# lebrice/blurred-GAN

Hardware: AMD Instinct MI355X
Metric: images/sec (G+D+GP step) (higher is better)
Workload: dtype f32; 1 GPU; celeba64 64x64x3 batch 256/GPU, blur sigma 5.0 (31 taps), D-step+GP+G-step+Adam; global_batch=256, parallelism=dp1

## Files before the change

### blurred-gan_amd/_lib.py

```python
from __future__ import annotations

import ctypes as C
import os

HERE = os.path.dirname(os.path.abspath(__file__))
LIB_PATH = os.environ.get("BGAN_HIP_LIB") or os.path.join(HERE, "libbgan_hip.so")


class BgError(RuntimeError):
    pass


class Epilogue(C.Structure):
    _fields_ = [("mode", C.c_int), ("bias", C.c_void_p), ("ref", C.c_void_p), ("keep", C.c_void_p),
                ("alpha", C.c_float), ("scale", C.c_float), ("splitk_ws", C.c_void_p), ("splitk_ws_bytes", C.c_size_t),
                ("keep_elems", C.c_size_t), ("stats", C.c_void_p), ("stats_capacity", C.c_size_t), ("stats_rows", C.POINTER(C.c_int))]


ABI_VERSION = 5
EPI_NONE, EPI_BIAS_LRELU, EPI_MUL_GRAD, EPI_TANH, EPI_AFFINE_LRELU = 0, 1, 2, 3, 4

_p, _i, _f, _z, _u64 = C.c_void_p, C.c_int, C.c_float, C.c_size_t, C.c_uint64

SIGNATURES = {
    "bg_version": (_i, []),
    "bg_last_error": (C.c_char_p, []),
    "bg_status_string": (C.c_char_p, [_i]),
    "bg_prof_enable": (_i, [_i]),
    "bg_prof_reset": (_i, []),
    "bg_prof_count": (_i, []),
    "bg_prof_get": (_i, [_i, C.c_char_p, _i, C.POINTER(_f), C.POINTER(C.c_double), C.POINTER(C.c_double)]),
    "bg_prof_get_exec": (_i, [_i, C.POINTER(C.c_double)]),
    "bg_prof_get_useful": (_i, [_i, C.POINTER(C.c_double)]),
    "bg_conv2d_useful_flops": (C.c_double, [_i] * 7),
    "bg_range_enable": (_i, [_i]),
    "bg_range_push": (_i, [C.c_char_p]),
    "bg_range_pop": (_i, []),
    "bg_blur_policy": (_i, [_f, _i, _i, C.POINTER(_f), C.POINTER(_f), C.POINTER(_i)]),
    "bg_gauss_kernel_1d": (_i, [_f, _f, C.POINTER(_f), _i, C.POINTER(_i)]),
    "bg_blur_workspace_bytes": (_z, [_i, _i, _i, _i, _i]),
    "bg_blur_nhwc_f32": (_i, [_p, _p, _i, _i, _i, _i, _p, _i, _p, _p]),
    "bg_blur3_lerp_supported": (_i, [_i, _i, _i, _i, _i]),
    "bg_blur3_lerp_nhwc_f32": (_i, [_p, _p, _p, _p, _i, _i, _i, _i, _p, _i, _p]),
    "bg_conv2d_splitk_workspace_bytes": (_z, [_i, _i, _i, _i, _i, _i, _i, _i]),
    "bg_conv2d_fwd": (_i, [_p, _p, _p, _i, _i, _i, _i, _i, _i, _i, C.POINTER(Epilogue), _p]),
    "bg_conv2d_bwd_data": (_i, [_p, _p, _p, _i, _i, _i, _i, _i, _i, _i, C.POINTER(Epilogue), _p]),
    "bg_conv2d_fwd_math": (_i, [_p, _p, _p, _i, _i, _i, _i, _i, _i, _i, C.POINTER(Epilogue), _p, _i]),
    "bg_conv2d_bwd_data_math": (_i, [_p, _p, _p, _i, _i, _i, _i, _i, _i, _i, C.POINTER(Epilogue), _p, _i]),
    "bg_conv2d_math_taken": (_i, [_i] * 9),
    "bg_conv2d_bwd_filter_workspace_bytes": (_z, [_i, _i, _i, _i, _i, _i, _i]),
    "bg_conv2d_bwd_filter": (_i, [_p, _p, _p, _i, _i, _i, _i, _i, _i, _i, _f, _f, _p, _z, _p]),
    "bg_transpose_last2": (_i, [_p, _p, _i, _i, _i, _p]),
    "bg_transpose_last2_batched": (_i, [_p, _p, _p, _i, _i, _p]),
    "bg_gemm_f32": (_i, [_p, _p, _p, _i, _i, _i, _i, _i, _p, _f, _f, _p]),
    "bg_colsum_workspace_bytes": (_z, [_i, _i]),
    "bg_colsum_f32": (_i, [_p, _p, _i, _i, _i, _f, _f, _p, _z, _p]),
    "bg_bn_workspace_bytes": (_z, [_i, _i]),
    "bg_bn_train_fwd": (_i, [_p, _p, _i, _i, _p, _p, _p, _p, _p, _p, _f, _f, _i, _f, _p, _z, _p]),
    "bg_bn_train_fwd_partials": (_i, [_p, _i, _p, _p, _i, _i, _p, _p, _p, _p, _p, _p, _f, _f, _i, _f, _p]),
    "bg_bn_sums_from_partials": (_i, [_p, _i, _i, _p, _p]),
    "bg_bn_infer_fwd": (_i, [_p, _p, _i, _i, _p, _p, _p, _p, _f, _f, _p]),
    "bg_bn_train_bwd": (_i, [_p, _p, _p, _p, _i, _i, _p, _p, _p, _p, _p, _p, _f, _p, _z, _p]),
    "bg_bn_fold_f32": (_i, [_p, _p, _p, _p, _f, _i, _p, _p, _p]),
    "bg_bn_fold_many_f32": (_i, [_i, _p, _p, _p, _p, _p, _p, _p, _p, _p]),
    "bg_bn_stats_f32": (_i, [_p, _i, _i, _p, _p, _z, _p]),
    "bg_bn_finalize_f32": (_i, [_p, _i, _i, _p, _p, _p, _p, _f, _f, _i, _p]),
    "bg_bn_apply_f32": (_i, [_p, _p, _i, _i, _p, _p, _p, _p, _f, _p]),
    "bg_bn_finalize_apply_f32": (_i, [_p, _i, _p, _p, _i, _i, _p, _p, _p, _p, _p, _p, _f, _f, _i, _f, _p]),
    "bg_bn_bwd_stats_f32": (_i, [_p, _p, _p, _i, _i, _p, _p, _p, _p, _f, _p, _p, _z, _p]),
    "bg_bn_bwd_apply_f32": (_i, [_p, _p, _p, _p, _i, _i, _i, _p, _p, _p, _p, _p, _f, _p]),
    "bg_bn_param_grads_f32": (_i, [_p, _i, _f, _p, _p, _p]),
    "bg_ln_route": (_i, [_i, C.POINTER(_i), C.POINTER(_i), C.POINTER(_i), C.POINTER(_i)]),
    "bg_ln_workspace_bytes": (_z, [_i, _i]),
    "bg_ln_fwd_f32": (_i, [_p, _p, _i, _i, _p, _p, _f, _f, _p, _f, _z, _p, _p, _p]),
    "bg_ln_bwd_f32": (_i, [_p, _p, _p, _i, _i, _p, _p, _p, _p, _f, _p, _f, _z, _p, _p, _i, _i, _p, _p, _i, _f, _f, _p, _z, _p]),
    "bg_ln_tangent_f32": (_i, [_p, _p, _p, _i, _i, _p, _p, _p, _p, _f, _p]),
    "bg_ln_gp_source_f32": (_i, [_p, _p, _p, _p, _i, _i, _p, _p, _p, _p, _f, _f, _p, _z, _p]),
    "bg_pixelnorm_route": (_i, [_i, C.POINTER(_i)]),
    "bg_pixelnorm_fwd_f32": (_i, [_p, _p, _p, _i, _i, _f, _f, _p]),
    "bg_pixelnorm_bwd_f32": (_i, [_p, _p, _p, _p, _i, _i, _f, _p]),
    "bg_diffaug_route": (_i, [_i, _i, _i, C.POINTER(_i), C.POINTER(_i)]),
    "bg_diffaug_plan": (_i, [_i, _i, _i, _i, _i] + [C.POINTER(_i)] * 5),
    "bg_diffaug_decode": (_i, [C.POINTER(_f), _i, _i, _i, _f, _f, C.POINTER(_f), C.POINTER(_i)]),
    "bg_diffaug_f32": (_i, [_p, _p, _p, _i, _i, _i, _i, _i, _f, _f, _i, _p]),
    "bg_diffaug_adjoint_f32": (_i, [_p, _p, _p, _i, _i, _i, _i, _i, _f, _f, _p]),
    "bg_mbstd_plan": (_i, [_i, _i, _i, _i, _i, _i, C.POINTER(_i)]),
    "bg_mbstd_workspace_bytes": (_z, [_i, _i, _i, _i]),
    "bg_mbstd_fwd_f32": (_i, [_p, _p, _p, _p, _p, _i, _i, _i, _i, _f, _p, _z, _p]),
    "bg_mbstd_bwd_f32": (_i, [_p, _p, _p, _p, _p, _p, _i, _i, _i, _i, _p]),
    "bg_mbstd_gp_f32": (_i, [_p, _p, _p, _p, _p, _p, _p, _p, _i, _i, _i, _i, _f, _p, _z, _p]),
    "bg_spectral_route":(_i, [_i, _i, _i] + [C.POINTER(_i)] * 8),
    "bg_spectral_workspace_bytes": (_z, [_p, _i]),
    "bg_spectral_power_f32": (_i, [_p, _p, _p, _p, _i, _i, _p, _z, _p]),
    "bg_spectral_scale_f32": (_i, [_p, _p, _p, _p, _p, _i, _p]),
    "bg_spectral_grad_f32": (_i, [_p, _p, _p, _p, _p, _i, _p, _z, _p]),
    "bg_eqlr_plan": (_i, [_i, _i, _i] + [C.POINTER(_i)] * 4),
    "bg_eqlr_check_table": (_i, [_p, _i, _z, _z]),
    "bg_eqlr_scale_f32": (_i, [_p, _z, _p, _z, _p, _p, _i, _p]),
    "bg_eqlr_grad_f32": (_i, [_p, _z, _p, _p, _i, _p]),
    "bg_lerp_f32":(_i, [_p, _p, _p, _p, _i, _i, _p]),
    "bg_row_norm_f32": (_i, [_p, _p, _i, _i, _p]),
    "bg_gp_seed_f32": (_i, [_p, _p, _f, _p, _i, _i, _p]),
    "bg_gp_seed_guarded_f32": (_i, [_p, _p, _f, _p, _i, _i, _p]),
    "bg_mul_grad_f32": (_i, [_p, _p, _p, _f, _f, _p, _z, _p]),
    "bg_tanh_bwd_f32": (_i, [_p, _p, _p, _z, _p]),
    "bg_outer_f32": (_i, [_p, _p, _p, _i, _i, _p]),
    "bg_fill_f32": (_i, [_p, _f, _z, _p]),
    "bg_scale_f32": (_i, [_p, _f, _z, _p]),
    "bg_copy_f32": (_i, [_p, _p, _z, _p]),
    "bg_upsample2x_nhwc_f32": (_i, [_p, _p, _i, _i, _i, _i, _f, _p, _p, _f, _f, _p]),
    "bg_pool2x_sum_nhwc_f32": (_i, [_p, _p, _i, _i, _i, _i, _f, _p]),
    "bg_wgangp_d_loss": (_i, [_p, _p, _p, _i, _f, _f, _f, _f, _p, _p, _p, _p]),
# ... 79 lines not shown
```

### blurred-gan_amd/csrc/conv_rows.hip

```cpp
#include "conv_common.h"
#include <algorithm>
#include <cstdlib>
#include <cstring>
#include <type_traits>

namespace {

typedef float floatx4 __attribute__((ext_vector_type(4)));

struct RowParams {
  const float* A;
  const float* Wt;
  float* C;
  int B, Hi, Wi, Ck, Ho, Wo, N;
  int pt, pl, flip;
  int R, strips;
  int wpr, ipw;
  int epi_mode;
  const float* bias;
  const float* ref;
  const unsigned char* keep;
  size_t keep_elems;
  float alpha, scale;
};

__device__ inline int floordiv(int a, int b) { return a >= 0 ? a / b : -((-a + b - 1) / b); }

__device__ inline float tanh_branchless(float x) {
  float ax = fabsf(x);
  ax = ax > 15.f ? 15.f : ax;
  const float e = __builtin_amdgcn_exp2f(ax * 2.885390081777927f);
  const float big = 1.f - 2.f * __builtin_amdgcn_rcpf(e + 1.f);
  const float x2 = ax * ax;
  const float small = ax * fmaf(x2, fmaf(x2, fmaf(x2, -17.f / 315.f, 2.f / 15.f), -1.f / 3.f), 1.f);
  return copysignf(ax < 0.1f ? small : big, x);
}

template <int KS, int K, int S, int PIXW, int EP>
__global__ __launch_bounds__(PIXW * 4) void conv_rows_scatter_kernel(const RowParams p) {
  constexpr int NTH = PIXW * 4;
  constexpr unsigned kOob = 0x80000000u;
  extern __shared__ __attribute__((aligned(16))) float row_lds[];
  constexpr int AS = 4 * KS + 4;
  float* abuf = row_lds;
  constexpr int PS = PIXW * 17 + 1;
  float* pbuf = row_lds + 2 * PIXW * AS;
  const int tid = threadIdx.x, lane = tid & 63, wave = tid >> 6;
  const int li = lane & 15, kq = lane >> 4;
  const int t = wave % p.wpr, img = wave / p.wpr;
  const int strip = blockIdx.x % p.strips, bgrp = blockIdx.x / p.strips;
  const int Ck = 4 * KS, N = p.N;
  const int y0 = strip * p.R, y1 = min(y0 + p.R, p.Ho);
  const int iy_lo = -floordiv(-(y0 + p.pt - (K - 1)), S);
  const int iy_hi = floordiv(y1 - 1 + p.pt, S);
  const int nrows = iy_hi - iy_lo + 1;
  const int nimg = min(p.ipw, p.B - bgrp * p.ipw);
  const size_t img0 = (size_t)bgrp * p.ipw;
  const __amdgpu_buffer_rsrc_t rsA = __builtin_amdgcn_make_buffer_rsrc(const_cast<float*>(p.A + img0 * p.Hi * p.Wi * Ck), 0,
                                                                        nimg * p.Hi * p.Wi * Ck * 4, 0x00020000);
  const __amdgpu_buffer_rsrc_t rsC = __builtin_amdgcn_make_buffer_rsrc(p.C + img0 * p.Ho * p.Wo * N, 0, nimg * p.Ho * p.Wo * N * 4, 0x00020000);

  float bw[K][KS];
  {
    const int lc = min(li, K * N - 1);
    const int kw = lc / N, n = lc - kw * N;
#pragma unroll
    for (int kh = 0; kh < K; ++kh) {
      const int tap = p.flip ? (K - 1 - kh) * K + (K - 1 - kw) : kh * K + kw;
#pragma unroll
      for (int ks = 0; ks < KS; ++ks) {
        const float w = p.Wt[((size_t)tap * N + n) * Ck + 4 * ks + kq];
        bw[kh][ks] = li < K * N ? w : 0.f;
      }
    }
  }
  floatx4 acc[K];
#pragma unroll
  for (int i = 0; i < K; ++i) acc[i] = floatx4{0.f, 0.f, 0.f, 0.f};

  constexpr int QPR = KS;
  constexpr int NQ = PIXW * QPR / NTH;
  static_assert(NQ >= 1, "Ck >= 16");
  unsigned g_off[NQ], l_off[NQ];
#pragma unroll
  for (int q = 0; q < NQ; ++q) {
    const int f = tid + q * NTH, pix = f / QPR, c4 = f - pix * QPR;
    const int im = pix / p.Wi, ix = pix - im * p.Wi;
    g_off[q] = im < nimg ? (unsigned)(((im * p.Hi * p.Wi + ix) * Ck + c4 * 4) * 4) : kOob;
    l_off[q] = (unsigned)(pix * AS + c4 * 4);
  }
  const int rowB = p.Wi * Ck * 4;
  auto gload = [&](int r, float4 (&g)[NQ]) {
    const int iy = iy_lo + r;
    const bool row_ok = r < nrows && (unsigned)iy < (unsigned)p.Hi;
    const unsigned add = row_ok ? (unsigned)(iy * rowB) : 0u, force = row_ok ? 0u : kOob;
#pragma unroll
    for (int q = 0; q < NQ; ++q)
      g[q] = __builtin_bit_cast(float4, __builtin_amdgcn_raw_buffer_load_b128(rsA, (g_off[q] + add) | force, 0, 0));
  };
  auto lstore = [&](int buf, const float4 (&g)[NQ]) {
#pragma unroll
    for (int q = 0; q < NQ; ++q) *reinterpret_cast<float4*>(abuf + (size_t)buf * PIXW * AS + l_off[q]) = g[q];
  };
  const float* afrag = abuf + ((size_t)img * p.Wi + 16 * t + li) * AS + kq;
  constexpr int NE = (S * (16 / K) + 3) / 4;
  constexpr int NTERM = (K + S - 1) / S;
  int e_src[NE][NTERM];
  unsigned e_dst[NE];
  float e_bias[NE], e_mul[NE];
  int e_n[NE];
  if (tid < 2 * S) pbuf[(size_t)tid * PS + PIXW * 17] = 0.f;
  {
    const int per_img = p.Wo * N;
#pragma unroll
    for (int q = 0; q < NE; ++q) {
      const int e = tid + q * NTH;
      const int im = e / per_img, rem = e - im * per_img;
      const int x = rem / N, n = rem - x * N;
      const bool ok = e < p.ipw * per_img && im < nimg;
      e_dst[q] = ok ? (unsigned)(((im * p.Ho * p.Wo + x) * N + n) * 4) : kOob;
      e_n[q] = n;
      e_bias[q] = ok && p.bias ? p.bias[n] : 0.f;
      e_mul[q] = ok && p.epi_mode == BG_EPI_AFFINE_LRELU ? p.ref[n] : 0.f;
#pragma unroll
      for (int i = 0; i < NTERM; ++i) {
        const int kw = (x + p.pl) % S + i * S;
        const int num = x + p.pl - kw, ix = num / S;
        e_src[q][i] = (ok && kw < K && num >= 0 && ix < p.Wi) ? (im * p.Wi + ix) * 17 + kw * N + n : PIXW * 17;
      }
    }
  }
  const size_t out0 = img0 * p.Ho * p.Wo * N;
  auto pwrite = [&](const floatx4& pacc, int slot) {
    float* pb = pbuf + (size_t)slot * PS;
#pragma unroll
    for (int rr = 0; rr < 4; ++rr) pb[((size_t)img * p.Wi + 16 * t + 4 * kq + rr) * 17 + li] = pacc[rr];
  };
  auto pstore = [&](int slot, int y, bool live) {
    const float* pb = pbuf + (size_t)slot * PS;
    float v[NE];
#pragma unroll
    for (int q = 0; q < NE; ++q) {
      v[q] = pb[e_src[q][0]];
#pragma unroll
      for (int i = 1; i < NTERM; ++i) v[q] += pb[e_src[q][i]];
    }
    const unsigned add = live ? (unsigned)(y * p.Wo * N * 4) : 0u, force = live ? 0u : kOob;
#pragma unroll
    for (int q = 0; q < NE; ++q) {
      const unsigned off = (e_dst[q] + add) | force;
      float o;
      if (EP == 0) {
        o = v[q] + e_bias[q];
      } else if (EP == 1) {
        o = tanh_branchless(v[q] + e_bias[q]);
      } else {
        const bool mine = (off & kOob) == 0;
        o = mine ? bg::apply_epilogue_pre(p, v[q], out0 + (off >> 2), e_bias[q], e_mul[q]) : 0.f;
      }
      __builtin_amdgcn_raw_buffer_store_b32(__builtin_bit_cast(unsigned, o), rsC, off, 0, 0);
    }
  };

  float4 g0[NQ], g1[NQ], g2[NQ], g3[NQ];
  gload(0, g0);
  gload(1, g1);
  gload(2, g2);
  gload(3, g3);
  lstore(0, g0);
  gload(4, g0);
#pragma unroll
  for (int i = 0; i < 4 * NE * S; ++i) __builtin_amdgcn_raw_buffer_store_b32(0u, rsC, kOob + 4u * i, 0, 0);
  int y_prev = 0;
  bool have_prev = false;
  auto flush_prev = [&](int prev_par) {
#pragma unroll
    for (int kh = 0; kh < S; ++kh) {
      const int y = y_prev + kh;
      pstore(prev_par * S + kh, y, have_prev & (y >= y0) & (y < y1));
    }
  };
  auto trip = [&](int r, auto parity, float4 (&g)[NQ]) {
    constexpr int cur = decltype(parity)::value;
    __syncthreads();
    float a[KS];
#pragma unroll
    for (int ks = 0; ks < KS; ++ks) a[ks] = afrag[(size_t)cur * PIXW * AS + 4 * ks];
#pragma unroll
    for (int ks = 0; ks < KS; ++ks)
#pragma unroll
      for (int kh = 0; kh < K; ++kh) acc[kh] = __builtin_amdgcn_mfma_f32_16x16x4f32(a[ks], bw[kh][ks], acc[kh], 0, 0, 0);
    flush_prev(cur ^ 1);
    lstore(cur ^ 1, g);
    gload(r + 5, g);
#pragma unroll
    for (int kh = 0; kh < S; ++kh) pwrite(acc[kh], cur * S + kh);
    y_prev = (iy_lo + r) * S - p.pt;
    have_prev = true;
#pragma unroll
    for (int i = 0; i < K; ++i) acc[i] = i + S < K ? acc[i + S] : floatx4{0.f, 0.f, 0.f, 0.f};
  };
  int r = 0;
  for (; r + 4 <= nrows; r += 4) {
    trip(r, std::integral_constant<int, 0>{}, g1);
    trip(r + 1, std::integral_constant<int, 1>{}, g2);
    trip(r + 2, std::integral_constant<int, 0>{}, g3);
    trip(r + 3, std::integral_constant<int, 1>{}, g0);
  }
  int last_par = 1;
  if (r < nrows) {
    trip(r, std::integral_constant<int, 0>{}, g1);
    last_par = 0;
    if (r + 1 < nrows) {
      trip(r + 1, std::integral_constant<int, 1>{}, g2);
      last_par = 1;
      if (r + 2 < nrows) {
        trip(r + 2, std::integral_constant<int, 0>{}, g3);
        last_par = 0;
      }
    }
  }
  __syncthreads();
  if (last_par == 0) flush_prev(0); else flush_prev(1);
}

template <int K, int S>
int launch_rows(const RowParams& p, dim3 grid, size_t lds, hipStream_t s) {
  const bool wide = p.Wi == 128;
  const int ep = p.epi_mode == BG_EPI_NONE ? 0 : p.epi_mode == BG_EPI_TANH ? 1 : 2;
#define BG_RS2(KSv, EPv) do { if (wide) bg::launch((conv_rows_scatter_kernel<KSv, K, S, 128, EPv>), grid, dim3(512), lds, s, p); \
                              else bg::launch((conv_rows_scatter_kernel<KSv, K, S, 64, EPv>), grid, dim3(256), lds, s, p); } while (0)
#define BG_RS(KSv) do { if (ep == 0) BG_RS2(KSv, 0); else if (ep == 1) BG_RS2(KSv, 1); else BG_RS2(KSv, 2); } while (0)
  switch (p.Ck) {
    case 16: BG_RS(4); return 1;
    case 32: BG_RS(8); return 1;
    case 64: BG_RS(16); return 1;
    default: return 0;
  }
#undef BG_RS
#undef BG_RS2
}

constexpr int kRgHalo = 16;

struct RowGParams {
  const float* A;
  const float* Wt;
  float* C;
  int B, Hi, Wi, Ct, Ho, Wo, N;
  int s, pt, pl, flip;
  int R, strips;
  int epi_mode;
  const float* bias;
  const float* ref;
  const unsigned char* keep;
  size_t keep_elems;
  float alpha, scale;
};

template <int TG, int NT, int K, bool MASK>
__global__ __launch_bounds__(256) void conv_rows_gather_kernel(const RowGParams p) {
  extern __shared__ __attribute__((aligned(16))) float xl[];
  const int tid = threadIdx.x, lane = tid & 63, wave = tid >> 6;
  const int li = lane & 15, kq = lane >> 4;
  const int Ct = p.Ct, N = 16 * NT, st = p.s;
  const int RS = p.Wi * Ct + 2 * kRgHalo;
  const int strip = blockIdx.x % p.strips, b = blockIdx.x / p.strips;
  const int oy0 = strip * p.R, rows = min(p.R, p.Ho - oy0);
  const int nrows_in = (rows - 1) * st + K;

  float bw[K][4][NT];
#pragma unroll
  for (int ks = 0; ks < 4; ++ks) {
    const int i = 4 * ks + kq, kw = i / Ct, ci = i - kw * Ct;
#pragma unroll
    for (int kh = 0; kh < K; ++kh) {
      const int tap = p.flip ? (K - 1 - kh) * K + (K - 1 - kw) : kh * K + kw;
#pragma unroll
      for (int nt = 0; nt < NT; ++nt) bw[kh][ks][nt] = i < K * Ct ? p.Wt[((size_t)tap * N + nt * 16 + li) * Ct + ci] : 0.f;
    }
  }
  const int RL = p.Wi * Ct;
// ... 89 lines not shown
#undef BG_RG
  return 1;
}

}

namespace bg {

int try_conv_rows_gather(int bwd_data, const float* a, const float* w, float* c, int B, int H, int W, int Cin, int Cout, int k, int s,
                         const bg_epilogue* epi, void* stream, int* taken) {
  *taken = 0;
  static const int off = getenv("BG_NO_ROWS") ? 1 : 0;
  if (off || (k != 5 && k != 3)) return BG_OK;
  RowGParams p;
  memset(&p, 0, sizeof p);
  int Ho, Wo, pt, pl;
  same_pads(H, k, s, &Ho, &pt);
  same_pads(W, k, s, &Wo, &pl);
  if (bwd_data) {
    if (s != 1 || Cout * k > 16 || (Cin != 16 && Cin != 32 && Cin != 64)) return BG_OK;
    p.Hi = H; p.Wi = W; p.Ct = Cout; p.Ho = H; p.Wo = W; p.N = Cin; p.s = 1; p.pt = k - 1 - pt; p.pl = k - 1 - pl; p.flip = 1;
  } else {
    if (Cin * k > 16 || (Cout != 16 && Cout != 32 && Cout != 64)) return BG_OK;
    p.Hi = H; p.Wi = W; p.Ct = Cin; p.Ho = Ho; p.Wo = Wo; p.N = Cout; p.s = s; p.pt = pt; p.pl = pl; p.flip = 0;
  }
  if (p.Wo % 16 != 0) return BG_OK;
  if ((size_t)B * p.Ho * p.Wo * p.N >= (1ull << 31)) return BG_OK;
  const int tiles = p.Wo / 16;
  const int tg = tiles % 4 == 0 ? 4 : (tiles % 2 == 0 ? 2 : 1);
  p.A = a; p.Wt = w; p.C = c; p.B = B;
  static const int rows_r = getenv("BG_ROWSG_R") ? atoi(getenv("BG_ROWSG_R")) : 0;
  p.R = std::min(rows_r ? rows_r : (s == 2 ? 8 : 16), p.Ho);
  p.strips = (int)cdiv(p.Ho, p.R);
  const size_t lds = ((size_t)((p.R - 1) * p.s + k) * (p.Wi * p.Ct + 2 * kRgHalo)) * sizeof(float);
  if (lds > 64 * 1024) return BG_OK;
  p.epi_mode = BG_EPI_NONE; p.alpha = 0.3f; p.scale = 1.f;
  if (epi) {
    BG_REQUIRE(epi->mode >= BG_EPI_NONE && epi->mode <= BG_EPI_AFFINE_LRELU, BG_ERR_UNSUPPORTED, "conv rows: epilogue mode %d", epi->mode);
    BG_REQUIRE(epi->mode != BG_EPI_MUL_GRAD || epi->ref, BG_ERR_NULL, "conv rows: BG_EPI_MUL_GRAD needs ref");
    BG_REQUIRE(epi->mode != BG_EPI_AFFINE_LRELU || (epi->ref && epi->bias), BG_ERR_NULL, "conv rows: BG_EPI_AFFINE_LRELU needs ref and bias");
    p.epi_mode = epi->mode; p.bias = epi->bias; p.ref = epi->ref; p.keep = epi->keep; p.keep_elems = epi->keep_elems; p.alpha = epi->alpha; p.scale = epi->scale;
  }
  const dim3 grid((unsigned)(B * p.strips));
  const double flops = 2.0 * B * (double)Ho * Wo * Cin * Cout * k * k;
  Launch L(stream, bwd_data ? "conv_rows_thin_k_dgrad" : "conv_rows_thin_k_fwd", flops, 0);
  if (k == 5) launch_rows_gather<5>(p, tg, grid, lds, L.s);
  else launch_rows_gather<3>(p, tg, grid, lds, L.s);
  *taken = 1;
  return L.done("conv_rows_gather_kernel");
}



int try_conv_rows(int bwd_data, const float* a, const float* w, float* c, int B, int H, int W, int Cin, int Cout, int k, int s,
                  const bg_epilogue* epi, void* stream, int* taken) {
  *taken = 0;
  static const int off = getenv("BG_NO_ROWS") ? 1 : 0;
  if (off || (k != 5 && k != 3)) return BG_OK;
  RowParams p;
  memset(&p, 0, sizeof p);
  int Ho, Wo, pt, pl;
  same_pads(H, k, s, &Ho, &pt);
  same_pads(W, k, s, &Wo, &pl);
  if (bwd_data) {
    if (Cin * k > 16 || (Cout != 16 && Cout != 32 && Cout != 64)) return BG_OK;
    p.Hi = Ho; p.Wi = Wo; p.Ck = Cout; p.Ho = H; p.Wo = W; p.N = Cin; p.pt = pt; p.pl = pl; p.flip = 0;
  } else {
    if (s != 1 || Cout * k > 16 || (Cin != 16 && Cin != 32 && Cin != 64)) return BG_OK;
    p.Hi = H; p.Wi = W; p.Ck = Cin; p.Ho = H; p.Wo = W; p.N = Cout; p.pt = k - 1 - pt; p.pl = k - 1 - pl; p.flip = 1;
  }
  if (p.Wi != 16 && p.Wi != 32 && p.Wi != 64 && p.Wi != 128) return BG_OK;
  if ((size_t)B * p.Hi * p.Wi * p.Ck >= (1ull << 31) || (size_t)B * p.Ho * p.Wo * p.N >= (1ull << 31)) return BG_OK;
  p.A = a; p.Wt = w; p.C = c; p.B = B;
  static const int rows_r = getenv("BG_ROWS_R") ? atoi(getenv("BG_ROWS_R")) : 0;
  p.R = std::min(rows_r ? rows_r : (s == 1 ? 32 : 16), p.Ho);
  p.strips = (int)cdiv(p.Ho, p.R);
  p.wpr = p.Wi / 16;
  p.ipw = p.Wi == 128 ? 1 : 4 / p.wpr;
  const int pixw = p.Wi == 128 ? 128 : 64;
  if ((long)p.ipw * p.Wo * p.N > (long)((s * (16 / k) + 3) / 4) * pixw * 4) return BG_OK;
  if ((size_t)p.ipw * p.Hi * p.Wi * p.Ck >= (1ull << 29) || (size_t)p.ipw * p.Ho * p.Wo * p.N >= (1ull << 29)) return BG_OK;
  p.epi_mode = BG_EPI_NONE; p.alpha = 0.3f; p.scale = 1.f;
  if (epi) {
    BG_REQUIRE(epi->mode >= BG_EPI_NONE && epi->mode <= BG_EPI_AFFINE_LRELU, BG_ERR_UNSUPPORTED, "conv rows: epilogue mode %d", epi->mode);
    BG_REQUIRE(epi->mode != BG_EPI_MUL_GRAD || epi->ref, BG_ERR_NULL, "conv rows: BG_EPI_MUL_GRAD needs ref");
    BG_REQUIRE(epi->mode != BG_EPI_AFFINE_LRELU || (epi->ref && epi->bias), BG_ERR_NULL, "conv rows: BG_EPI_AFFINE_LRELU needs ref and bias");
    p.epi_mode = epi->mode; p.bias = epi->bias; p.ref = epi->ref; p.keep = epi->keep; p.keep_elems = epi->keep_elems; p.alpha = epi->alpha; p.scale = epi->scale;
  }
  const dim3 grid((unsigned)(cdiv(B, p.ipw) * p.strips));
  const size_t lds = ((size_t)2 * pixw * (p.Ck + 4) + (size_t)2 * s * (pixw * 17 + 1)) * sizeof(float);
  const double flops = 2.0 * B * (double)H * W * Cin * Cout * k * k / (s * s);
  Launch L(stream, bwd_data ? "conv_rows_dgrad" : "conv_rows_fwd", flops, 0);
  int ok;
  if (k == 5) ok = s == 2 ? launch_rows<5, 2>(p, grid, lds, L.s) : launch_rows<5, 1>(p, grid, lds, L.s);
  else ok = s == 2 ? launch_rows<3, 2>(p, grid, lds, L.s) : launch_rows<3, 1>(p, grid, lds, L.s);
  (void)ok;
  *taken = 1;
  return L.done("conv_rows_scatter_kernel");
}

}
```

### blurred-gan_amd/csrc/conv_wgrad.hip

```cpp
#include "conv_common.h"
#include <algorithm>
#include <cmath>
#include <cstdlib>
#include <mutex>
#include <type_traits>
#include <utility>

namespace {

typedef float floatx16 __attribute__((ext_vector_type(16)));

struct WgradParams {
  const float* X;
  const float* DY;
  float* out;
  int B, H, W, Ci, Ho, Wo, Co;
  int k, s, pt, pl;
  int M;
  int chunk;
  int ksplit;
  int tiles_m, tiles_n, xcd_swizzle;
  float beta, scale;
  unsigned x_bytes, dy_bytes;
  unsigned mul_hw, sh_hw, mul_w, sh_w;
  int lg_w, lg_h, lg_b, pow2;
  int order_n;
  unsigned char tap_order[32];
};

__device__ inline int fastdiv(int m, unsigned mul, unsigned sh) { return (int)(((unsigned long long)(unsigned)m * mul) >> sh); }

template <int BM, int BN, int BKP, int WAVES_M, int WAVES_N, int WAVES_K, int P2>
__global__ __launch_bounds__(256) void conv_wgrad_v3_kernel(const WgradParams p) {
  static_assert(WAVES_M * WAVES_N * WAVES_K == 4, "4 waves");
  constexpr int WTM = BM / WAVES_M, WTN = BN / WAVES_N;
  constexpr int MI = WTM / 32, NI = WTN / 32;
  static_assert(MI >= 1 && NI >= 1 && WTM % 32 == 0 && WTN % 32 == 0, "wave tile");
  constexpr int TPR_A = BM / 4, RPP_A = 256 / TPR_A, AP = BKP / RPP_A;
  constexpr int TPR_B = BN / 4, RPP_B = 256 / TPR_B, BP = BKP / RPP_B;
  static_assert(AP >= 1 && BP >= 1 && BKP % RPP_A == 0 && BKP % RPP_B == 0, "loader passes must tile the chunk exactly");
  constexpr int STAGE = BKP * (BM + BN);
  constexpr int RED = (WAVES_K > 1) ? (WAVES_K - 1) * WAVES_M * WAVES_N * MI * NI * 1024 : 0;
  constexpr int SMEM = (2 * STAGE > RED) ? 2 * STAGE : RED;
  constexpr unsigned kOob = 0x80000000u;
  __shared__ __attribute__((aligned(16))) float smem[SMEM];

  const int tid = threadIdx.x, lane = tid & 63, wave = tid >> 6;
  const int wk = wave % WAVES_K, wmn = wave / WAVES_K;
  const int wm = wmn / WAVES_N, wn = wmn % WAVES_N;
  const int ntile = p.tiles_m * p.tiles_n, ntap = p.k * p.k;
  int tile, tap, zsplit;
  if (P2 == 2 && p.order_n > 0) {
    const int w = blockIdx.x, r = w >> 8;
    const int u = ((r & 1) && ((r + 1) << 8) <= (int)gridDim.x) ? (r << 8) + ((31 - ((w & 255) >> 3)) << 3) + (w & 7) : w;
    tile = u % ntile;
    const int rest = u / ntile;
    zsplit = rest % p.ksplit;
    tap = p.tap_order[rest / p.ksplit];
  } else {
    const int L = p.xcd_swizzle ? bg::xcd_remap(blockIdx.x, gridDim.x) : (int)blockIdx.x;
    tile = L % ntile; tap = (L / ntile) % ntap; zsplit = L / (ntile * ntap);
  }
  const int tile_m = tile / p.tiles_n, tile_n = tile % p.tiles_n;
  const int ci0 = tile_m * BM, co0 = tile_n * BN;
  const int kh = tap / p.k, kw = tap % p.k;
  const int m_begin = zsplit * p.chunk;
  const int m_end = min(p.M, m_begin + p.chunk);
  const int nsteps = (m_end - m_begin + BKP - 1) / BKP;

  const __amdgpu_buffer_rsrc_t rsX = __builtin_amdgcn_make_buffer_rsrc(const_cast<float*>(p.X), 0, (int)p.x_bytes, 0x00020000);
  const __amdgpu_buffer_rsrc_t rsY = __builtin_amdgcn_make_buffer_rsrc(const_cast<float*>(p.DY), 0, (int)p.dy_bytes, 0x00020000);
  const int arow = tid / TPR_A, aq = tid % TPR_A;
  const int brow = tid / TPR_B, bq = tid % TPR_B;
  const int HoWo = p.Ho * p.Wo;
  const bool a_col_ok = ci0 + aq * 4 < p.Ci, b_col_ok = co0 + bq * 4 < p.Co;
  const int a_coloff = (ci0 + aq * 4) * 4, b_coloff = (co0 + bq * 4) * 4;
  const int dyk = kh - p.pt, dxk = kw - p.pl;
  float4 regA[AP], regB[BP];

  const int WoS = p.Wo * p.s, HoS = p.Ho * p.s;
// ... 632 lines not shown
          const int ci = ci0 + row, co = co0 + col;
          ok = ci < p.Ci && co < p.Co;
          idx = ((size_t)tap * p.Ci + ci) * p.Co + co;
        } else if (MODE == 1) {
          const int co = co0 + col;
          ok = row < kk * p.Ci && co < p.Co;
          idx = (size_t)row * p.Co + co;
        } else {
          const int ci = ci0 + row;
          const int t = col / p.Co, co = col - t * p.Co;
          ok = ci < p.Ci && col < kk * p.Co;
          idx = ((size_t)t * p.Ci + ci) * p.Co + co;
        }
        if (ok) {
          float* q = out + idx;
          const float v = acc[i][j][r];
          if (direct) *q = (p.beta != 0.f ? p.beta * *q : 0.f) + p.scale * v;
          else *q = v;
        }
      }
    }
}

__global__ __launch_bounds__(256) void wgrad_direct_kernel(const WgradParams p) {
  const int nout = p.k * p.k * p.Ci * p.Co;
  const int e = blockIdx.x * 256 + threadIdx.x;
  if (e >= nout) return;
  const int co = e % p.Co;
  const int ci = (e / p.Co) % p.Ci;
  const int tap = e / (p.Co * p.Ci);
  const int kh = tap / p.k, kw = tap % p.k;
  const int m_begin = blockIdx.y * p.chunk, m_end = min(p.M, m_begin + p.chunk);
  const int HoWo = p.Ho * p.Wo;
  int b = m_begin / HoWo;
  int rem = m_begin - b * HoWo;
  int oh = rem / p.Wo, ow = rem - oh * p.Wo;
  float acc = 0.f;
  for (int m = m_begin; m < m_end; ++m) {
    const int iy = oh * p.s + kh - p.pt, ix = ow * p.s + kw - p.pl;
    if ((unsigned)iy < (unsigned)p.H && (unsigned)ix < (unsigned)p.W)
      acc = fmaf(p.X[((size_t)(b * p.H + iy) * p.W + ix) * p.Ci + ci], p.DY[(size_t)m * p.Co + co], acc);
    if (++ow == p.Wo) {
      ow = 0;
      if (++oh == p.Ho) { oh = 0; ++b; }
    }
  }
  float* q = p.out + (size_t)blockIdx.y * nout + e;
  if (p.ksplit == 1) *q = (p.beta != 0.f ? p.beta * *q : 0.f) + p.scale * acc;
  else *q = acc;
}

typedef float floatx4 __attribute__((ext_vector_type(4)));
constexpr int kTcRows = 16, kTcHalo = 8;

template <int MT, int K>
__global__ __launch_bounds__(256) void conv_wgrad_thin_co_kernel(const WgradParams p, int nblocks, int blocks_per_img) {
  extern __shared__ __attribute__((aligned(16))) float tc_lds[];
  const int W = p.W, H = p.H, Ci = 16 * MT, Co = p.Co;
  const int RS = W * Co + 2 * kTcHalo;
  const int nrows = kTcRows + K - 1;
  const int tid = threadIdx.x, lane = tid & 63, wave = tid >> 6;
  const int li = lane & 15, kq = lane >> 4;
  floatx4 acc[K][MT];
#pragma unroll
  for (int kh = 0; kh < K; ++kh)
#pragma unroll
    for (int mt = 0; mt < MT; ++mt) acc[kh][mt] = floatx4{0.f, 0.f, 0.f, 0.f};
  const int ncol = K * Co;
  const int kw_n = li / Co, co_n = li - kw_n * Co;
  const int b_base = li < ncol ? kTcHalo + (kq + p.pl - kw_n) * Co + co_n : 0;
  const int b_step = li < ncol ? 4 * Co : 0;
  const int ksteps = W / 4;

  for (int blk = blockIdx.x; blk < nblocks; blk += gridDim.x) {
    const int b = blk / blocks_per_img, y0 = (blk - b * blocks_per_img) * kTcRows;
    __syncthreads();
    if (((W * Co) & 3) == 0) {
      const int q4 = RS / 4;
      bg::stage_rows_f4<4>(tc_lds, nrows, q4, RS, tid, [&](int r, int c4) -> const float* {
        const int oy = y0 - (K - 1 - p.pt) + r, e = c4 * 4 - kTcHalo;
        return ((unsigned)oy < (unsigned)p.Ho && (unsigned)e < (unsigned)(W * Co)) ? p.DY + ((size_t)b * p.Ho + oy) * W * Co + e : nullptr;
      });
    } else {
      for (int idx = tid; idx < nrows * RS; idx += 256) {
        const int r = idx / RS, c = idx - r * RS;
        const int oy = y0 - (K - 1 - p.pt) + r, e = c - kTcHalo;
        float v = 0.f;
        if ((unsigned)oy < (unsigned)p.Ho && (unsigned)e < (unsigned)(W * Co)) v = p.DY[((size_t)b * p.Ho + oy) * W * Co + e];
        tc_lds[idx] = v;
      }
    }
    __syncthreads();
    const int groups = (ksteps + 7) / 8;
    const int myrows = min(kTcRows, H - y0);
    const int nitems = ((myrows - wave + 3) / 4) * groups;
    const float* xblk = p.X + ((size_t)b * H + y0) * W * Ci + kq * Ci + li;
    auto xload = [&](int it, float (&a)[8][MT]) {
      const int j = it / groups, g = it - j * groups;
      const float* xrow = xblk + (size_t)(wave + 4 * j) * W * Ci + (size_t)g * 32 * Ci;
#pragma unroll
      for (int q = 0; q < 8; ++q)
#pragma unroll
        for (int mt = 0; mt < MT; ++mt) a[q][mt] = (it < nitems && g * 8 + q < ksteps) ? xrow[(size_t)q * 4 * Ci + mt * 16] : 0.f;
    };
    auto compute = [&](int it, const float (&a)[8][MT]) {
      const int j = it / groups, g = it - j * groups;
      const int r = wave + 4 * j;
#pragma unroll
      for (int kh = 0; kh < K; ++kh) {
        const float* brow = tc_lds + (r + (K - 1) - kh) * RS + b_base + g * 8 * b_step;
#pragma unroll
        for (int q = 0; q < 8; ++q) {
          const float bv = brow[q * b_step];
#pragma unroll
          for (int mt = 0; mt < MT; ++mt) acc[kh][mt] = __builtin_amdgcn_mfma_f32_16x16x4f32(a[q][mt], bv, acc[kh][mt], 0, 0, 0);
        }
      }
    };
    float a0[8][MT], a1[8][MT];
    xload(0, a0);
    for (int it = 0; it < nitems; it += 2) {
      xload(it + 1, a1);
      compute(it, a0);
      xload(it + 2, a0);
      if (it + 1 < nitems) compute(it + 1, a1);
    }
  }
  __syncthreads();
  float* red = tc_lds;
#pragma unroll
  for (int kh = 0; kh < K; ++kh)
#pragma unroll
    for (int mt = 0; mt < MT; ++mt)
#pragma unroll
      for (int rr = 0; rr < 4; ++rr) red[((wave * K + kh) * MT * 4 + mt * 4 + rr) * 64 + lane] = acc[kh][mt][rr];
  __syncthreads();
  float* out = p.out + (size_t)blockIdx.x * K * K * Ci * Co;
  for (int e = tid; e < K * MT * 4 * 64; e += 256) {
    const int l = e & 63, slot = e >> 6;
    const int rr = slot & 3, mt = (slot >> 2) % MT, kh = slot / (4 * MT);
    const int n = l & 15;
    if (n >= ncol) continue;
    const float v = (red[(0 * K * MT * 4 + slot) * 64 + l] + red[(1 * K * MT * 4 + slot) * 64 + l]) +
                    (red[(2 * K * MT * 4 + slot) * 64 + l] + red[(3 * K * MT * 4 + slot) * 64 + l]);
    const int kw = n / Co, co = n - kw * Co, ci = mt * 16 + 4 * (l >> 4) + rr;
    out[((size_t)(kh * K + kw) * Ci + ci) * Co + co] = v;
  }
}

constexpr int kTiHalo = 16;

template <int NT, int K>
__global__ __launch_bounds__(256) void conv_wgrad_thin_ci_kernel(const WgradParams p, int nblocks, int blocks_per_img, int RB) {
  extern __shared__ __attribute__((aligned(16))) float ti_lds[];
  const int W = p.W, H = p.H, Ci = p.Ci, Co = 16 * NT, Ho = p.Ho, Wo = p.Wo, st = p.s;
  const int RS = W * Ci + 2 * kTiHalo;
  const int nrows = (RB - 1) * st + K;
  const int tid = threadIdx.x, lane = tid & 63, wave = tid >> 6;
  const int li = lane & 15, kq = lane >> 4;
  floatx4 acc[K][NT];
// ... 464 lines not shown
    }
    if (z < ksplit) {
      const float4 v0 = *reinterpret_cast<const float4*>(slabs + (size_t)z * n + e);
      s0.x += v0.x; s0.y += v0.y; s0.z += v0.z; s0.w += v0.w;
    }
  }
  red[zg][c] = make_float4(s0.x + s1.x, s0.y + s1.y, s0.z + s1.z, s0.w + s1.w);
  __syncthreads();
  for (int h = 32; h > 0; h >>= 1) {
    if (zg < h) {
      const float4 a = red[zg][c], b = red[zg + h][c];
      red[zg][c] = make_float4(a.x + b.x, a.y + b.y, a.z + b.z, a.w + b.w);
    }
    __syncthreads();
  }
  if (zg != 0 || e >= n) return;
  const float4 a = red[0][c];
  float4 o = make_float4(scale * a.x, scale * a.y, scale * a.z, scale * a.w);
  if (beta != 0.f) {
    const float4 q = *reinterpret_cast<const float4*>(dw + e);
    o.x += beta * q.x; o.y += beta * q.y; o.z += beta * q.z; o.w += beta * q.w;
  }
  *reinterpret_cast<float4*>(dw + e) = o;
}

__global__ __launch_bounds__(256) void wgrad_reduce_scalar_kernel(const float* __restrict__ slabs, float* __restrict__ dw, int n,
                                                                  int ksplit, float beta, float scale) {
  const int e = blockIdx.x * 256 + threadIdx.x;
  if (e >= n) return;
  float s = 0.f;
  for (int z = 0; z < ksplit; ++z) s += slabs[(size_t)z * n + e];
  dw[e] = (beta != 0.f ? beta * dw[e] : 0.f) + scale * s;
}

struct WgradPlan {
  int mode;
  int ksplit, chunk, tiles_m, tiles_n, bkp, taps_in_grid;
  int always_slab;
};

inline bool strip_ok(int H, int W, int Ci, int Co, int k, int s) {
  if (k != 5 || s != 2 || (H & 1) || (W & 1) || Ci % 32 || Co % 64) return false;
  const int Wo = W / 2, Ho = H / 2;
  if (Wo != 8 && Wo != 16 && Wo != 32) return false;
  return Ho % (64 / Wo) == 0;
}

constexpr size_t kRowLdsMax = 64 * 1024;
inline int thin_ci_rows(int s) { return s == 2 ? 8 : 16; }
inline size_t thin_ci_lds(int W, int Ci, int Co, int k, int s) {
  return std::max((size_t)((thin_ci_rows(s) - 1) * s + k) * ((size_t)W * Ci + 2 * kTiHalo), (size_t)k * (Co / 16) * 4 * 64) * sizeof(float);
}
inline size_t thin_co_lds(int W, int Ci, int Co, int k) {
  return std::max((size_t)(kTcRows + k - 1) * ((size_t)W * Co + 2 * kTcHalo), (size_t)4 * k * (Ci / 16) * 4 * 64) * sizeof(float);
}

WgradPlan plan_wgrad(int B, int H, int W, int Ci, int Co, int k, int s) {
  WgradPlan pl{};
  int Ho, Wo, pt, pp;
  bg::same_pads(H, k, s, &Ho, &pt);
  bg::same_pads(W, k, s, &Wo, &pp);
  const long M = (long)B * Ho * Wo;
  const bool mfma = (Ci % 4 == 0) && (Co % 4 == 0) && Ci >= 16 && Co >= 16;
  const int kk = k * k;
  const bool thin_ci = Ci <= 4 && Co % 4 == 0 && Co >= 16 && kk * Ci <= 128;
  const bool thin_co = Co <= 4 && Ci % 4 == 0 && Ci >= 16 && s == 1 && kk * Co <= 128;
  int bm = 0, bn = 0;
  if (!mfma && !thin_ci && !thin_co) {
    pl.mode = 0;
    const long nblk = bg::cdiv((size_t)k * k * Ci * Co, 256);
    long want = std::max(1L, 2048 / nblk);
    long chunk = std::max(256L, (M + want - 1) / want);
    pl.chunk = (int)chunk;
    pl.ksplit = (int)((M + chunk - 1) / chunk);
    return pl;
  }
  static const int no_strip = getenv("BG_WGRAD_NO_STRIP") ? 1 : 0;
  if (strip_ok(H, W, Ci, Co, k, s) && !no_strip) {
    pl.mode = 33;
    pl.bkp = 2;
    pl.tiles_m = Ci / 32;
    pl.tiles_n = Co / 64;
    const long nstrips = (long)B * (Ho / (64 / Wo));
    const long ntile = (long)pl.tiles_m * pl.tiles_n;
    long ks = std::max(1L, std::min(nstrips, std::max(1L, 256 / ntile)));
    long spw = (nstrips + ks - 1) / ks;
    ks = (nstrips + spw - 1) / spw;
    pl.ksplit = (int)ks;
    pl.chunk = (int)spw;
    pl.taps_in_grid = 0;
    pl.always_slab = 1;
    return pl;
  }
  static const int no_c16 = getenv("BG_NO_C16") ? 1 : 0;
  if (Ci == 16 && Co == 32 && k == 5 && s == 2 && !(H & 1) && !(W & 1) && (Wo == 32 || Wo == 64) && !(Ho & 1) && !no_c16) {
    pl.mode = 32;
    pl.bkp = 4;
    const long nstrips = (long)B * (Ho / 2);
    pl.ksplit = (int)std::max<long>(2, std::min<long>(nstrips, 256));
    pl.chunk = (int)nstrips;
    pl.tiles_m = pl.tiles_n = 1;
    pl.taps_in_grid = 0;
    return pl;
  }
  static const int no_tc = getenv("BG_WGRAD_NO_TC") ? 1 : 0;
  if (thin_ci && k * Ci <= 16 && (k == 5 || k == 3) && (Co == 16 || Co == 32 || Co == 64) && Wo % 4 == 0 && !no_tc &&
      thin_ci_lds(W, Ci, Co, k, s) <= kRowLdsMax) {
// ... 39 lines not shown
  static const int no_tg = getenv("BG_WGRAD_NO_TG") ? 1 : 0;
  if (k == 5 && Ci <= 64 && !no_tg && M >= 131072) {
    pl.bkp = 32; bm = 32;
    if (Co > 32) { pl.mode = 6; bn = 64; } else { pl.mode = 7; bn = 32; }
    pl.tiles_m = bg::cdiv(Ci, bm);
    pl.tiles_n = bg::cdiv(Co, bn);
    pl.taps_in_grid = 2;
  } else {
  if (Ci > 64 && Co > 64) { pl.mode = 1; bm = 128; bn = 128; pl.bkp = 32; }
  else if (Ci > 32 && Co > 32) { pl.mode = 2; bm = 64; bn = 64; pl.bkp = 32; }
  else if (Ci > 32) { pl.mode = 3; bm = 64; bn = 32; pl.bkp = 64; }
  else if (Co > 32) { pl.mode = 4; bm = 32; bn = 64; pl.bkp = 64; }
  else { pl.mode = 5; bm = 32; bn = 32; pl.bkp = 128; }
  pl.tiles_m = bg::cdiv(Ci, bm);
  pl.tiles_n = bg::cdiv(Co, bn);
  pl.taps_in_grid = 1;
  }
  }
  const long base = (long)pl.tiles_m * pl.tiles_n * (pl.taps_in_grid == 1 ? kk : (pl.taps_in_grid == 2 ? k : 1));
  const long steps = (M + pl.bkp - 1) / pl.bkp;
  long want;
  const bool skipping = Ho * Wo <= 16 && B >= 128 && B % 128 == 0;
  if (pl.taps_in_grid != 1 || skipping) {
    static const int tgt_env = getenv("BG_WGRAD_TARGET") ? atoi(getenv("BG_WGRAD_TARGET")) : 0;
    const int tgt = tgt_env ? tgt_env : (pl.taps_in_grid == 2 && M >= 200000 ? 1536 : 768);
    want = std::max(1L, (tgt + base - 1) / base);
    want = std::min(want, std::max(1L, steps / (skipping ? 8 : 4)));
    if ((size_t)kk * Ci * Co * sizeof(float) > (8u << 20)) want = std::min(want, 2L);
  } else {
    const int bm_eff = pl.taps_in_grid == 2 ? k * bm : bm;
    const int lds = 2 * pl.bkp * (bm_eff + bn) * 4;
    const int per_cu = std::max(1, std::min(160 * 1024 / lds, 5));
    const double slots = 256.0 * per_cu;
    const double t_step = 2.0 * bm_eff * bn * pl.bkp * per_cu / 614e9 * 1e6;
    const double ovh = 5.0 / t_step;
    const double nout_bytes = (double)kk * Ci * Co * 4.0;
    double best = 1e30;
    want = 1;
    for (long ks = 1; ks <= std::min<long>(64, std::max(1L, steps / 4)); ++ks) {
      const double rounds = std::ceil(base * ks / slots);
      const double per_wg = std::ceil((double)steps / ks);
      const double cost = rounds * (per_wg + ovh) * t_step + (ks > 1 ? 5.0 + (ks + 1) * nout_bytes / 3.5e6 + ks * nout_bytes / 5e6 : 0.0);
      if (cost < best * 0.999) { best = cost; want = ks; }
    }
  }
  long chunk = ((M + want - 1) / want + pl.bkp - 1) / pl.bkp * pl.bkp;
  pl.chunk = (int)chunk;
  pl.ksplit = (int)((M + chunk - 1) / chunk);
  return pl;
}

}

extern "C" {

size_t bg_conv2d_bwd_filter_workspace_bytes(int B, int H, int W, int Cin, int Cout, int ksize, int stride) {
  if (B <= 0 || H <= 0 || W <= 0 || Cin <= 0 || Cout <= 0 || ksize <= 0 || stride <= 0) return 0;
  WgradPlan pl = plan_wgrad(B, H, W, Cin, Cout, ksize, stride);
  if (pl.ksplit <= 1 && !pl.always_slab) return 0;
  return (size_t)pl.ksplit * ksize * ksize * Cin * Cout * sizeof(float);
}

int bg_conv2d_bwd_filter(const float* x, const float* dy, float* dw, int B, int H, int W, int Cin, int Cout, int ksize,
                         int stride, float beta, float scale, void* ws_d, size_t ws_bytes, void* stream) {
  BG_REQUIRE(x && dy && dw, BG_ERR_NULL, "bg_conv2d_bwd_filter: null pointer");
  BG_REQUIRE(B > 0 && H > 0 && W > 0 && Cin > 0 && Cout > 0, BG_ERR_BAD_SHAPE, "bg_conv2d_bwd_filter: B=%d H=%d W=%d Cin=%d Cout=%d", B, H, W, Cin, Cout);
  BG_REQUIRE(ksize >= 1 && (ksize & 1) && ksize * ksize <= bg::kMaxTaps, BG_ERR_UNSUPPORTED, "bg_conv2d_bwd_filter: kernel size %d", ksize);
  BG_REQUIRE(stride == 1 || stride == 2, BG_ERR_UNSUPPORTED, "bg_conv2d_bwd_filter: stride %d", stride);
  BG_REQUIRE(bg::aligned16(x) && bg::aligned16(dy) && bg::aligned16(dw), BG_ERR_BAD_ALIGNMENT, "bg_conv2d_bwd_filter: pointers must be 16-byte aligned");
  bg::UsefulScope useful(bg::conv_useful_flops(B, H, W, Cin, Cout, ksize, stride));
  WgradPlan pl = plan_wgrad(B, H, W, Cin, Cout, ksize, stride);
  const size_t nout = (size_t)ksize * ksize * Cin * Cout;
  const bool slabs = pl.ksplit > 1 || pl.always_slab;
  const size_t need = slabs ? (size_t)pl.ksplit * nout * sizeof(float) : 0;
  BG_REQUIRE(need == 0 || (ws_d && ws_bytes >= need), BG_ERR_WORKSPACE, "bg_conv2d_bwd_filter: workspace %zu bytes < %zu needed", ws_bytes, need);
  WgradParams p;
  memset(&p, 0, sizeof p);
  p.X = x; p.DY = dy;
  p.B = B; p.H = H; p.W = W; p.Ci = Cin; p.Co = Cout; p.k = ksize; p.s = stride;
  bg::same_pads(H, ksize, stride, &p.Ho, &p.pt);
  bg::same_pads(W, ksize, stride, &p.Wo, &p.pl);
  p.M = B * p.Ho * p.Wo;
  BG_REQUIRE((size_t)B * H * W * (size_t)Cin < (1ull << 29) && (size_t)p.M * (size_t)Cout < (1ull << 29), BG_ERR_UNSUPPORTED,
             "bg_conv2d_bwd_filter: tensor exceeds 2 GiB");
  {
    auto magic = [](unsigned d, unsigned* mul, unsigned* sh) {
      unsigned sft = 0;
      while ((1ull << sft) < d) ++sft;
      *mul = (unsigned)((1ull << (31 + sft)) / d + 1);
      *sh = 31 + sft;
    };
    magic((unsigned)(p.Ho * p.Wo), &p.mul_hw, &p.sh_hw);
    magic((unsigned)p.Wo, &p.mul_w, &p.sh_w);
    auto lg2 = [](int v) { int l = 0; while ((1 << l) < v) ++l; return l; };
    p.lg_w = lg2(p.Wo); p.lg_h = lg2(p.Ho);
    p.pow2 = ((1 << p.lg_w) == p.Wo && (1 << p.lg_h) == p.Ho) ? 1 : 0;
    p.lg_b = lg2(B);
    static const int no_pm = getenv("BG_NO_POS_MAJOR") ? 1 : 0;
    if (p.pow2 && !no_pm && B % 128 == 0 && B >= 128 && p.Ho * p.Wo <= 16) p.pow2 = 2;
    p.x_bytes = (unsigned)((size_t)B * H * W * Cin * sizeof(float));
    p.dy_bytes = (unsigned)((size_t)p.M * Cout * sizeof(float));
  }
  p.chunk = pl.chunk; p.ksplit = pl.ksplit; p.tiles_n = pl.tiles_n; p.tiles_m = pl.tiles_m;
  {
    static const int swz = getenv("BG_WGRAD_SWZ") ? atoi(getenv("BG_WGRAD_SWZ")) : 0;
    static const int swz_tg = getenv("BG_WGRAD_SWZ_TG") ? atoi(getenv("BG_WGRAD_SWZ_TG")) : 1;
    p.xcd_swizzle = (pl.mode == 6 || pl.mode == 7) ? swz_tg : swz;
  }
  p.beta = beta; p.scale = scale;
  p.order_n = 0;
  {
    static const int no_sort = getenv("BG_NO_TILE_SORT") ? 1 : 0;
    if (p.pow2 == 2 && pl.taps_in_grid == 1 && pl.mode >= 1 && pl.mode <= 5 && !no_sort && ksize * ksize <= 32) {
      int live[32], idx[32];
      for (int t = 0; t < ksize * ksize; ++t) {
        const int dyk = t / ksize - p.pt, dxk = t % ksize - p.pl;
        auto floordiv = [](int a, int b) { return a >= 0 ? a / b : -((-a + b - 1) / b); };
        const int oh_lo = std::max(0, (-dyk + stride - 1) / stride), oh_hi = std::min(p.Ho - 1, floordiv(H - 1 - dyk, stride));
        const int ow_lo = std::max(0, (-dxk + stride - 1) / stride), ow_hi = std::min(p.Wo - 1, floordiv(W - 1 - dxk, stride));
        live[t] = std::max(0, oh_hi - oh_lo + 1) * std::max(0, ow_hi - ow_lo + 1);
        idx[t] = t;
      }
      std::stable_sort(idx, idx + ksize * ksize, [&](int a, int b) { return live[a] > live[b]; });
      for (int t = 0; t < ksize * ksize; ++t) p.tap_order[t] = (unsigned char)idx[t];
      p.order_n = ksize * ksize;
    }
  }
  p.out = slabs ? static_cast<float*>(ws_d) : dw;
  const double flops = 2.0 * p.M * (double)nout;
  const double abytes = 4.0 * ((double)B * H * W * Cin + (double)p.M * Cout + (double)nout * (beta != 0.f ? 2 : 1));
  int rc;
  if (pl.mode == 0) {
    bg::Launch L(stream, "conv_wgrad_direct", flops, abytes);
    bg::launch(wgrad_direct_kernel, dim3(bg::cdiv(nout, 256), pl.ksplit), dim3(256), 0, L.s, p);
    rc = L.done("wgrad_direct_kernel");
  } else if (pl.mode == 33) {
    bg::Launch L(stream, "conv_wgrad_mfma", flops, abytes);
    const int lgwo = p.Wo == 32 ? 5 : (p.Wo == 16 ? 4 : 3);
    const int spi = p.Ho / (64 / p.Wo), nstrips = B * spi, ntile = pl.tiles_m * pl.tiles_n;
    BG_LDS_ATTR_ONCE_V(conv_wgrad_strip_kernel<5>, StripGeom<5>::lds_bytes);
    BG_LDS_ATTR_ONCE_V(conv_wgrad_strip_kernel<4>, StripGeom<4>::lds_bytes);
    BG_LDS_ATTR_ONCE_V(conv_wgrad_strip_kernel<3>, StripGeom<3>::lds_bytes);
    const dim3 grid((unsigned)(ntile * pl.ksplit));
    if (lgwo == 5) bg::launch((conv_wgrad_strip_kernel<5>), grid, dim3(256), StripGeom<5>::lds_bytes, L.s, p, nstrips, spi, pl.chunk, ntile);
    else if (lgwo == 4) bg::launch((conv_wgrad_strip_kernel<4>), grid, dim3(256), StripGeom<4>::lds_bytes, L.s, p, nstrips, spi, pl.chunk, ntile);
    else bg::launch((conv_wgrad_strip_kernel<3>), grid, dim3(256), StripGeom<3>::lds_bytes, L.s, p, nstrips, spi, pl.chunk, ntile);
    rc = L.done("conv_wgrad_strip_kernel");
  } else if (pl.mode == 32) {
    bg::Launch L(stream, "conv_wgrad_c16", flops, abytes);
    const int spi = p.Ho / 2, nstrips = B * spi;
    const size_t lds = std::max((size_t)2 * kC16Rows * 2 * (p.Wo + 2) * 16, (size_t)25 * 2 * 4 * 64) * sizeof(float);
    BG_LDS_ATTR_ONCE_V(conv_wgrad_c16_kernel<64>, 150 * 1024);
    BG_LDS_ATTR_ONCE_V(conv_wgrad_c16_kernel<32>, 150 * 1024);
    if (p.Wo == 64) bg::launch((conv_wgrad_c16_kernel<64>), dim3(pl.ksplit), dim3(256), lds, L.s, p, nstrips, spi);
    else bg::launch((conv_wgrad_c16_kernel<32>), dim3(pl.ksplit), dim3(256), lds, L.s, p, nstrips, spi);
    rc = L.done("conv_wgrad_c16_kernel");
  } else if (pl.mode == 31) {
    bg::Launch L(stream, "conv_wgrad_mfma_thin_ci", flops, abytes);
    const int rb = thin_ci_rows(stride);
    const int bpi = (int)bg::cdiv(p.Ho, rb), nblocks = B * bpi;
    const int nt = Cout / 16;
    const size_t lds = thin_ci_lds(W, Cin, Cout, ksize, stride);
    BG_REQUIRE(lds <= kRowLdsMax, BG_ERR_UNSUPPORTED, "bg_conv2d_bwd_filter: thin-Ci row kernel needs %zu bytes of LDS", lds);
#define BG_TI(NTv, Kv) bg::launch((conv_wgrad_thin_ci_kernel<NTv, Kv>), dim3(pl.ksplit), dim3(256), lds, L.s, p, nblocks, bpi, rb)
    if (ksize == 5) { if (nt == 1) BG_TI(1, 5); else if (nt == 2) BG_TI(2, 5); else BG_TI(4, 5); }
    else { if (nt == 1) BG_TI(1, 3); else if (nt == 2) BG_TI(2, 3); else BG_TI(4, 3); }
#undef BG_TI
    rc = L.done("conv_wgrad_thin_ci_kernel");
  } else if (pl.mode == 30) {
    bg::Launch L(stream, "conv_wgrad_mfma_thin_co", flops, abytes);
    const int bpi = (int)bg::cdiv(H, kTcRows), nblocks = B * bpi;
    const int mt = Cin / 16;
    const size_t lds = thin_co_lds(W, Cin, Cout, ksize);
    BG_REQUIRE(lds <= kRowLdsMax, BG_ERR_UNSUPPORTED, "bg_conv2d_bwd_filter: thin-Co row kernel needs %zu bytes of LDS", lds);
    if (ksize == 5 && mt == 2) bg::launch((conv_wgrad_thin_co_kernel<2, 5>), dim3(pl.ksplit), dim3(256), lds, L.s, p, nblocks, bpi);
    else if (ksize == 5) bg::launch((conv_wgrad_thin_co_kernel<1, 5>), dim3(pl.ksplit), dim3(256), lds, L.s, p, nblocks, bpi);
    else if (mt == 2) bg::launch((conv_wgrad_thin_co_kernel<2, 3>), dim3(pl.ksplit), dim3(256), lds, L.s, p, nblocks, bpi);
    else bg::launch((conv_wgrad_thin_co_kernel<1, 3>), dim3(pl.ksplit), dim3(256), lds, L.s, p, nblocks, bpi);
    rc = L.done("conv_wgrad_thin_co_kernel");
  } else {
    dim3 grid(pl.tiles_m * pl.tiles_n, pl.taps_in_grid == 1 ? ksize * ksize : (pl.taps_in_grid == 2 ? ksize : 1), pl.ksplit);
    bg::Launch L(stream, pl.mode >= 20 ? "conv_wgrad_mfma_thin_co" : (pl.mode >= 10 ? "conv_wgrad_mfma_thin_ci" : "conv_wgrad_mfma"), flops, abytes);
    const dim3 grid1((unsigned)(grid.x * grid.y * grid.z));
    switch (pl.mode) {
#define BG_V3(BMv, BNv, BKv, WMv, WNv, WKv)                                                                               \
  do {                                                                                                                   \
    if (p.pow2 == 2) bg::launch((conv_wgrad_v3_kernel<BMv, BNv, BKv, WMv, WNv, WKv, 2>), grid1, dim3(256), 0, L.s, p);     \
    else if (p.pow2 == 1) bg::launch((conv_wgrad_v3_kernel<BMv, BNv, BKv, WMv, WNv, WKv, 1>), grid1, dim3(256), 0, L.s, p); \
    else bg::launch((conv_wgrad_v3_kernel<BMv, BNv, BKv, WMv, WNv, WKv, 0>), grid1, dim3(256), 0, L.s, p);        \
  } while (0)
      case 1: BG_V3(128, 128, 32, 2, 2, 1); break;
      case 2: BG_V3(64, 64, 32, 2, 2, 1); break;
      case 3: BG_V3(64, 32, 64, 2, 1, 2); break;
      case 4: BG_V3(32, 64, 64, 1, 2, 2); break;
      case 5: BG_V3(32, 32, 128, 1, 1, 4); break;
#undef BG_V3
      case 6: bg::launch((conv_wgrad_tg_kernel<5, 64, 2, 2>), grid1, dim3(256), 0, L.s, p); break;
      case 7: bg::launch((conv_wgrad_tg_kernel<5, 32, 1, 4>), grid1, dim3(256), 0, L.s, p); break;
      case 10: bg::launch((conv_wgrad_kernel<32, 64, 64, 1, 2, 2, 1>), grid, dim3(256), 0, L.s, p); break;
      case 11: bg::launch((conv_wgrad_kernel<96, 32, 64, 1, 1, 4, 1>), grid, dim3(256), 0, L.s, p); break;
      case 12: bg::launch((conv_wgrad_kernel<128, 32, 64, 1, 1, 4, 1>), grid, dim3(256), 0, L.s, p); break;
      case 20: bg::launch((conv_wgrad_kernel<64, 32, 64, 2, 1, 2, 2>), grid, dim3(256), 0, L.s, p); break;
      case 21: bg::launch((conv_wgrad_kernel<32, 96, 64, 1, 1, 4, 2>), grid, dim3(256), 0, L.s, p); break;
      default: bg::launch((conv_wgrad_kernel<32, 128, 64, 1, 1, 4, 2>), grid, dim3(256), 0, L.s, p); break;
    }
    rc = L.done("conv_wgrad_kernel");
  }
  if (rc) return rc;
  if (slabs) {
    bg::Launch L(stream, "conv_wgrad_reduce", 0, (double)(pl.ksplit + 1) * nout * 4);
    if (nout % 4 == 0 && bg::aligned16(ws_d) && pl.ksplit >= 64 && nout <= 65536)
      bg::launch(wgrad_reduce_tall_kernel, dim3(bg::cdiv(nout / 4, 16)), dim3(1024), 0, L.s, static_cast<const float*>(ws_d), dw,
                         (int)nout, pl.ksplit, beta, scale);
    else if (nout % 4 == 0 && bg::aligned16(ws_d))
      bg::launch(wgrad_reduce_kernel, dim3(bg::cdiv(nout / 4, 64)), dim3(256), 0, L.s, static_cast<const float*>(ws_d), dw,
                         (int)nout, pl.ksplit, beta, scale);
    else
      bg::launch(wgrad_reduce_scalar_kernel, dim3(bg::cdiv(nout, 256)), dim3(256), 0, L.s, static_cast<const float*>(ws_d), dw,
                         (int)nout, pl.ksplit, beta, scale);
    rc = L.done("wgrad_reduce_kernel");
  }
  return rc;
}

}
```

### blurred-gan_amd/csrc/misc.hip

```cpp
#include "common.h"
#include "reduce.h"
#include <algorithm>
#include <cmath>

namespace {

__device__ inline bool bg_aligned16(const void* p) { return (reinterpret_cast<uintptr_t>(p) & 15u) == 0; }

constexpr int kT = 256;

inline unsigned grid_for(size_t n, int per_thread = 1) { return bg::grid_cap(n, kT, per_thread); }

__global__ __launch_bounds__(kT) void gemm_naive_kernel(const float* __restrict__ A, const float* __restrict__ Bm,
                                                        float* __restrict__ C, int M, int N, int K, int transA, int transB,
                                                        const float* __restrict__ bias, float beta, float scale) {
  const size_t total = (size_t)M * N;
  for (size_t e = (size_t)blockIdx.x * kT + threadIdx.x; e < total; e += (size_t)gridDim.x * kT) {
    const int m = (int)(e / N), n = (int)(e - (size_t)m * N);
    float acc = 0.f;
    for (int k = 0; k < K; ++k) {
      const float a = transA ? A[(size_t)k * M + m] : A[(size_t)m * K + k];
      const float b = transB ? Bm[(size_t)n * K + k] : Bm[(size_t)k * N + n];
      acc = fmaf(a, b, acc);
    }
    float v = scale * acc;
    if (bias) v += bias[n];
    if (beta != 0.f) v += beta * C[e];
    C[e] = v;
  }
}

typedef float gemm_floatx16 __attribute__((ext_vector_type(16)));
__global__ __launch_bounds__(kT) void gemm_tiled_kernel(const float* __restrict__ A, const float* __restrict__ Bm,
                                                        float* __restrict__ C, int M, int N, int K, int transA, int transB,
                                                        const float* __restrict__ bias, float beta, float scale) {
  constexpr int KT = 32, NL = 64 * KT / kT;
  __shared__ float As[KT][64 + 4], Bs[KT][64 + 4];
  const int lane = threadIdx.x & 63, wave = threadIdx.x >> 6;
  const int li = lane & 31, kk = lane >> 5, wm = wave >> 1, wn = wave & 1;
  const int m0 = blockIdx.y * 64, n0 = blockIdx.x * 64;
  gemm_floatx16 acc;
#pragma unroll
  for (int q = 0; q < 16; ++q) acc[q] = 0.f;
  float ra[NL], rb[NL];
  auto gload = [&](int k0) {
#pragma unroll
    for (int i = 0; i < NL; ++i) {
      const int e = threadIdx.x + i * kT;
      int ka, mm;
      if (transA) { ka = e >> 6; mm = e & 63; } else { mm = e / KT; ka = e - mm * KT; }
      const int m = m0 + mm, k = k0 + ka;
      ra[i] = (m < M && k < K) ? (transA ? A[(size_t)k * M + m] : A[(size_t)m * K + k]) : 0.f;
// ... 193 lines not shown
    return o;
  }, [&](const Ops& o, int c4, float4* a) {
    const float4 d = o.d, xx = o.xx;
    const float4 mu = *reinterpret_cast<const float4*>(mean + c4), iv = *reinterpret_cast<const float4*>(inv + c4);
    float4 yy = o.yy;
    if (!y) {
      const float4 g = make_float4(gamma[c4], gamma[c4 + 1], gamma[c4 + 2], gamma[c4 + 3]);
      const float4 bt = make_float4(beta[c4], beta[c4 + 1], beta[c4 + 2], beta[c4 + 3]);
      yy.x = bn_pre_act(xx.x, g.x, mu.x, iv.x, bt.x); yy.y = bn_pre_act(xx.y, g.y, mu.y, iv.y, bt.y);
      yy.z = bn_pre_act(xx.z, g.z, mu.z, iv.z, bt.z); yy.w = bn_pre_act(xx.w, g.w, mu.w, iv.w, bt.w);
    }
    const float dz0 = d.x * (yy.x > 0.f ? 1.f : alpha), dz1 = d.y * (yy.y > 0.f ? 1.f : alpha);
    const float dz2 = d.z * (yy.z > 0.f ? 1.f : alpha), dz3 = d.w * (yy.w > 0.f ? 1.f : alpha);
    a[0].x += dz0; a[0].y += dz1; a[0].z += dz2; a[0].w += dz3;
    a[1].x = fmaf(dz0, (xx.x - mu.x) * iv.x, a[1].x); a[1].y = fmaf(dz1, (xx.y - mu.y) * iv.y, a[1].y);
    a[1].z = fmaf(dz2, (xx.z - mu.z) * iv.z, a[1].z); a[1].w = fmaf(dz3, (xx.w - mu.w) * iv.w, a[1].w);
  }, M, C, partial);
}

__device__ inline float wave_sum_partials(const float* __restrict__ partial, int nblk, int NQ, int q, int C, int c) {
  float s = bg::lane_sum_partials(partial, nblk, NQ, q, C, c);
  for (int off = 32; off > 0; off >>= 1) s += __shfl_down(s, off, 64);
  return __shfl(s, 0, 64);
}

__global__ __launch_bounds__(kT) void colsum_partial_kernel(const float* __restrict__ x, int M, int N, int square, float* partial) {
  col_reduce<1>([&](int m, int n, float* a) {
    const float v = x[(size_t)m * N + n];
    a[0] += square ? v * v : v;
  }, M, N, partial);
}

__global__ __launch_bounds__(kT) void colsum_final_kernel(const float* __restrict__ partial, int nblk, int N, float* out, float beta,
                                                          float scale) {
  const int n = blockIdx.x * (kT / 64) + (threadIdx.x >> 6);
  if (n >= N) return;
  const float s = wave_sum_partials(partial, nblk, 1, 0, N, n);
  if ((threadIdx.x & 63) == 0) out[n] = (beta != 0.f ? beta * out[n] : 0.f) + scale * s;
}

int col_blocks(int M) { return std::max(1, std::min(kColBlocks, M / 16)); }
int red_blocks(int M, int C) { return flat_ok(M, C) ? flat_blocks(M, C) : col_blocks(M); }

__global__ __launch_bounds__(kT) void bn_stats_partial_kernel(const float* __restrict__ x, int M, int C, float* partial) {
  col_reduce<2>([&](int m, int n, float* a) {
    const float v = x[(size_t)m * C + n];
    a[0] += v;
    a[1] = fmaf(v, v, a[1]);
  }, M, C, partial);
}

__global__ __launch_bounds__(kT) void bn_stats_final_kernel(const float* __restrict__ partial, int nblk, int M, int C, float* save_mean,
                                                            float* save_inv, float* moving_mean, float* moving_var, float eps,
                                                            float momentum, int unbiased) {
  const int c = blockIdx.x * (kT / 64) + (threadIdx.x >> 6);
  if (c >= C) return;
  const float s = wave_sum_partials(partial, nblk, 2, 0, C, c), s2 = wave_sum_partials(partial, nblk, 2, 1, C, c);
  if ((threadIdx.x & 63) != 0) return;
  const float mean = s / (float)M;
  const float var = fmaxf(s2 / (float)M - mean * mean, 0.f);
  save_mean[c] = mean;
  save_inv[c] = 1.0f / sqrtf(var + eps);
  if (moving_mean) {
    const float vu = unbiased ? var * ((float)M / (float)max(M - 1, 1)) : var;
    moving_mean[c] = moving_mean[c] * momentum + mean * (1.f - momentum);
    moving_var[c] = moving_var[c] * momentum + vu * (1.f - momentum);
  }
}

__global__ __launch_bounds__(kT) void bn_fold_kernel(const float* __restrict__ gamma, const float* __restrict__ beta,
                                                     const float* __restrict__ mm, const float* __restrict__ mv, float eps, int C,
                                                     float* scale, float* shift) {
  const int c = blockIdx.x * kT + threadIdx.x;
  if (c >= C) return;
  const float s = gamma[c] * (1.0f / sqrtf(mv[c] + eps));
  scale[c] = s;
  shift[c] = beta[c] - mm[c] * s;
}

constexpr int kFoldMax = 8;
struct FoldMany {
  const float* gamma[kFoldMax]; const float* beta[kFoldMax]; const float* mm[kFoldMax]; const float* mv[kFoldMax];
  float* scale[kFoldMax]; float* shift[kFoldMax];
  float eps[kFoldMax]; int C[kFoldMax];
};
__global__ __launch_bounds__(kT) void bn_fold_many_kernel(const FoldMany f) {
  const int l = blockIdx.y, c = blockIdx.x * kT + threadIdx.x;
  if (c >= f.C[l]) return;
  const float s = f.gamma[l][c] * (1.0f / sqrtf(f.mv[l][c] + f.eps[l]));
  f.scale[l][c] = s;
  f.shift[l][c] = f.beta[l][c] - f.mm[l][c] * s;
}

__global__ __launch_bounds__(kT) void partials_to_sums_kernel(const float* __restrict__ partial, int nblk, int C, float* sums) {
  const int c = blockIdx.x * (kT / 64) + (threadIdx.x >> 6);
  if (c >= C) return;
  const float s0 = wave_sum_partials(partial, nblk, 2, 0, C, c), s1 = wave_sum_partials(partial, nblk, 2, 1, C, c);
  if ((threadIdx.x & 63) == 0) {
    sums[c] = s0;
    sums[C + c] = s1;
  }
}

__global__ __launch_bounds__(kT) void bn_finalize_sums_kernel(const float* __restrict__ sums, int M, int C, float* save_mean,
                                                              float* save_inv, float* moving_mean, float* moving_var, float eps,
                                                              float momentum, int unbiased) {
  const int c = blockIdx.x * kT + threadIdx.x;
  if (c >= C) return;
  const float mean = sums[c] / (float)M;
  const float var = fmaxf(sums[C + c] / (float)M - mean * mean, 0.f);
  save_mean[c] = mean;
  save_inv[c] = 1.0f / sqrtf(var + eps);
  if (moving_mean) {
    const float vu = unbiased ? var * ((float)M / (float)max(M - 1, 1)) : var;
    moving_mean[c] = moving_mean[c] * momentum + mean * (1.f - momentum);
    moving_var[c] = moving_var[c] * momentum + vu * (1.f - momentum);
  }
}

__device__ inline float4 load4_param(const float* __restrict__ p, int c, bool al16) {
  if (al16) return *reinterpret_cast<const float4*>(p + c);
  return make_float4(p[c], p[c + 1], p[c + 2], p[c + 3]);
}
__device__ inline bool ptr_al16(const void* p) { return (reinterpret_cast<uintptr_t>(p) & 15) == 0; }

__global__ __launch_bounds__(kT) void bn_finalize_apply_kernel(const float* __restrict__ sums, int M, const float* __restrict__ x,
                                                               float* __restrict__ y, size_t total, int C, const float* __restrict__ gamma,
                                                               const float* __restrict__ beta, float* save_mean, float* save_inv,
                                                               float* moving_mean, float* moving_var, float eps, float momentum,
                                                               int unbiased, float alpha) {
  for (size_t e = (size_t)blockIdx.x * kT + threadIdx.x; e < total; e += (size_t)gridDim.x * kT) {
    const int c = (int)(e % C);
    const float mean = sums[c] / (float)M;
    const float var = fmaxf(sums[C + c] / (float)M - mean * mean, 0.f);
    const float inv = 1.0f / sqrtf(var + eps);
    if (e < (size_t)C) {
      save_mean[c] = mean;
      save_inv[c] = inv;
      if (moving_mean) {
        const float vu = unbiased ? var * ((float)M / (float)max(M - 1, 1)) : var;
        moving_mean[c] = moving_mean[c] * momentum + mean * (1.f - momentum);
        moving_var[c] = moving_var[c] * momentum + vu * (1.f - momentum);
      }
    }
    const float v = gamma[c] * ((x[e] - mean) * inv) + beta[c];
    y[e] = v > 0.f ? v : alpha * v;
  }
}

__global__ __launch_bounds__(kT) void bn_apply_kernel(const float* __restrict__ x, float* __restrict__ y, size_t total, int C,
                                                      const float* __restrict__ gamma, const float* __restrict__ beta,
                                                      const float* __restrict__ mean, const float* __restrict__ inv_or_var,
                                                      int is_var, float eps, float alpha) {
  if ((C & 3) == 0 && ptr_al16(x) && ptr_al16(y) && total <= 0xffffffffull) {
    const bool pa = ptr_al16(gamma) && ptr_al16(beta) && ptr_al16(mean) && ptr_al16(inv_or_var);
    const unsigned total4 = (unsigned)(total >> 2);
    const unsigned stride = gridDim.x * kT;
    auto one = [&](const float4& xv, const float4& g, const float4& bt, const float4& m, const float4& iv) {
      float4 v;
      v.x = g.x * ((xv.x - m.x) * iv.x) + bt.x; v.y = g.y * ((xv.y - m.y) * iv.y) + bt.y;
      v.z = g.z * ((xv.z - m.z) * iv.z) + bt.z; v.w = g.w * ((xv.w - m.w) * iv.w) + bt.w;
      v.x = v.x > 0.f ? v.x : alpha * v.x; v.y = v.y > 0.f ? v.y : alpha * v.y;
      v.z = v.z > 0.f ? v.z : alpha * v.z; v.w = v.w > 0.f ? v.w : alpha * v.w;
      return v;
    };
    auto params = [&](int c, float4& g, float4& bt, float4& m, float4& iv) {
      g = load4_param(gamma, c, pa); bt = load4_param(beta, c, pa); m = load4_param(mean, c, pa);
      iv = load4_param(inv_or_var, c, pa);
      if (is_var) { iv.x = 1.0f / sqrtf(iv.x + eps); iv.y = 1.0f / sqrtf(iv.y + eps); iv.z = 1.0f / sqrtf(iv.z + eps); iv.w = 1.0f / sqrtf(iv.w + eps); }
    };
    unsigned q = blockIdx.x * kT + threadIdx.x;
    if ((stride * 4u) % (unsigned)C == 0u) {
      float4 g, bt, m, iv;
      params((int)((q * 4u) % (unsigned)C), g, bt, m, iv);
      for (; q + stride < total4; q += 2 * stride) {
        const float4 x0 = *reinterpret_cast<const float4*>(x + q * 4u), x1 = *reinterpret_cast<const float4*>(x + (q + stride) * 4u);
        *reinterpret_cast<float4*>(y + q * 4u) = one(x0, g, bt, m, iv);
        *reinterpret_cast<float4*>(y + (q + stride) * 4u) = one(x1, g, bt, m, iv);
      }
      if (q < total4) *reinterpret_cast<float4*>(y + q * 4u) = one(*reinterpret_cast<const float4*>(x + q * 4u), g, bt, m, iv);
      return;
    }
    for (; q < total4; q += stride) {
      const unsigned e = q * 4u;
      float4 g, bt, m, iv;
      params((int)(e % (unsigned)C), g, bt, m, iv);
      *reinterpret_cast<float4*>(y + e) = one(*reinterpret_cast<const float4*>(x + e), g, bt, m, iv);
    }
    return;
  }
  for (size_t e = (size_t)blockIdx.x * kT + threadIdx.x; e < total; e += (size_t)gridDim.x * kT) {
    const int c = (int)(e % C);
    const float inv = is_var ? 1.0f / sqrtf(inv_or_var[c] + eps) : inv_or_var[c];
    float v = gamma[c] * ((x[e] - mean[c]) * inv) + beta[c];
    y[e] = v > 0.f ? v : alpha * v;
  }
}

__global__ __launch_bounds__(kT) void bn_bwd_partial_kernel(const float* __restrict__ dy, const float* __restrict__ y,
                                                            const float* __restrict__ x, int M, int C, const float* __restrict__ gamma,
                                                            const float* __restrict__ beta,
                                                            const float* __restrict__ mean, const float* __restrict__ inv, float alpha,
                                                            float* partial) {
  col_reduce<2>([&](int m, int n, float* a) {
    const size_t e = (size_t)m * C + n;
    const float yv = y ? y[e] : bn_pre_act(x[e], gamma[n], mean[n], inv[n], beta[n]);
    const float dz = dy[e] * (yv > 0.f ? 1.f : alpha);
    a[0] += dz;
    a[1] = fmaf(dz, (x[e] - mean[n]) * inv[n], a[1]);
  }, M, C, partial);
}

__global__ __launch_bounds__(kT) void bn_bwd_final_kernel(const float* __restrict__ partial, int nblk, int C, float* dgamma, float* dbeta) {
  const int c = blockIdx.x * (kT / 64) + (threadIdx.x >> 6);
  if (c >= C) return;
  const float s = wave_sum_partials(partial, nblk, 2, 0, C, c), s2 = wave_sum_partials(partial, nblk, 2, 1, C, c);
  if ((threadIdx.x & 63) != 0) return;
  dbeta[c] = s;
  dgamma[c] = s2;
}

__global__ __launch_bounds__(kT) void bn_bwd_apply_kernel(const float* __restrict__ dy, const float* __restrict__ y,
                                                          const float* __restrict__ x, float* __restrict__ dx, size_t total, int M , int C,
                                                          const float* __restrict__ gamma, const float* __restrict__ beta,
                                                          const float* __restrict__ mean,
                                                          const float* __restrict__ inv, const float* __restrict__ dgamma,
                                                          const float* __restrict__ dbeta, float alpha) {
  const float invM = 1.0f / (float)M;
  if ((C & 3) == 0 && ptr_al16(dy) && ptr_al16(y) && ptr_al16(x) && ptr_al16(dx) && total <= 0xffffffffull) {
    const bool pa = ptr_al16(gamma) && ptr_al16(mean) && ptr_al16(inv) && ptr_al16(dgamma) && ptr_al16(dbeta) && ptr_al16(beta);
    const unsigned total4 = (unsigned)(total >> 2);
    const float fM = (float)M;
    const unsigned stride = gridDim.x * kT;
    struct P { float4 g, m, iv, dg, db, bt; };
    auto params = [&](int c) {
      P p;
      p.g = load4_param(gamma, c, pa); p.m = load4_param(mean, c, pa); p.iv = load4_param(inv, c, pa);
      p.dg = load4_param(dgamma, c, pa); p.db = load4_param(dbeta, c, pa);
      p.bt = y ? make_float4(0.f, 0.f, 0.f, 0.f) : load4_param(beta, c, pa);
      return p;
    };
    auto one = [&](const float4& dyv, const float4& xv, float4 yv, const P& p) {
      if (!y) {
        yv.x = bn_pre_act(xv.x, p.g.x, p.m.x, p.iv.x, p.bt.x); yv.y = bn_pre_act(xv.y, p.g.y, p.m.y, p.iv.y, p.bt.y);
        yv.z = bn_pre_act(xv.z, p.g.z, p.m.z, p.iv.z, p.bt.z); yv.w = bn_pre_act(xv.w, p.g.w, p.m.w, p.iv.w, p.bt.w);
      }
      float4 o;
#define BG_BN_BWD1(k)                                                   \
// ... 386 lines not shown
extern "C" {

int bg_gemm_f32(const float* A, const float* Bm, float* C, int M, int N, int K, int transA, int transB, const float* bias,
                float beta, float scale, void* stream) {
  BG_REQUIRE(A && Bm && C, BG_ERR_NULL, "bg_gemm_f32: null pointer");
  BG_REQUIRE(M > 0 && N > 0 && K > 0, BG_ERR_BAD_SHAPE, "bg_gemm_f32: M=%d N=%d K=%d", M, N, K);
  const double flops = 2.0 * M * (double)N * K;
  if (N == 1 && !transA && K >= 64) {
    bg::Launch L(stream, "dense_rowdot", flops, 4.0 * M * K);
    bg::launch(rowdot_kernel, dim3(M), dim3(kT), 0, L.s, A, Bm, C, M, K, bias, beta, scale);
    return L.done("rowdot_kernel");
  }
  if (N == 1 && transA && K >= 64) {
    bg::Launch L(stream, "dense_gemv_t", flops, 4.0 * M * K);
    bg::launch(gemv_t_kernel, dim3(bg::cdiv(M, 64)), dim3(1024), 0, L.s, A, Bm, C, M, K, bias, beta, scale);
    return L.done("gemv_t_kernel");
  }
  if ((size_t)M * N >= 4096 && K >= 8) {
    bg::Launch L(stream, "dense_gemm_tiled", flops, 0);
    bg::launch(gemm_tiled_kernel, dim3(bg::cdiv(N, 64), bg::cdiv(M, 64)), dim3(kT), 0, L.s, A, Bm, C, M, N, K, transA, transB, bias, beta, scale);
    return L.done("gemm_tiled_kernel");
  }
  bg::Launch L(stream, "dense_gemm", flops, 0);
  bg::launch(gemm_naive_kernel, dim3(grid_for((size_t)M * N)), dim3(kT), 0, L.s, A, Bm, C, M, N, K, transA, transB, bias, beta, scale);
  return L.done("gemm_naive_kernel");
}

size_t bg_colsum_workspace_bytes(int M, int N) {
  if (M <= 0 || N <= 0) return 0;
  return (size_t)std::max(col_blocks(M), 512) * 2 * N * sizeof(float);
}

int bg_colsum_f32(const float* x, float* out, int M, int N, int square, float beta, float scale, void* ws_d, size_t ws_bytes,
                  void* stream) {
  BG_REQUIRE(x && out, BG_ERR_NULL, "bg_colsum_f32: null pointer");
  BG_REQUIRE(M > 0 && N > 0, BG_ERR_BAD_SHAPE, "bg_colsum_f32: M=%d N=%d", M, N);
  BG_REQUIRE(ws_d && ws_bytes >= bg_colsum_workspace_bytes(M, N), BG_ERR_WORKSPACE, "bg_colsum_f32: workspace too small");
  const int nblk = red_blocks(M, N);
  float* partial = static_cast<float*>(ws_d);
  {
    bg::Launch L(stream, "colsum_partial", 0, 4.0 * M * N);
    if (flat_ok(M, N) && bg::aligned16(x)) bg::launch(colsum_flat_kernel, dim3(nblk), dim3(kT), 0, L.s, x, M, N, square, partial);
    else bg::launch(colsum_partial_kernel, dim3(nblk, bg::cdiv(N, 64)), dim3(kT), 0, L.s, x, M, N, square, partial);
    int rc = L.done("colsum_partial_kernel");
    if (rc) return rc;
  }
  bg::Launch L(stream, "colsum_final", 0, 0);
  bg::launch(colsum_final_kernel, dim3(bg::cdiv(N, kT / 64)), dim3(kT), 0, L.s, partial, nblk, N, out, beta, scale);
  return L.done("colsum_final_kernel");
}

size_t bg_bn_workspace_bytes(int M, int C) { return bg_colsum_workspace_bytes(M, C); }

int bg_bn_train_fwd(const float* x, float* y, int M, int C, const float* gamma, const float* beta, float* moving_mean,
                    float* moving_var, float* save_mean, float* save_inv, float eps, float momentum, int unbiased,
                    float lrelu_alpha, void* ws_d, size_t ws_bytes, void* stream) {
  BG_REQUIRE(x && y && gamma && beta && save_mean && save_inv, BG_ERR_NULL, "bg_bn_train_fwd: null pointer");
  BG_REQUIRE((moving_mean == nullptr) == (moving_var == nullptr), BG_ERR_NULL, "bg_bn_train_fwd: moving_mean/var must both be given or both NULL");
  BG_REQUIRE(M > 0 && C > 0, BG_ERR_BAD_SHAPE, "bg_bn_train_fwd: M=%d C=%d", M, C);
  BG_REQUIRE(ws_d && ws_bytes >= bg_bn_workspace_bytes(M, C), BG_ERR_WORKSPACE, "bg_bn_train_fwd: workspace too small");
  const int nblk = red_blocks(M, C);
  float* partial = static_cast<float*>(ws_d);
  const size_t total = (size_t)M * C;
  {
    bg::Launch L(stream, "bn_stats_partial", 0, 4.0 * total);
    if (flat_ok(M, C) && bg::aligned16(x)) bg::launch(bn_stats_flat_kernel, dim3(nblk), dim3(kT), 0, L.s, x, M, C, partial);
    else bg::launch(bn_stats_partial_kernel, dim3(nblk, bg::cdiv(C, 64)), dim3(kT), 0, L.s, x, M, C, partial);
    int rc = L.done("bn_stats_partial_kernel");
    if (rc) return rc;
  }
  {
    bg::Launch L(stream, "bn_stats_final", 0, 0);
    bg::launch(bn_stats_final_kernel, dim3(bg::cdiv(C, kT / 64)), dim3(kT), 0, L.s, partial, nblk, M, C, save_mean, save_inv,
                       moving_mean, moving_var, eps, momentum, unbiased);
    int rc = L.done("bn_stats_final_kernel");
    if (rc) return rc;
  }
  bg::Launch L(stream, "bn_apply_lrelu", 0, 8.0 * total);
  bg::launch(bn_apply_kernel, dim3(grid_for(total)), dim3(kT), 0, L.s, x, y, total, C, gamma, beta, save_mean, save_inv, 0, eps,
                     lrelu_alpha);
  return L.done("bn_apply_kernel");
}

int bg_bn_train_fwd_partials(const float* partial_d, int nrows, const float* x, float* y, int M, int C, const float* gamma,
                             const float* beta, float* moving_mean, float* moving_var, float* save_mean, float* save_inv, float eps,
                             float momentum, int unbiased, float lrelu_alpha, void* stream) {
  BG_REQUIRE(partial_d && x && y && gamma && beta && save_mean && save_inv, BG_ERR_NULL, "bg_bn_train_fwd_partials: null pointer");
  BG_REQUIRE((moving_mean == nullptr) == (moving_var == nullptr), BG_ERR_NULL, "bg_bn_train_fwd_partials: moving_mean/var must both be given or both NULL");
  BG_REQUIRE(M > 0 && C > 0 && nrows > 0, BG_ERR_BAD_SHAPE, "bg_bn_train_fwd_partials: M=%d C=%d nrows=%d", M, C, nrows);
  const size_t total = (size_t)M * C;
  {
    bg::Launch L(stream, "bn_stats_final", 0, 0);
    bg::launch(bn_stats_final_kernel, dim3(bg::cdiv(C, kT / 64)), dim3(kT), 0, L.s, partial_d, nrows, M, C, save_mean, save_inv,
                       moving_mean, moving_var, eps, momentum, unbiased);
    int rc = L.done("bn_stats_final_kernel");
    if (rc) return rc;
  }
  bg::Launch L(stream, "bn_apply_lrelu", 0, 8.0 * total);
  bg::launch(bn_apply_kernel, dim3(grid_for(total)), dim3(kT), 0, L.s, x, y, total, C, gamma, beta, save_mean, save_inv, 0, eps,
                     lrelu_alpha);
  return L.done("bn_apply_kernel");
}

int bg_bn_sums_from_partials(const float* partial_d, int nrows, int C, float* sums_d, void* stream) {
  BG_REQUIRE(partial_d && sums_d, BG_ERR_NULL, "bg_bn_sums_from_partials: null pointer");
  BG_REQUIRE(C > 0 && nrows > 0, BG_ERR_BAD_SHAPE, "bg_bn_sums_from_partials: C=%d nrows=%d", C, nrows);
  bg::Launch L(stream, "bn_stats_final", 0, 0);
  bg::launch(partials_to_sums_kernel, dim3(bg::cdiv(C, kT / 64)), dim3(kT), 0, L.s, partial_d, nrows, C, sums_d);
  return L.done("partials_to_sums_kernel");
}

int bg_bn_infer_fwd(const float* x, float* y, int M, int C, const float* gamma, const float* beta, const float* moving_mean,
                    const float* moving_var, float eps, float lrelu_alpha, void* stream) {
  BG_REQUIRE(x && y && gamma && beta && moving_mean && moving_var, BG_ERR_NULL, "bg_bn_infer_fwd: null pointer");
  BG_REQUIRE(M > 0 && C > 0, BG_ERR_BAD_SHAPE, "bg_bn_infer_fwd: M=%d C=%d", M, C);
  const size_t total = (size_t)M * C;
  bg::Launch L(stream, "bn_apply_lrelu", 0, 8.0 * total);
  bg::launch(bn_apply_kernel, dim3(grid_for(total)), dim3(kT), 0, L.s, x, y, total, C, gamma, beta, moving_mean, moving_var, 1,
                     eps, lrelu_alpha);
  return L.done("bn_apply_kernel");
}

int bg_bn_train_bwd(const float* dy, const float* y, const float* x, float* dx, int M, int C, const float* gamma, const float* beta,
                    const float* save_mean, const float* save_inv, float* dgamma, float* dbeta, float lrelu_alpha, void* ws_d,
                    size_t ws_bytes, void* stream) {
  BG_REQUIRE(dy && (y || beta) && x && dx && gamma && save_mean && save_inv && dgamma && dbeta, BG_ERR_NULL, "bg_bn_train_bwd: null pointer");
  BG_REQUIRE(y || lrelu_alpha >= 0.f, BG_ERR_UNSUPPORTED, "bg_bn_train_bwd: the sign of y follows from x only for lrelu_alpha >= 0");
  BG_REQUIRE(M > 0 && C > 0, BG_ERR_BAD_SHAPE, "bg_bn_train_bwd: M=%d C=%d", M, C);
  BG_REQUIRE(ws_d && ws_bytes >= bg_bn_workspace_bytes(M, C), BG_ERR_WORKSPACE, "bg_bn_train_bwd: workspace too small");
  const int nblk = red_blocks(M, C);
  float* partial = static_cast<float*>(ws_d);
  const size_t total = (size_t)M * C;
  {
    bg::Launch L(stream, "bn_bwd_partial", 0, (y ? 12.0 : 8.0) * total);
    if (flat_ok(M, C) && bg::aligned16(dy) && bg::aligned16(y) && bg::aligned16(x) && bg::aligned16(save_mean) && bg::aligned16(save_inv))
      bg::launch(bn_bwd_flat_kernel, dim3(nblk), dim3(kT), 0, L.s, dy, y, x, M, C, gamma, beta, save_mean, save_inv, lrelu_alpha, partial);
    else
      bg::launch(bn_bwd_partial_kernel, dim3(nblk, bg::cdiv(C, 64)), dim3(kT), 0, L.s, dy, y, x, M, C, gamma, beta, save_mean, save_inv,
                         lrelu_alpha, partial);
    int rc = L.done("bn_bwd_partial_kernel");
    if (rc) return rc;
  }
  {
    bg::Launch L(stream, "bn_bwd_final", 0, 0);
    bg::launch(bn_bwd_final_kernel, dim3(bg::cdiv(C, kT / 64)), dim3(kT), 0, L.s, partial, nblk, C, dgamma, dbeta);
    int rc = L.done("bn_bwd_final_kernel");
    if (rc) return rc;
// ... 318 lines not shown
```

### blurred-gan_amd/engine.py

```python
from __future__ import annotations

import functools
import os
from typing import List, Optional

import numpy as np
import torch

from . import dist, ops
from ._lib import EPI_NONE, EPI_BIAS_LRELU, EPI_MUL_GRAD, EPI_TANH, EPI_AFFINE_LRELU
from .layers import EqualizedLearningRate, SpectralNormalization


RESAMPLE = ("upsample", "avgpool")
PARAMETER_FREE = RESAMPLE + ("mbstd",)
SOURCE_KINDS = ("ln", "mbstd")


class Stage:
    def __init__(self, lin, in_shape):
        self.lin = lin
        self.kind = lin.kind
        self.in_shape = tuple(in_shape)
        self.out_shape = tuple(lin.out_shape(in_shape))
        self.bn = None
        self.ln = None
        self.pn = None
        self.pn_channels = None
        self.act = getattr(lin, "activation", None)
        self.alpha = 1.0
        self.drop = None
        self.mask_index = None
        self.folds_inference_bn = False
        self.geom = None
        if self.kind == "conv":
            self.geom = (*self.in_shape, lin.filters, lin.k, lin.stride)
        elif self.kind == "convT":
            self.geom = (*self.out_shape[:2], lin.filters, self.in_shape[2], lin.k, lin.stride)

    @property
    def fusable_grad(self):
        return self.bn is None and self.ln is None and self.pn is None and self.act == "lrelu"

    @property
    def drop_scale(self):
        return 1.0 / (1.0 - self.drop) if self.drop else 1.0

    def bn_args(self):
        v = self.bn.vars
        return dict(gamma=v["gamma"], beta=v["beta"], moving_mean=v["moving_mean"], moving_var=v["moving_variance"], eps=self.bn.epsilon)

    @property
    def ln_pixels(self):
        return int(np.prod(self.out_shape[:-1]))

    @property
    def pn_rows(self):
        return int(np.prod(self.out_shape)) // self.pn_channels


class _StageBuffers:
    def buf(self, lst, i):
        if lst[i] is None:
            lst[i] = torch.empty((self.B,) + self._net.stages[i].out_shape, dtype=torch.float32, device=self._device)
        return lst[i]

    def mbstd_source(self, i):
        st = self._net.stages[i]
        if self.s[i] is None:
            self.s[i] = torch.empty((self.B,) + st.in_shape, dtype=torch.float32, device=self._device)
        return self.s[i], self.mbstd_stats(i)[4]


class Context(_StageBuffers):

    def __init__(self, net, B, device, drop_rows=None):
        self.B = B
        self.drop_rows = B if drop_rows is None else int(drop_rows)
        f = lambda *s: torch.empty(*s, dtype=torch.float32, device=device)
        self.a0 = f(B, *net.in_shape)
        self.din = None
        self.a, self.z, self.keep, self.mean, self.inv, self.dz, self.v = [], [], [], [], [], [], []
        n = len(net.stages)
        self.u, self.u_rows, self.zdot, self.s, self.gin = [None] * n, None, [None] * n, [None] * n, [None] * n
        self.xin: List[Optional[torch.Tensor]] = [None] * len(net.stages)
        for st in net.stages:
            self.a.append(f(B, *st.out_shape))
            self.dz.append(None)
            self.v.append(None)
            self.z.append(f(B, *st.out_shape) if st.bn is not None or st.ln is not None or st.pn is not None else None)
            c = B * st.ln_pixels if st.ln is not None else B * st.pn_rows if st.pn is not None else st.out_shape[-1]
            self.mean.append(f(c) if st.bn is not None or st.ln is not None else None)
            self.inv.append(f(c) if st.bn is not None or st.ln is not None or st.pn is not None else None)
            self.keep.append(None)
        DR = self.drop_rows
        sizes = [int(np.prod((DR,) + st.out_shape)) if st.drop else 0 for st in net.stages]
        offs, total = [], 0
        for n in sizes:
            offs.append(total)
            total += -(-n // 16) * 16
        self.keep_flat = torch.empty(max(total, 16), dtype=torch.uint8, device=device)
        self.keep_total = total
        for i, (st, n) in enumerate(zip(net.stages, sizes)):
            if n:
                self.keep[i] = self.keep_flat[offs[i]:offs[i] + n].view((DR,) + st.out_shape)
        rates = {float(st.drop) for st in net.stages if st.drop}
        self.keep_rate = rates.pop() if len(rates) == 1 else None
        self._net, self._device = net, device
        net.check_rows(B)
        self._extra = {}
        self._bn_grad_scratch = {}
        self.dropout_active = False
        self.aug = None

    def keep_elems(self, i):
        return 0 if self.drop_rows >= self.B else self.drop_rows * int(np.prod(self._net.stages[i].out_shape))

    def dropout(self, i):
        st = self._net.stages[i]
        if not (st.drop and self.dropout_active):
            return None, 1.0, 0
        return self.keep[i], st.drop_scale, self.keep_elems(i)

    def masked_then_tail(self, i, launch):
        keep, scale, _ = self.dropout(i)
        if keep is not None and self.drop_rows < self.B:
            launch(slice(0, self.drop_rows), keep, scale)
            launch(slice(self.drop_rows, None), None, 1.0)
        else:
            launch(slice(None), keep, scale)

    def rows(self, lo, hi):
        return _RowView(self, lo, hi)

    def bn_partials(self, i, rows, C):
        key = ("bn_partials", i)
        n = rows * 2 * C
        if key not in self._extra or self._extra[key].numel() < n:
            self._extra[key] = torch.empty(n, dtype=torch.float32, device=self._device)
        return self._extra[key]

    def bn_sums(self, i, C):
        key = ("bn_sums", i)
        if key not in self._extra:
            self._extra[key] = torch.empty(2 * C, dtype=torch.float32, device=self._device)
        return self._extra[key]

    def bn_grad_scratch(self, i, C):
        if i not in self._bn_grad_scratch:
            self._bn_grad_scratch[i] = tuple(torch.empty(C, dtype=torch.float32, device=self._device) for _ in range(2))
        return self._bn_grad_scratch[i]

    def mbstd_stats(self, i):
        key = ("mbstd", i)
        if key not in self._extra:
            st = self._net.stages[i]
            n, E = self.B // st.lin.group_size, int(np.prod(st.in_shape))
            f = lambda *s: torch.empty(*s, dtype=torch.float32, device=self._device)
            self._extra[key] = (f(n, E), f(n, E), f(n), f(n), f(n))
        return self._extra[key]

    def keep_u(self, i, rows):
        n = rows[1] - rows[0]
        if self.u[i] is None or self.u[i].size(0) != n:
            self.u[i] = torch.empty((n,) + self._net.stages[i].out_shape, dtype=torch.float32, device=self._device)
        self.u_rows = tuple(rows)
        return self.u[i]

    def aug_input(self):
        if "aug_input" not in self._extra:
            self._extra["aug_input"] = torch.empty_like(self.a0)
        return self._extra["aug_input"]

    def blur_grad(self):
        if "blur_grad" not in self._extra:
            self._extra["blur_grad"] = torch.empty_like(self.a0)
        return self._extra["blur_grad"]

    def input_grad(self):
        if self.din is None:
            self.din = torch.empty((self.B,) + self._net.in_shape, dtype=torch.float32, device=self._device)
        return self.din


class _RowView(_StageBuffers):

    def __init__(self, ctx, lo, hi):
        self._ctx, self.lo, self.hi, self.B = ctx, lo, hi, hi - lo
        self.a = [t[lo:hi] for t in ctx.a]
        self.dz = [None if t is None else t[lo:hi] for t in ctx.dz]
        key = ("rowview_v", lo, hi)
        self.v = ctx._extra.setdefault(key, [None] * len(ctx.a))
        self._net, self._device = ctx._net, ctx._device
        px = [st.ln_pixels for st in ctx._net.stages]
        self.z = [None if t is None else t[lo:hi] for t in ctx.z]
        self.mean = [t[lo * n:hi * n] if st.ln is not None else None for t, n, st in zip(ctx.mean, px, ctx._net.stages)]
        self.inv = [t[lo * n:hi * n] if st.ln is not None else None for t, n, st in zip(ctx.inv, px, ctx._net.stages)]
        self.xin = [None if t is None else t[lo:hi] for t in ctx.xin]
        self.u, self.u_rows = ctx.u, (None if ctx.u_rows is None else (ctx.u_rows[0] - lo, ctx.u_rows[1] - lo))
        self.zdot = ctx._extra.setdefault(("rowview_zdot", lo, hi), [None] * len(ctx.a))
        self.s = ctx._extra.setdefault(("rowview_s", lo, hi), [None] * len(ctx.a))

    def mbstd_stats(self, i):
        G = self._net.stages[i].lin.group_size
        assert self.lo % G == 0 and self.hi % G == 0, (self.lo, self.hi, G)
        return tuple(t[self.lo // G:self.hi // G] for t in self._ctx.mbstd_stats(i))


class _BackwardPass:

    def __init__(self, ctx, need_dw, beta, scale, reducer, dw_rows, defer_conv_dw, sync_bn, keep_u_rows=None):
        self.ctx, self.need_dw, self.beta, self.scale, self.reducer = ctx, need_dw, beta, scale, reducer
        self.keep_u_rows = keep_u_rows
        self.dw_rows = ctx.B if dw_rows is None else int(dw_rows)
        self.defer_conv_dw, self.sync_bn = defer_conv_dw, sync_bn
        self.pending_stats = None
        self.deferred_ready = []

    def release_deferred(self):
        if self.reducer is not None:
            for rng in self.deferred_ready:
                self.reducer.ready(*rng)
        self.deferred_ready.clear()


_GP_SHAPE_MESSAGE = ("gradient penalty second order supports the reference critic shape only: "
                     "[Conv2D+LeakyReLU(+Dropout) | UpSampling2D | AveragePooling2D]* -> Flatten -> Dense(1) (demo_celeba.py:96-124)")


class Net:
    def __init__(self, flat_layers, store):
        self.store = store
        self.device = store.device
        self.blur = None
        self.capture_branches = None
        self.stages: List[Stage] = []
        self.latent_pn = None
        self.in_shape = tuple(flat_layers[0][1])
        cur = None
        n_masks = 0
        for idx, (l, s) in enumerate(flat_layers):
            k = l.kind
# ... 21 lines not shown
            elif k == "layernorm":
                if cur is not None and cur.bn is not None:
                    raise NotImplementedError("LayerNormalization together with BatchNormalization in one stage is not supported")
                if cur is not None and cur.act == "tanh":
                    raise NotImplementedError("LayerNormalization and tanh in one stage are not supported")
                if cur is None or cur.kind != "conv" or cur.ln is not None or cur.act is not None or cur.drop:
                    raise NotImplementedError("LayerNormalization must directly follow a Conv2D (not a Dense, a Conv2DTranspose or a "
                                              "resampling layer)")
                cur.ln = l
            elif k == "lrelu":
                if cur is None or cur.kind in PARAMETER_FREE or cur.act is not None or cur.drop:
                    raise NotImplementedError("LeakyReLU must follow a linear layer or its BatchNormalization")
                cur.act, cur.alpha = "lrelu", l.alpha
            elif k == "dropout":
                if cur is None or cur.kind in PARAMETER_FREE or cur.drop or cur.bn is not None or cur.act != "lrelu":
                    raise NotImplementedError("Dropout is supported after conv + LeakyReLU (demo_celeba.py:99-121)")
                cur.drop = l.rate
                if cur.drop:
                    cur.mask_index, n_masks = n_masks, n_masks + 1
            elif k in ("reshape", "flatten"):
                pass
            else:
                raise NotImplementedError(f"layer kind {k!r}")
        for st in self.stages:
            st.folds_inference_bn = st.bn is not None and st.kind != "dense" and st.lin.vars.get("bias") is None
            if st.kind == "dense" and st.bn is None and st.pn is None and st.act is not None:
                raise NotImplementedError("Dense + activation without BatchNormalization is not on the reference path")
            if st.act == "tanh" and st.bn is not None:
                raise NotImplementedError("tanh after BatchNormalization is not on the reference path")
            if st.ln is not None and st.act != "lrelu":
                raise NotImplementedError("LayerNormalization must be followed by a LeakyReLU")
        if self.stages and (self.stages[0].kind in RESAMPLE or self.stages[-1].kind in RESAMPLE):
            raise NotImplementedError("UpSampling2D / AveragePooling2D must stand between two linear layers, not first or last in a network")
        self.out_shape = self.stages[-1].out_shape
        self.conv_layers = [st.lin for st in self.stages if st.kind in ("conv", "convT")]
        self.spectral_layers = [st.lin for st in self.stages if isinstance(st.lin, SpectralNormalization)]
        self.eqlr_layers = [st.lin for st in self.stages if isinstance(st.lin, EqualizedLearningRate)]
        if self.spectral_layers and self.eqlr_layers:
            raise NotImplementedError("SpectralNormalization and EqualizedLearningRate layers in one model are not supported: both lay "
                                      "out the store's effective-weight buffer")
        self.plain_conv_layers = [l for l in self.conv_layers if not isinstance(l, (SpectralNormalization, EqualizedLearningRate))]
        rounds = {l.power_iterations for l in self.spectral_layers}
        if len(rounds) > 1:
            raise NotImplementedError(f"SpectralNormalization layers of one model must share power_iterations, got {sorted(rounds)}")
        self.spectral_rounds = rounds.pop() if rounds else 0
        self.has_ln = any(st.ln is not None for st in self.stages)
        self.mbstd_layers = [st.lin for st in self.stages if st.kind == "mbstd"]
        self.has_source = self.has_ln or bool(self.mbstd_layers)
        self.has_pn = self.latent_pn is not None or any(st.pn is not None for st in self.stages)
        self._ctx = {}
        self._rows_checked = set()
        self._ws = None
        self._taps_cache = {}
        self._taps_ring = {"i": 0, "bufs": [], "evs": []}
        self._splitk_bytes = {}
        self.rng_offset = 0
        self.conv_math = "fp32"
        self.sync_bn = True
        self.fuse_bn_stats = False

    def context(self, B, tag="default", drop_rows=None) -> Context:
        key = (B, tag, drop_rows)
        if key not in self._ctx:
            self._ctx[key] = Context(self, B, self.device, drop_rows=drop_rows)
        return self._ctx[key]

    def workspace(self, nbytes):
        n = max(int(nbytes), 1024)
        if self._ws is None or self._ws.numel() * 4 < n:
            self._ws = torch.empty((n + 3) // 4 + 1024, dtype=torch.float32, device=self.device)
        return self._ws

    def _epi(self, bwd_data, B, H, W, Cin, Cout, k, stride, mode, **kw):
        key = (bool(bwd_data), B, H, W, Cin, Cout, k, stride)
        nb = self._splitk_bytes.get(key)
        if nb is None:
            nb = self._splitk_bytes[key] = ops.conv2d_splitk_workspace_bytes(bwd_data, B, H, W, Cin, Cout, k, stride)
        return ops.epilogue(mode, ws=self.workspace(nb) if nb else None, **kw)

    def _conv(self, st, x, y, transpose, mode, **kw):
        bwd_data = (st.kind == "convT") != transpose
        lin = st.lin
        epi = self._epi(bwd_data, x.size(0), *st.geom, mode, **kw)
        if bwd_data:
            ops.conv2d_bwd_data(x, self.store.kernel(lin), y, lin.k, lin.stride, epi, math=self.conv_math)
        else:
            ops.conv2d_fwd(x, self.store.kernel(lin, transposed=True), y, lin.k, lin.stride, epi, math=self.conv_math)
        return epi

    def _filter_grad(self, st, a, dz, beta, scale):
        x, dy = (a, dz) if st.kind == "conv" else (dz, a)
        dW = self.store.grad_of(st.lin, "kernel")
        nb = ops.conv2d_bwd_filter_workspace_bytes(x.size(0), *st.geom)
        ops.conv2d_bwd_filter(x, dy, dW, st.lin.k, st.lin.stride, beta, scale, self.workspace(nb) if nb else None)

    def prepare_weights(self):
        self.spectral_update(iterate=False)
        self.eqlr_update()
        self.store.refresh_transposed(self.plain_conv_layers)

    def spectral_update(self, iterate=True):
        if not self.spectral_layers or not (iterate or self.store.sn_dirty):
            return
        table = self.store.spectral_table(self.spectral_layers)
        for _ in range(self.spectral_rounds if iterate else 1):
            ops.spectral.power(self.store.theta, self.store.state, table, sigma_only=not iterate)
        ops.spectral.scale(self.store.theta, self.store.state, self.store.eff, table)
        self.store.sn_dirty = False

    def spectral_project_gradients(self):
        if self.spectral_layers:
            ops.spectral.grad(self.store.grad, self.store.eff, self.store.state, self.store.spectral_table(self.spectral_layers))

    def eqlr_update(self):
        if self.eqlr_layers:
            table = self.store.eqlr_table(self.eqlr_layers)
            ops.eqlr.scale(self.store.theta, self.store.eff, table)

    def eqlr_scale_gradients(self):
        if self.eqlr_layers:
            ops.eqlr.grad(self.store.grad, self.store.eqlr_table(self.eqlr_layers))

    def blur_taps(self, H, W):
        std = float(self.blur.std)
        ent = self._taps_cache.get((H, W))
        if ent is None:
            ent = self._taps_cache[(H, W)] = {"std": None, "nt": 0, "dev": torch.zeros(1024, dtype=torch.float32, device=self.device)}
        if ent["std"] != std:
            ks, se, nt = ops.blur_policy(std, H, W)
            taps = ops.gauss_kernel_1d(se, ks)
            assert len(taps) == nt
            if nt > 1024:
                raise NotImplementedError(f"blur with {nt} taps (> 1024)")
            ring = self._taps_ring
            if not ring["bufs"]:
                for _ in range(8):
                    ring["bufs"].append(torch.empty(1024, dtype=torch.float32, pin_memory=self.device.type == "cuda"))
                    ring["evs"].append(None)
            i = ring["i"] = (ring["i"] + 1) % len(ring["bufs"])
            if ring["evs"][i] is not None:
                ring["evs"][i].synchronize()
            host = ring["bufs"][i][:nt]
            host.copy_(torch.tensor(taps, dtype=torch.float32))
            ent["dev"][:nt].copy_(host, non_blocking=True)
            if self.device.type == "cuda":
                ev = torch.cuda.Event()
                ev.record()
                ring["evs"][i] = ev
            ent["std"], ent["nt"] = std, nt
        return ent["dev"], ent["nt"]

    def blur_n_taps(self, H=None, W=None):
        if self.blur is None:
            return 0
        H = self.in_shape[0] if H is None else H
        W = self.in_shape[1] if W is None else W
        return self.blur_taps(H, W)[1]

    def apply_blur(self, x, y):
        B, H, W, C = x.shape
        taps, nt = self.blur_taps(H, W)
        nb = ops.blur_workspace_bytes(B, H, W, C, nt)
        tmp = self.workspace(nb) if nb else None
        with ops.trace_range("blur"):
            return ops.blur_nhwc(x, y, taps, nt, tmp)

    def forward(self, ctx: Context, inputs, training=False, masks=None, seed=0, lerp_alpha=None, lerp_out=None, augment=None):
        if self.store.tr_dirty:
            self.prepare_weights()
        x = self._assemble_input(ctx, inputs, lerp_alpha, lerp_out)
        ctx.aug = augment
        if augment is not None: x = self.aug_forward(ctx, x)
        if self.latent_pn is not None: x = self.pn_latents(ctx, x)
        ctx.dropout_active = bool(training)
        one_draw = bool(training and masks is None and ctx.keep_rate is not None and ctx.keep_total)
        if one_draw:
            ops.keep_mask(ctx.keep_flat[:ctx.keep_total], 1.0 - ctx.keep_rate, seed, counter=(self, "rng_offset"))
        folded = () if training else self._fold_inference_bns(ctx)
        for i, st in enumerate(self.stages):
            xin = ctx.xin[i] = x.view(ctx.B, *st.in_shape)
            x = ctx.a[i]
            if st.kind == "mbstd": self.mbstd_forward(ctx, i, st, xin, x); continue
            if st.kind in RESAMPLE:
                self._resample(st, xin, x)
            else:
                if st.drop and training and masks is not None:
                    ctx.keep[i].copy_(masks[st.mask_index].view(ctx.keep[i].shape))
                elif st.drop and training and not one_draw:
                    ops.keep_mask(ctx.keep[i], 1.0 - st.drop, seed, counter=(self, "rng_offset"))
                self._linear_forward(ctx, i, st, xin, x, training, i in folded)
        return x

    def _assemble_input(self, ctx, inputs, lerp_alpha, lerp_out):
        if not isinstance(inputs, (list, tuple)):
            inputs = [inputs]
        if lerp_alpha is not None:
            f, r = inputs
            n = int(f.shape[0])
            assert 3 * n == ctx.B
            if self.blur is not None:
                H, W, C = self.in_shape
                taps, nt = self.blur_taps(H, W)
                if not os.environ.get("BGAN_NO_FUSED_BLUR3") and ops.blur3_lerp_supported(n, H, W, C, nt):
                    with ops.trace_range("blur"):
                        ops.blur3_lerp(f.view(n, *self.in_shape), r.view(n, *self.in_shape), lerp_alpha, ctx.a0, taps, nt)
                    return ctx.a0
            inputs = [f, r, ops.lerp(r, f, lerp_alpha, lerp_out)]
        assert sum(int(t.shape[0]) for t in inputs) == ctx.B, "batch mismatch"
        if self.blur is None and len(inputs) == 1:
            return inputs[0]
        o = 0
        for t in inputs:
            n = int(t.shape[0])
            if self.blur is not None:
                self.apply_blur(t.view(n, *self.in_shape), ctx.a0[o:o + n])
            else:
                ops.copy_(ctx.a0[o:o + n], t.view(n, *self.in_shape).contiguous())
            o += n
        return ctx.a0

    def _fold_inference_bns(self, ctx):
        fl = [j for j, st in enumerate(self.stages) if st.folds_inference_bn]
        if not 1 < len(fl) <= ops.FOLD_MAX:
            return ()
        ops.bn_fold_many([(*self.stages[j].bn_args().values(), *self._fold_out(ctx, j)) for j in fl])
        return set(fl)

    def _fold_out(self, ctx, i):
        C = self.stages[i].out_shape[-1]
        sc = ctx.bn_sums(i, C)
        return sc[:C], sc[C:]

    def _linear_forward(self, ctx, i, st, xin, out, training, folded):
        if st.ln is not None: return self.ln_forward(ctx, i, st, xin, out)
        if st.pn is not None: return self.pn_forward(ctx, i, st, xin, out)
        bias = st.lin.vars.get("bias")
        tgt = ctx.z[i] if st.bn is not None else out
        stat_rows = 0
        if st.kind == "dense":
            ops.gemm(xin, self.store.kernel(st.lin), tgt, ctx.B, st.out_shape[0], st.in_shape[0], bias=bias)
        elif st.folds_inference_bn and not training:
            scale, shift = self._fold_out(ctx, i)
            if not folded:
                ops.bn_fold(**st.bn_args(), scale_out=scale, shift_out=shift)
            self._conv(st, xin, out, False, EPI_AFFINE_LRELU, bias=shift, ref=scale, alpha=st.alpha)
            return
        elif st.bn is not None:
            stats = None
            if training and bias is None and (self.fuse_bn_stats or (self.sync_bn and dist.collectives_active()
                                                                   and not os.environ.get("BGAN_NO_FUSED_BN_STATS"))):
                stats = ctx.bn_partials(i, int(np.prod((ctx.B,) + st.out_shape[:-1])) // 32 + 64, st.out_shape[-1])
            stat_rows = ops.conv2d_stats_rows(self._conv(st, xin, tgt, False, EPI_NONE, bias=bias, stats=stats))
        elif st.act == "lrelu":
            keep, _, keep_elems = ctx.dropout(i)
            self._conv(st, xin, tgt, False, EPI_BIAS_LRELU, bias=bias, keep=keep, alpha=st.alpha, scale=st.drop_scale, keep_elems=keep_elems)
        else:
            self._conv(st, xin, tgt, False, EPI_TANH if st.act == "tanh" else EPI_NONE, bias=bias)
        if st.bn is not None:
            self._bn_forward(ctx, i, st, tgt, out, training, stat_rows)

    def _bn_forward(self, ctx, i, st, tgt, out, training, stat_rows):
        C = st.out_shape[-1]
        M = tgt.numel() // C
        if not training:
            ops.bn_infer_fwd(tgt, out, M, C, **st.bn_args(), lrelu_alpha=st.alpha)
            return
        train = dict(st.bn_args(), save_mean=ctx.mean[i], save_inv=ctx.inv[i], momentum=st.bn.momentum,
                     unbiased=(len(st.out_shape) == 3), lrelu_alpha=st.alpha)
        if self.sync_bn and dist.collectives_active():
            sums = ctx.bn_sums(i, C)
            if stat_rows:
                ops.bn_sums_from_partials(ctx.bn_partials(i, stat_rows, C), stat_rows, C, sums)
            else:
                ops.bn_stats(tgt, M, C, sums, self.workspace(ops.bn_workspace_bytes(M, C)))
            dist.all_reduce_sum_(sums)
            ops.bn_finalize_apply(sums, M * dist.world_size(), tgt, out, M, C, **train)
        elif stat_rows:
            ops.bn_train_fwd_partials(ctx.bn_partials(i, stat_rows, C), stat_rows, tgt, out, M, C, **train)
        else:
            ops.bn_train_fwd(tgt, out, M, C, ws=self.workspace(ops.bn_workspace_bytes(M, C)), **train)

    def ln_args(self, ctx, i, st):
        C = st.out_shape[-1]
        return dict(R=ctx.B * st.ln_pixels, Cc=C, gamma=st.ln.vars["gamma"], mu=ctx.mean[i], r=ctx.inv[i])

    def ln_forward(self, ctx, i, st, xin, out):
        z = ctx.z[i]
        self._conv(st, xin, z, False, EPI_NONE, bias=st.lin.vars.get("bias"))
        keep, scale, keep_elems = ctx.dropout(i)
        ops.layernorm.fwd(z, out, **self.ln_args(ctx, i, st), beta=st.ln.vars["beta"], eps=st.ln.epsilon, lrelu_alpha=st.alpha, keep=keep,
                          scale=scale, keep_elems=keep_elems)

    @staticmethod
    def _resample(st, x, y):
        if st.kind == "upsample":
            ops.upsample2x(x, y, 1.0)
        else:
            ops.pool2x_sum(x, y, 0.25)

    def predict(self, x, training=False):
        B = x.size(0)
        ctx = self.context(B, "predict")
        x = x.to(self.device, torch.float32).contiguous()
        return self.forward(ctx, x, training=training, seed=np.random.randint(1 << 30)).clone()

    def backward(self, ctx: Context, dout, need_dx=False, need_dw=True, beta=0.0, scale=1.0, reducer=None, dw_rows=None,
                 dx_rows=None, defer_conv_dw=False, keep_u_rows=None):
        if need_dx and self.latent_pn is not None: raise NotImplementedError("the gradient at the input of a network that starts with a PixelNormalization (the latents' normalisation has no backward)")
        if need_dw:
            self.store.ensure_opt_state()
        p = _BackwardPass(ctx, need_dw, beta, scale, reducer, dw_rows, defer_conv_dw, self.sync_bn and dist.collectives_active(),
                          keep_u_rows if self.has_source else None)
        g, g_is_dz = dout, False
        for i in range(len(self.stages) - 1, -1, -1):
            st = self.stages[i]
            prev = self.stages[i - 1] if i > 0 else None
            has_dw = need_dw and st.kind not in PARAMETER_FREE
            dz = ctx.dz[i] = self._grad_through_activation(p, i, st, g.view(ctx.B, *st.out_shape), g_is_dz)
            overlap = has_dw and p.sync_bn and prev is not None and prev.bn is not None
            if has_dw and not overlap:
                self._weight_grads(p, i, st, dz)
            if i == 0 and not need_dx:
                p.release_deferred()
                return None
            g, g_is_dz = self._input_grad(p, i, st, prev, dz, dx_rows)
            if overlap:
                self._bn_bwd_stats(p, i - 1, prev, g)
                p.release_deferred()
                self._weight_grads(p, i, st, dz, defer_ready=True)
        p.release_deferred()
        if ctx.aug is not None: return self.aug_backward(ctx, g, dx_rows)
        if self.blur is not None:
            dst = ctx.a0 if p.keep_u_rows is None else ctx.blur_grad()
# ... 20 lines not shown
        C = st.out_shape[-1]
        M = gv.numel() // C
        dz = ctx.buf(ctx.dz, i)
        dg, db = (self.store.grad_of(st.bn, "gamma"), self.store.grad_of(st.bn, "beta")) if p.need_dw else ctx.bn_grad_scratch(i, C)
        gamma, beta = st.bn.vars["gamma"], st.bn.vars["beta"]
        if not p.sync_bn:
            ops.bn_train_bwd(gv, None, ctx.z[i], dz, M, C, gamma, ctx.mean[i], ctx.inv[i], dg, db,
                             self.workspace(ops.bn_workspace_bytes(M, C)), lrelu_alpha=st.alpha, beta=beta)
            return dz
        world = dist.world_size()
        if p.pending_stats is None:
            self._bn_bwd_stats(p, i, st, gv)
        p.pending_stats.wait()
        p.pending_stats = None
        sums = ctx.bn_sums(i, C)
        ops.bn_bwd_apply(gv, None, ctx.z[i], dz, M, M * world, C, gamma, ctx.mean[i], ctx.inv[i], sums, lrelu_alpha=st.alpha, beta=beta)
        if p.need_dw:
            ops.bn_param_grads(sums, C, 1.0 / world, dg, db)
        return dz

    def ln_backward(self, p, i, st, gv):
        ctx = p.ctx
        dz = ctx.buf(ctx.dz, i)
        keep, scale, keep_elems = ctx.dropout(i)
        args = self.ln_args(ctx, i, st)
        grads = {}
        if p.need_dw:
            grads = dict(dgamma=self.store.grad_of(st.ln, "gamma"), dbeta=self.store.grad_of(st.ln, "beta"), dw_rows=p.dw_rows * st.ln_pixels,
                         acc_beta=p.beta, acc_scale=p.scale, ws=self.workspace(ops.layernorm.workspace_bytes(args["R"], args["Cc"])))
        if p.keep_u_rows is not None:
            lo, hi = p.keep_u_rows
            grads.update(u_out=ctx.keep_u(i, (lo, hi)), u_rows=(lo * st.ln_pixels, hi * st.ln_pixels))
        return ops.layernorm.bwd(gv, ctx.z[i], dz, **args, beta=st.ln.vars["beta"], lrelu_alpha=st.alpha, keep=keep, scale=scale,
                                 keep_elems=keep_elems, **grads)

    def _bn_bwd_stats(self, p, i, st, g):
        ctx = p.ctx
        C = st.out_shape[-1]
        gv = g.view(ctx.B, *st.out_shape)
        M = gv.numel() // C
        sums = ctx.bn_sums(i, C)
        ops.bn_bwd_stats(gv, None, ctx.z[i], M, C, ctx.mean[i], ctx.inv[i], sums, self.workspace(ops.bn_workspace_bytes(M, C)),
                         lrelu_alpha=st.alpha, gamma=st.bn.vars["gamma"], beta=st.bn.vars["beta"])
        p.pending_stats = dist.all_reduce_sum_async(sums)

    def _weight_grads(self, p, i, st, dz, defer_ready=False):
        B, WB, lin = p.ctx.B, p.dw_rows, st.lin
        xin = p.ctx.xin[i]
        xw, dzw = (xin, dz) if WB == B else (xin[:WB], dz.view(B, *st.out_shape)[:WB])
        deferred = p.defer_conv_dw and st.kind == "conv"
        if st.kind == "dense":
            ops.gemm(xw, dzw, self.store.grad_of(lin, "kernel"), st.in_shape[0], st.out_shape[0], WB, transA=True, beta=p.beta, scale=p.scale)
        elif not deferred:
            self._filter_grad(st, xw, dzw, p.beta, p.scale)
        if "bias" in lin.vars:
            N = st.out_shape[-1]
            rows = dzw.numel() // N
            ops.colsum(dzw, self.store.grad_of(lin, "bias"), rows, N, self.workspace(ops.colsum_workspace_bytes(rows, N)), beta=p.beta, scale=p.scale)
        if p.reducer is not None and not deferred:
            if defer_ready:
                p.deferred_ready.append(self._train_range(st))
            else:
                p.reducer.ready(*self._train_range(st))

    def _train_range(self, st):
        return self.store.train_range(st.lin, st.bn if st.ln is None else st.ln)

    def _input_grad(self, p, i, st, prev, dz, dx_rows):
        ctx = p.ctx
        if st.kind == "mbstd": return self.mbstd_backward(p, i, st, prev, dz)
        fuse = prev is not None and prev.fusable_grad and st.kind not in ("dense", "upsample")
        below = ctx.gin if prev is not None and self.rereads_rows(prev) else ctx.dz
        tgt = (ctx.buf(below, i - 1) if i > 0 else ctx.input_grad()).view(ctx.B, *st.in_shape)
        if st.kind == "upsample":
            ops.pool2x_sum(dz.view(ctx.B, *st.out_shape), tgt, 1.0)
        elif st.kind == "avgpool" and not fuse:
            ops.upsample2x(dz.view(ctx.B, *st.out_shape), tgt, 0.25)
        elif st.kind == "avgpool":
            dzp, ref = dz.view(ctx.B, *st.out_shape), ctx.a[i - 1]
            ctx.masked_then_tail(i - 1, lambda rows, keep, scale: ops.upsample2x(dzp[rows], tgt[rows], 0.25, ref=ref[rows], keep=keep,
                                                                                alpha=prev.alpha, grad_scale=scale))
        else:
            if i == 0 and dx_rows is not None:
                lo, hi = dx_rows
                dz, tgt = dz.view(ctx.B, *st.out_shape)[lo:hi], tgt[lo:hi]
            if st.kind == "dense":
                ops.gemm(dz, self.store.kernel(st.lin), tgt, tgt.size(0), st.in_shape[0], st.out_shape[0], transB=True)
            elif fuse:
                keep, scale, keep_elems = ctx.dropout(i - 1)
                self._conv(st, dz, tgt, True, EPI_MUL_GRAD, ref=ctx.a[i - 1], keep=keep, alpha=prev.alpha, scale=scale, keep_elems=keep_elems)
            else:
                self._conv(st, dz, tgt, True, EPI_NONE)
        return tgt, fuse

    @staticmethod
    def rereads_rows(st):
        if st.ln is not None:
            return ops.layernorm.route(st.out_shape[-1])["chunks"] > 1
        return st.pn is not None and ops.pixelnorm.route(st.pn_channels)["chunks"] > 1

    PN_RULE = ("PixelNormalization is supported directly behind the LeakyReLU of a Dense (through its Reshape), Conv2D or Conv2DTranspose "
               "stage without BatchNormalization, LayerNormalization, Dropout or tanh, or as the network's first layer on a [C] vector")

    def pn_place(self, flat_layers, idx, cur):
        l, s = flat_layers[idx]
        if idx == 0:
            if len(s) != 1:
# ... 186 lines not shown
```

### blurred-gan_amd/ops.py

```python
from __future__ import annotations

import ctypes as C

import torch

from . import _lib, program
from ._lib import Epilogue, EPI_NONE, EPI_BIAS_LRELU, EPI_MUL_GRAD, EPI_TANH, EPI_AFFINE_LRELU, check

LRELU_ALPHA = 0.3


_dev_index = None
_raw_stream = getattr(torch._C, "_cuda_getCurrentRawStream", None)
_get_device = getattr(torch._C, "_cuda_getDevice", None)


def _stream():
    if _raw_stream is None or _get_device is None:
        return C.c_void_p(torch.cuda.current_stream().cuda_stream)
    cur = _get_device()
    if _dev_index is not None and cur != _dev_index:
        raise BgDeviceError(f"operands live on cuda:{_dev_index} but the current device is cuda:{cur}")
    return _raw_stream(cur)

# ... 249 lines not shown

def bn_fold_many(layers):
    import ctypes as C
    n = len(layers)
    assert 0 < n <= FOLD_MAX
    P = C.c_void_p * n
    cols = [P(*[_ptr(l[j]) for l in layers]) for j in (0, 1, 2, 3, 5, 6)]
    eps = (C.c_float * n)(*[float(l[4]) for l in layers])
    cs = (C.c_int * n)(*[int(l[0].numel()) for l in layers])
    check(_lib.load().bg_bn_fold_many_f32(n, cols[0], cols[1], cols[2], cols[3], eps, cs, cols[4], cols[5], _stream()),
          "bg_bn_fold_many_f32")


def bn_stats(x, M, Cc, sums, ws):
    check(_lib.load().bg_bn_stats_f32(_ptr(x), M, Cc, _ptr(sums), _ptr(ws), ws.numel() * ws.element_size(), _stream()), "bg_bn_stats_f32")
    return sums


def bn_finalize(sums, M_total, Cc, save_mean, save_inv, moving_mean, moving_var, eps=1e-3, momentum=0.99, unbiased=True):
    check(_lib.load().bg_bn_finalize_f32(_ptr(sums), M_total, Cc, _ptr(save_mean), _ptr(save_inv), _ptr(moving_mean), _ptr(moving_var),
                                         eps, momentum, int(unbiased), _stream()), "bg_bn_finalize_f32")


def bn_apply(x, y, M, Cc, gamma, beta, mean, inv, lrelu_alpha=LRELU_ALPHA):
    check(_lib.load().bg_bn_apply_f32(_ptr(x), _ptr(y), M, Cc, _ptr(gamma), _ptr(beta), _ptr(mean), _ptr(inv), lrelu_alpha, _stream()),
          "bg_bn_apply_f32")
    return y


def bn_finalize_apply(sums, M_total, x, y, M, Cc, gamma, beta, save_mean, save_inv, moving_mean, moving_var, eps=1e-3, momentum=0.99,
                      unbiased=True, lrelu_alpha=LRELU_ALPHA):
    check(_lib.load().bg_bn_finalize_apply_f32(_ptr(sums), M_total, _ptr(x), _ptr(y), M, Cc, _ptr(gamma), _ptr(beta), _ptr(save_mean),
                                               _ptr(save_inv), _ptr(moving_mean), _ptr(moving_var), eps, momentum, int(unbiased), lrelu_alpha,
                                               _stream()), "bg_bn_finalize_apply_f32")
    return y


def bn_bwd_stats(dy, y, x, M, Cc, save_mean, save_inv, sums, ws, lrelu_alpha=LRELU_ALPHA, gamma=None, beta=None):
    check(_lib.load().bg_bn_bwd_stats_f32(_ptr(dy), _ptr(y), _ptr(x), M, Cc, _ptr(gamma), _ptr(beta), _ptr(save_mean), _ptr(save_inv), lrelu_alpha, _ptr(sums),
                                          _ptr(ws), ws.numel() * ws.element_size(), _stream()), "bg_bn_bwd_stats_f32")
    return sums


def bn_bwd_apply(dy, y, x, dx, M, M_total, Cc, gamma, save_mean, save_inv, sums, lrelu_alpha=LRELU_ALPHA, beta=None):
    check(_lib.load().bg_bn_bwd_apply_f32(_ptr(dy), _ptr(y), _ptr(x), _ptr(dx), M, M_total, Cc, _ptr(gamma), _ptr(beta), _ptr(save_mean),
                                          _ptr(save_inv), _ptr(sums), lrelu_alpha, _stream()), "bg_bn_bwd_apply_f32")
    return dx


def bn_param_grads(sums, Cc, scale, dgamma, dbeta):
    check(_lib.load().bg_bn_param_grads_f32(_ptr(sums), Cc, scale, _ptr(dgamma), _ptr(dbeta), _stream()), "bg_bn_param_grads_f32")


class layernorm:

    @staticmethod
    def route(Cc):
        v = [C.c_int() for _ in range(4)]
        check(_lib.load().bg_ln_route(int(Cc), *[C.byref(x) for x in v]), "bg_ln_route")
        vec, lanes, regs, chunks = (x.value for x in v)
        return dict(vec=vec, lanes=lanes, regs=regs, chunks=chunks, rows_per_workgroup=4 * (64 // lanes))

    @staticmethod
    def workspace_bytes(R, Cc):
        return _lib.load().bg_ln_workspace_bytes(R, Cc)

    @staticmethod
    def _ws_bytes(ws):
        return 0 if ws is None else ws.numel() * ws.element_size()

    @staticmethod
    def fwd(z, a, R, Cc, gamma, beta, mu, r, eps=1e-3, lrelu_alpha=LRELU_ALPHA, keep=None, scale=1.0, keep_elems=0):
        _f32(z, a, gamma, beta, mu, r)
        assert z.numel() == R * Cc == a.numel() and gamma.numel() == Cc == beta.numel() and mu.numel() >= R and r.numel() >= R
        assert keep is None or (keep.dtype == torch.uint8 and keep.numel() >= (keep_elems or R * Cc))
        check(_lib.load().bg_ln_fwd_f32(_ptr(z), _ptr(a), R, Cc, _ptr(gamma), _ptr(beta), eps, lrelu_alpha, _ptr(keep), scale, int(keep_elems),
                                        _ptr(mu), _ptr(r), _stream()), "bg_ln_fwd_f32")
        return a

    @staticmethod
    def bwd(g, z, dz, R, Cc, gamma, beta, mu, r, lrelu_alpha=LRELU_ALPHA, keep=None, scale=1.0, keep_elems=0, addend=None, u_out=None,
            u_rows=None, dgamma=None, dbeta=None, dw_rows=0, acc_beta=0.0, acc_scale=1.0, ws=None):
        _f32(g, z, dz, gamma, beta, mu, r, addend, u_out, dgamma, dbeta)
        assert g.numel() == R * Cc == z.numel() == dz.numel() and (addend is None or addend.numel() == R * Cc)
        assert keep is None or (keep.dtype == torch.uint8 and keep.numel() >= (keep_elems or R * Cc))
        lo, hi = (0, R) if u_rows is None else u_rows
        assert u_out is None or u_out.numel() == (hi - lo) * Cc
        assert dgamma is None or (dgamma.numel() == Cc == dbeta.numel())
        check(_lib.load().bg_ln_bwd_f32(_ptr(g), _ptr(z), _ptr(dz), R, Cc, _ptr(gamma), _ptr(beta), _ptr(mu), _ptr(r), lrelu_alpha, _ptr(keep),
                                        scale, int(keep_elems), _ptr(addend), _ptr(u_out), lo, hi - lo, _ptr(dgamma), _ptr(dbeta), int(dw_rows),
                                        acc_beta, acc_scale, _ptr(ws), layernorm._ws_bytes(ws), _stream()), "bg_ln_bwd_f32")
        return dz

    @staticmethod
    def tangent(zdot, z, vout, R, Cc, gamma, beta, mu, r, lrelu_alpha=LRELU_ALPHA):
        _f32(zdot, z, vout, gamma, beta, mu, r)
        assert zdot.numel() == R * Cc == z.numel() == vout.numel()
        check(_lib.load().bg_ln_tangent_f32(_ptr(zdot), _ptr(z), _ptr(vout), R, Cc, _ptr(gamma), _ptr(beta), _ptr(mu), _ptr(r), lrelu_alpha,
                                            _stream()), "bg_ln_tangent_f32")
        return vout

    @staticmethod
    def gp_source(u, zdot, z, s, R, Cc, gamma, mu, r, dgamma, ws, acc_beta=1.0, acc_scale=1.0):
        _f32(u, zdot, z, s, gamma, mu, r, dgamma)
        assert u.numel() == R * Cc == zdot.numel() == z.numel() == s.numel() and dgamma.numel() == Cc
        check(_lib.load().bg_ln_gp_source_f32(_ptr(u), _ptr(zdot), _ptr(z), _ptr(s), R, Cc, _ptr(gamma), _ptr(mu), _ptr(r), _ptr(dgamma),
# ... 545 lines not shown
```

### blurred-gan_amd/wgan.py

```python
from __future__ import annotations

import numbers
import os
from contextlib import contextmanager
from dataclasses import dataclass
from typing import List

import numpy as np
import torch

from . import _lib, diffaugment, dist, ema as ema_mod, objective as objective_mod, ops, optimizers, program
from .gaussian_blur import Variable
from .layers import Sequential, get_seed
from .utils import JsonSerializable, ParseableFromCommandLine

_KEY_ENV = ("BGAN_NO_FUSED_BLUR3", "BGAN_NO_FUSED_BN_STATS", "BG_BLUR_BAND_LD", "BG_BLUR_NO_ROWS", "BG_BLUR_NO_PANEL", "BG_BLUR_PANEL16")


def _env_switches():
    return tuple(os.environ.get(k) for k in _KEY_ENV)


def _plain(v):
    if isinstance(v, (bool, np.bool_)):
        return bool(v)
    if isinstance(v, (numbers.Integral, np.integer)):
        return int(v)
    if isinstance(v, (numbers.Real, np.floating)):
        return float(v)
    return v


@dataclass
class TrainingConfig(JsonSerializable, ParseableFromCommandLine):
    log_dir: str = "results/log"
    checkpoint_dir: str = "results/log/checkpoints"
    save_image_summaries_interval: int = 50


class Mean:

    def __init__(self, name, dtype=None):
        self.name = name
        self.reset_states()

    def reset_states(self):
        self.total, self.count = 0.0, 0

    def __call__(self, value, weight=1):
        self.total += float(value) * weight
        self.count += weight

    update_state = __call__

    def result(self):
        return self.total / self.count if self.count else 0.0


class _SummaryWriter:

    def __init__(self, log_dir):
        self.log_dir = log_dir
        self._fh = None

    @contextmanager
    def as_default(self):
        yield self

    def scalar(self, name, value, step=None):
# ... 615 lines not shown
```

### include/bgan.h

```cpp
#ifndef BGAN_H
#define BGAN_H

#include <stddef.h>
#include <stdint.h>

#ifdef __cplusplus
extern "C" {
#endif

#define BG_ABI_VERSION 5

typedef enum {
  BG_OK = 0,
  BG_ERR_BAD_SHAPE = -1,
  BG_ERR_BAD_ALIGNMENT = -2,
  BG_ERR_UNSUPPORTED = -3,
  BG_ERR_HIP = -4,
  BG_ERR_WORKSPACE = -5,
  BG_ERR_NULL = -6,
  BG_ERR_RCCL = -7
} bg_status;

int bg_version(void);
const char* bg_last_error(void);
// ... 8 lines not shown
double bg_conv2d_useful_flops(int B, int H, int W, int Cin, int Cout, int ksize, int stride);

int bg_range_enable(int on);
int bg_range_push(const char* name);
int bg_range_pop(void);

int bg_blur_policy(float sigma, int H, int W, float* kernel_size, float* sigma_eff, int* n_taps);
int bg_gauss_kernel_1d(float sigma_eff, float kernel_size, float* taps_host, int cap, int* n_taps);
size_t bg_blur_workspace_bytes(int B, int H, int W, int C, int n_taps);
int bg_blur_nhwc_f32(const float* x, float* y, int B, int H, int W, int C,
                     const float* taps_d, int n_taps, float* tmp_d, void* stream);

int bg_blur3_lerp_supported(int B, int H, int W, int C, int n_taps);
int bg_blur3_lerp_nhwc_f32(const float* f, const float* r, const float* alpha_b, float* y3, int B, int H, int W, int C,
                           const float* taps_d, int n_taps, void* stream);

typedef enum {
  BG_EPI_NONE = 0,
  BG_EPI_BIAS_LRELU = 1,
  BG_EPI_MUL_GRAD = 2,
  BG_EPI_TANH = 3,
  BG_EPI_AFFINE_LRELU = 4
} bg_epi_mode;

typedef struct {
  int mode;
  const float* bias;
  const float* ref;
  const uint8_t* keep;
  float alpha;
  float scale;
  void* splitk_ws;
  size_t splitk_ws_bytes;
  size_t keep_elems;
  float* stats;
  size_t stats_capacity;
  int* stats_rows;
} bg_epilogue;

size_t bg_conv2d_splitk_workspace_bytes(int bwd_data, int B, int H, int W, int Cin, int Cout, int ksize, int stride);
int bg_conv2d_fwd(const float* x, const float* wT_d, float* y, int B, int H, int W, int Cin, int Cout,
                  int ksize, int stride, const bg_epilogue* epi, void* stream);
int bg_conv2d_bwd_data(const float* dy, const float* w_d, float* dx, int B, int H, int W, int Cin, int Cout,
                       int ksize, int stride, const bg_epilogue* epi, void* stream);
typedef enum { BG_CONV_MATH_FP32 = 0, BG_CONV_MATH_BF16X6 = 1 } bg_conv_math;
int bg_conv2d_fwd_math(const float* x, const float* wT_d, float* y, int B, int H, int W, int Cin, int Cout,
                       int ksize, int stride, const bg_epilogue* epi, void* stream, int math);
int bg_conv2d_bwd_data_math(const float* dy, const float* w_d, float* dx, int B, int H, int W, int Cin, int Cout,
                            int ksize, int stride, const bg_epilogue* epi, void* stream, int math);
int bg_conv2d_math_taken(int bwd_data, int B, int H, int W, int Cin, int Cout, int ksize, int stride, int math);
size_t bg_conv2d_bwd_filter_workspace_bytes(int B, int H, int W, int Cin, int Cout, int ksize, int stride);
int bg_conv2d_bwd_filter(const float* x, const float* dy, float* dw, int B, int H, int W, int Cin, int Cout,
                         int ksize, int stride, float beta, float scale, void* ws_d, size_t ws_bytes, void* stream);
int bg_transpose_last2(const float* src, float* dst, int T, int R, int C, void* stream);
int bg_transpose_last2_batched(const float* src_base, float* dst_base, const int* desc_d, int n, int total_tiles, void* stream);

int bg_gemm_f32(const float* A, const float* Bm, float* C, int M, int N, int K, int transA, int transB,
                const float* bias, float beta, float scale, void* stream);

size_t bg_colsum_workspace_bytes(int M, int N);
int bg_colsum_f32(const float* x, float* out, int M, int N, int square, float beta, float scale,
                  void* ws_d, size_t ws_bytes, void* stream);

size_t bg_bn_workspace_bytes(int M, int C);
int bg_bn_train_fwd(const float* x, float* y, int M, int C, const float* gamma, const float* beta,
                    float* moving_mean, float* moving_var, float* save_mean, float* save_inv,
                    float eps, float momentum, int unbiased, float lrelu_alpha,
                    void* ws_d, size_t ws_bytes, void* stream);
int bg_bn_infer_fwd(const float* x, float* y, int M, int C, const float* gamma, const float* beta,
                    const float* moving_mean, const float* moving_var, float eps, float lrelu_alpha, void* stream);
int bg_bn_train_bwd(const float* dy, const float* y, const float* x, float* dx, int M, int C,
                    const float* gamma, const float* beta, const float* save_mean, const float* save_inv,
                    float* dgamma, float* dbeta, float lrelu_alpha, void* ws_d, size_t ws_bytes, void* stream);

int bg_bn_fold_f32(const float* gamma, const float* beta, const float* moving_mean, const float* moving_var, float eps, int C,
                   float* scale_out, float* shift_out, void* stream);
int bg_bn_fold_many_f32(int n, const float* const* gamma, const float* const* beta, const float* const* moving_mean,
                        const float* const* moving_var, const float* eps, const int* C, float* const* scale_out,
                        float* const* shift_out, void* stream);
int bg_bn_stats_f32(const float* x, int M, int C, float* sums_d, void* ws_d, size_t ws_bytes, void* stream);
int bg_bn_finalize_f32(const float* sums_d, int M_total, int C, float* save_mean, float* save_inv, float* moving_mean,
                       float* moving_var, float eps, float momentum, int unbiased, void* stream);
int bg_bn_apply_f32(const float* x, float* y, int M, int C, const float* gamma, const float* beta, const float* mean,
                    const float* inv, float lrelu_alpha, void* stream);
int bg_bn_finalize_apply_f32(const float* sums_d, int M_total, const float* x, float* y, int M, int C, const float* gamma,
                             const float* beta, float* save_mean, float* save_inv, float* moving_mean, float* moving_var, float eps,
                             float momentum, int unbiased, float lrelu_alpha, void* stream);
int bg_bn_train_fwd_partials(const float* partial_d, int nrows, const float* x, float* y, int M, int C, const float* gamma,
                             const float* beta, float* moving_mean, float* moving_var, float* save_mean, float* save_inv, float eps,
                             float momentum, int unbiased, float lrelu_alpha, void* stream);
int bg_bn_sums_from_partials(const float* partial_d, int nrows, int C, float* sums_d, void* stream);
int bg_bn_bwd_stats_f32(const float* dy, const float* y, const float* x, int M, int C, const float* gamma, const float* beta,
                        const float* save_mean, const float* save_inv, float lrelu_alpha, float* sums_d, void* ws_d, size_t ws_bytes,
                        void* stream);
int bg_bn_bwd_apply_f32(const float* dy, const float* y, const float* x, float* dx, int M, int M_total, int C, const float* gamma,
                        const float* beta, const float* save_mean, const float* save_inv, const float* sums_d, float lrelu_alpha,
                        void* stream);
int bg_bn_param_grads_f32(const float* sums_d, int C, float scale, float* dgamma, float* dbeta, void* stream);

int bg_ln_route(int C, int* vec, int* lanes, int* regs, int* chunks);
size_t bg_ln_workspace_bytes(int R, int C);
int bg_ln_fwd_f32(const float* z, float* a, int R, int C, const float* gamma, const float* beta, float eps, float lrelu_alpha,
                  const uint8_t* keep , float keep_scale, size_t keep_elems, float* mu, float* r, void* stream);
int bg_ln_bwd_f32(const float* g, const float* z, float* dz, int R, int C, const float* gamma, const float* beta, const float* mu,
                  const float* r, float lrelu_alpha, const uint8_t* keep, float keep_scale, size_t keep_elems,
                  const float* addend , float* u_out, int u_row0, int u_rows, float* dgamma, float* dbeta, int dw_rows,
                  float acc_beta, float acc_scale, void* ws_d, size_t ws_bytes, void* stream);
int bg_ln_tangent_f32(const float* zdot, const float* z, float* vout, int R, int C, const float* gamma, const float* beta,
                      const float* mu, const float* r, float lrelu_alpha, void* stream);
int bg_ln_gp_source_f32(const float* u, const float* zdot, const float* z, float* s, int R, int C, const float* gamma, const float* mu,
                        const float* r, float* dgamma, float acc_beta, float acc_scale, void* ws_d, size_t ws_bytes, void* stream);

#define BG_PIXELNORM_ROUTE_INTS 8
int bg_pixelnorm_route(int C, int* out);
int bg_pixelnorm_fwd_f32(const float* x, float* y, float* r , int R, int C, float eps, float lrelu_alpha, void* stream);
int bg_pixelnorm_bwd_f32(const float* g, const float* y, const float* r, float* dz, int R, int C, float lrelu_alpha, void* stream);

int bg_diffaug_route(int H, int W, int C, int* resident, int* resident_floats);
int bg_diffaug_plan(int n, int H, int W, int C, int ops_mask, int* resident, int* threads, int* grid_x, int* grid_y, int* lds_bytes);
int bg_diffaug_decode(const float* u, int H, int W, int ops_mask, float translation_ratio, float cutout_ratio, float* bsc, int* geo);
int bg_diffaug_f32(const float* x, float* y, const float* params, int n, int H, int W, int C, int ops_mask, float translation_ratio,
                   float cutout_ratio, int linear, void* stream);
int bg_diffaug_adjoint_f32(const float* dy, float* dx, const float* params, int n, int H, int W, int C, int ops_mask,
                           float translation_ratio, float cutout_ratio, void* stream);

#define BG_MBSTD_PLAN_INTS 12
int bg_mbstd_plan(int N, int G, int P, int C, int call, int offset_floats, int* out);
size_t bg_mbstd_workspace_bytes(int N, int G, int P, int C);
int bg_mbstd_fwd_f32(const float* x, float* y, float* mu, float* rs, float* f, int N, int G, int P, int C, float eps, void* ws_d,
                     size_t ws_bytes, void* stream);
int bg_mbstd_bwd_f32(const float* u, const float* x, const float* mu, const float* rs, float* dx, float* q, int N, int G, int P, int C,
                     void* stream);
int bg_mbstd_gp_f32(const float* d, const float* x, const float* mu, const float* rs, const float* q, float* vout, float* src,
                    float* fdot, int N, int G, int P, int C, float eps, void* ws_d, size_t ws_bytes, void* stream);

#define BG_SPECTRAL_DESC_INTS 16
int bg_spectral_route(int K, int N, int taps, int* vec, int* lanes, int* chunks, int* strip_rows, int* pass_units, int* ew_units,
                      int* tiles, int* ws_floats);
size_t bg_spectral_workspace_bytes(const int* desc_h, int n);
int bg_spectral_power_f32(const float* theta, float* state, const int* desc_d, const int* desc_h, int n, int sigma_only, float* ws_d,
                          size_t ws_bytes, void* stream);
int bg_spectral_scale_f32(const float* theta, const float* state, float* eff, const int* desc_d, const int* desc_h, int n, void* stream);
int bg_spectral_grad_f32(float* grad, const float* eff, const float* state, const int* desc_d, const int* desc_h, int n, float* ws_d,
// ... 99 lines not shown
```

Measured before the change: 32630 images/s.

## Fuse BatchNorm+LeakyReLU apply into thin-channel conv forward and filter-grad input loads

For thin-channel stride-1 convs whose input is a batch-normalized, leaky-ReLU activation, the BN apply is moved into the conv kernels: the row-scatter forward kernel and the thin-Co weight-gradient kernel now normalize and activate input values as they load them. BN stats are computed by new stats-only entry points, so the normalized activation tensor no longer has to be written and re-read. This trades a separate elementwise pass and its memory traffic for extra ALU work inside the conv kernels, plus recomputation in the weight-gradient pass. The fused path is gated by a support check and an env switch.

Measured after the change: 32760 images/s (median of 6 runs). Within noise of the previous version (+0.4%).

```diff
diff --git a/blurred-gan_amd/_lib.py b/blurred-gan_amd/_lib.py
--- a/blurred-gan_amd/_lib.py
+++ b/blurred-gan_amd/_lib.py
@@ -15,6 +15,10 @@
     _fields_ = [("mode", C.c_int), ("bias", C.c_void_p), ("ref", C.c_void_p), ("keep", C.c_void_p),
                 ("alpha", C.c_float), ("scale", C.c_float), ("splitk_ws", C.c_void_p), ("splitk_ws_bytes", C.c_size_t),
                 ("keep_elems", C.c_size_t), ("stats", C.c_void_p), ("stats_capacity", C.c_size_t), ("stats_rows", C.POINTER(C.c_int))]
+
+
+class BnInput(C.Structure):
+    _fields_ = [("gamma", C.c_void_p), ("beta", C.c_void_p), ("mean", C.c_void_p), ("inv", C.c_void_p), ("alpha", C.c_float)]
 
 
 ABI_VERSION = 5
@@ -50,6 +54,9 @@
     "bg_conv2d_math_taken": (_i, [_i] * 9),
     "bg_conv2d_bwd_filter_workspace_bytes": (_z, [_i, _i, _i, _i, _i, _i, _i]),
     "bg_conv2d_bwd_filter": (_i, [_p, _p, _p, _i, _i, _i, _i, _i, _i, _i, _f, _f, _p, _z, _p]),
+    "bg_conv2d_bn_in_supported": (_i, [_i] * 7),
+    "bg_conv2d_fwd_bn_in": (_i, [_p, _p, _p, _i, _i, _i, _i, _i, _i, _i, C.POINTER(Epilogue), C.POINTER(BnInput), _p]),
+    "bg_conv2d_bwd_filter_bn_in": (_i, [_p, _p, _p, _i, _i, _i, _i, _i, _i, _i, _f, _f, _p, _z, C.POINTER(BnInput), _p]),
     "bg_transpose_last2": (_i, [_p, _p, _i, _i, _i, _p]),
     "bg_transpose_last2_batched": (_i, [_p, _p, _p, _i, _i, _p]),
     "bg_gemm_f32": (_i, [_p, _p, _p, _i, _i, _i, _i, _i, _p, _f, _f, _p]),
@@ -58,6 +65,8 @@
     "bg_bn_workspace_bytes": (_z, [_i, _i]),
     "bg_bn_train_fwd": (_i, [_p, _p, _i, _i, _p, _p, _p, _p, _p, _p, _f, _f, _i, _f, _p, _z, _p]),
     "bg_bn_train_fwd_partials": (_i, [_p, _i, _p, _p, _i, _i, _p, _p, _p, _p, _p, _p, _f, _f, _i, _f, _p]),
+    "bg_bn_train_stats": (_i, [_p, _i, _i, _p, _p, _p, _p, _f, _f, _i, _p, _p, _p, _p, _z, _p]),
+    "bg_bn_train_stats_partials": (_i, [_p, _i, _i, _i, _p, _p, _p, _p, _f, _f, _i, _p, _p, _p, _p]),
     "bg_bn_sums_from_partials": (_i, [_p, _i, _i, _p, _p]),
     "bg_bn_infer_fwd": (_i, [_p, _p, _i, _i, _p, _p, _p, _p, _f, _f, _p]),
     "bg_bn_train_bwd": (_i, [_p, _p, _p, _p, _i, _i, _p, _p, _p, _p, _p, _p, _f, _p, _z, _p]),
diff --git a/blurred-gan_amd/csrc/bn_act.h b/blurred-gan_amd/csrc/bn_act.h
--- /dev/null
+++ b/blurred-gan_amd/csrc/bn_act.h
@@ -0,0 +1,37 @@
+#pragma once
+#include <hip/hip_runtime.h>
+
+namespace bg {
+
+__device__ __forceinline__ float bn_lrelu(float x, float g, float m, float iv, float bt, float alpha) {
+  const float v = g * ((x - m) * iv) + bt;
+  return v > 0.f ? v : alpha * v;
+}
+
+struct BnInput {
+  const float* gamma;
+  const float* beta;
+  const float* mean;
+  const float* inv;
+  float alpha;
+};
+
+bool conv_wgrad_thin_co_takes(int B, int H, int W, int Cin, int Cout, int k, int s);
+
+struct BnQuad {
+  float4 g, bt, m, iv;
+  float alpha;
+  __device__ __forceinline__ void load(const BnInput& t, int c) {
+    g = make_float4(t.gamma[c], t.gamma[c + 1], t.gamma[c + 2], t.gamma[c + 3]);
+    bt = make_float4(t.beta[c], t.beta[c + 1], t.beta[c + 2], t.beta[c + 3]);
+    m = make_float4(t.mean[c], t.mean[c + 1], t.mean[c + 2], t.mean[c + 3]);
+    iv = make_float4(t.inv[c], t.inv[c + 1], t.inv[c + 2], t.inv[c + 3]);
+    alpha = t.alpha;
+  }
+  __device__ __forceinline__ float4 apply(const float4& x) const {
+    return make_float4(bn_lrelu(x.x, g.x, m.x, iv.x, bt.x, alpha), bn_lrelu(x.y, g.y, m.y, iv.y, bt.y, alpha),
+                       bn_lrelu(x.z, g.z, m.z, iv.z, bt.z, alpha), bn_lrelu(x.w, g.w, m.w, iv.w, bt.w, alpha));
+  }
+};
+
+}
diff --git a/blurred-gan_amd/csrc/conv_rows.hip b/blurred-gan_amd/csrc/conv_rows.hip
--- a/blurred-gan_amd/csrc/conv_rows.hip
+++ b/blurred-gan_amd/csrc/conv_rows.hip
@@ -1,3 +1,4 @@
+#include "bn_act.h"
 #include "conv_common.h"
 #include <algorithm>
 #include <cstdlib>
@@ -22,6 +23,7 @@
   const unsigned char* keep;
   size_t keep_elems;
   float alpha, scale;
+  bg::BnInput tf;
 };
 
 __device__ inline int floordiv(int a, int b) { return a >= 0 ? a / b : -((-a + b - 1) / b); }
@@ -36,7 +38,7 @@
   return copysignf(ax < 0.1f ? small : big, x);
 }
 
-template <int KS, int K, int S, int PIXW, int EP>
+template <int KS, int K, int S, int PIXW, int EP, bool TF = false>
 __global__ __launch_bounds__(PIXW * 4) void conv_rows_scatter_kernel(const RowParams p) {
   constexpr int NTH = PIXW * 4;
   constexpr unsigned kOob = 0x80000000u;
@@ -90,6 +92,9 @@
     l_off[q] = (unsigned)(pix * AS + c4 * 4);
   }
   const int rowB = p.Wi * Ck * 4;
+  static_assert(NTH % QPR == 0, "a thread's float4 of every row set holds the same channels");
+  bg::BnQuad tq;
+  if (TF) tq.load(p.tf, (tid % QPR) * 4);
   auto gload = [&](int r, float4 (&g)[NQ]) {
     const int iy = iy_lo + r;
     const bool row_ok = r < nrows && (unsigned)iy < (unsigned)p.Hi;
@@ -98,9 +103,15 @@
     for (int q = 0; q < NQ; ++q)
       g[q] = __builtin_bit_cast(float4, __builtin_amdgcn_raw_buffer_load_b128(rsA, (g_off[q] + add) | force, 0, 0));
   };
-  auto lstore = [&](int buf, const float4 (&g)[NQ]) {
-#pragma unroll
-    for (int q = 0; q < NQ; ++q) *reinterpret_cast<float4*>(abuf + (size_t)buf * PIXW * AS + l_off[q]) = g[q];
+  auto lstore = [&](int buf, int r, const float4 (&g)[NQ]) {
+    const int iy = iy_lo + r;
+    const bool row_ok = r < nrows && (unsigned)iy < (unsigned)p.Hi;
+#pragma unroll
+    for (int q = 0; q < NQ; ++q) {
+      float4 v = g[q];
+      if (TF) v = (row_ok & (g_off[q] != kOob)) ? tq.apply(v) : v;
+      *reinterpret_cast<float4*>(abuf + (size_t)buf * PIXW * AS + l_off[q]) = v;
+    }
   };
   const float* afrag = abuf + ((size_t)img * p.Wi + 16 * t + li) * AS + kq;
   constexpr int NE = (S * (16 / K) + 3) / 4;
@@ -167,7 +178,7 @@
   gload(1, g1);
   gload(2, g2);
   gload(3, g3);
-  lstore(0, g0);
+  lstore(0, 0, g0);
   gload(4, g0);
 #pragma unroll
   for (int i = 0; i < 4 * NE * S; ++i) __builtin_amdgcn_raw_buffer_store_b32(0u, rsC, kOob + 4u * i, 0, 0);
@@ -191,7 +202,7 @@
 #pragma unroll
       for (int kh = 0; kh < K; ++kh) acc[kh] = __builtin_amdgcn_mfma_f32_16x16x4f32(a[ks], bw[kh][ks], acc[kh], 0, 0, 0);
     flush_prev(cur ^ 1);
-    lstore(cur ^ 1, g);
+    lstore(cur ^ 1, r + 1, g);
     gload(r + 5, g);
 #pragma unroll
     for (int kh = 0; kh < S; ++kh) pwrite(acc[kh], cur * S + kh);
@@ -228,6 +239,22 @@
 int launch_rows(const RowParams& p, dim3 grid, size_t lds, hipStream_t s) {
   const bool wide = p.Wi == 128;
   const int ep = p.epi_mode == BG_EPI_NONE ? 0 : p.epi_mode == BG_EPI_TANH ? 1 : 2;
+  if (p.tf.gamma) {
+    if constexpr (S == 1) {
+#define BG_RT(KSv, EPv) do { if (wide) bg::launch((conv_rows_scatter_kernel<KSv, K, 1, 128, EPv, true>), grid, dim3(512), lds, s, p); \
+                             else bg::launch((conv_rows_scatter_kernel<KSv, K, 1, 64, EPv, true>), grid, dim3(256), lds, s, p); } while (0)
+#define BG_RTK(KSv) do { if (ep == 1) BG_RT(KSv, 1); else BG_RT(KSv, 2); } while (0)
+      switch (p.Ck) {
+        case 16: BG_RTK(4); return 1;
+        case 32: BG_RTK(8); return 1;
+        case 64: BG_RTK(16); return 1;
+        default: return 0;
+      }
+#undef BG_RTK
+#undef BG_RT
+    }
+    return 0;
+  }
 #define BG_RS2(KSv, EPv) do { if (wide) bg::launch((conv_rows_scatter_kernel<KSv, K, S, 128, EPv>), grid, dim3(512), lds, s, p); \
                               else bg::launch((conv_rows_scatter_kernel<KSv, K, S, 64, EPv>), grid, dim3(256), lds, s, p); } while (0)
 #define BG_RS(KSv) do { if (ep == 0) BG_RS2(KSv, 0); else if (ep == 1) BG_RS2(KSv, 1); else BG_RS2(KSv, 2); } while (0)
@@ -423,8 +450,8 @@
 
 
 
-int try_conv_rows(int bwd_data, const float* a, const float* w, float* c, int B, int H, int W, int Cin, int Cout, int k, int s,
-                  const bg_epilogue* epi, void* stream, int* taken) {
+static int conv_rows_impl(int bwd_data, const float* a, const float* w, float* c, int B, int H, int W, int Cin, int Cout, int k, int s,
+                          const bg_epilogue* epi, void* stream, int* taken, const BnInput* tf) {
   *taken = 0;
   static const int off = getenv("BG_NO_ROWS") ? 1 : 0;
   if (off || (k != 5 && k != 3)) return BG_OK;
@@ -433,6 +460,10 @@
   int Ho, Wo, pt, pl;
   same_pads(H, k, s, &Ho, &pt);
   same_pads(W, k, s, &Wo, &pl);
+  if (tf) {
+    if (bwd_data) return BG_OK;
+    p.tf = *tf;
+  }
   if (bwd_data) {
     if (Cin * k > 16 || (Cout != 16 && Cout != 32 && Cout != 64)) return BG_OK;
     p.Hi = Ho; p.Wi = Wo; p.Ck = Cout; p.Ho = H; p.Wo = W; p.N = Cin; p.pt = pt; p.pl = pl; p.flip = 0;
@@ -451,6 +482,10 @@
   const int pixw = p.Wi == 128 ? 128 : 64;
   if ((long)p.ipw * p.Wo * p.N > (long)((s * (16 / k) + 3) / 4) * pixw * 4) return BG_OK;
   if ((size_t)p.ipw * p.Hi * p.Wi * p.Ck >= (1ull << 29) || (size_t)p.ipw * p.Ho * p.Wo * p.N >= (1ull << 29)) return BG_OK;
+  if (!a) {
+    *taken = 1;
+    return BG_OK;
+  }
   p.epi_mode = BG_EPI_NONE; p.alpha = 0.3f; p.scale = 1.f;
   if (epi) {
     BG_REQUIRE(epi->mode >= BG_EPI_NONE && epi->mode <= BG_EPI_AFFINE_LRELU, BG_ERR_UNSUPPORTED, "conv rows: epilogue mode %d", epi->mode);
@@ -470,4 +505,34 @@
   return L.done("conv_rows_scatter_kernel");
 }
 
-}
+int try_conv_rows(int bwd_data, const float* a, const float* w, float* c, int B, int H, int W, int Cin, int Cout, int k, int s,
+                  const bg_epilogue* epi, void* stream, int* taken) {
+  return conv_rows_impl(bwd_data, a, w, c, B, H, W, Cin, Cout, k, s, epi, stream, taken, nullptr);
+}
+
+}
+
+extern "C" {
+
+int bg_conv2d_bn_in_supported(int B, int H, int W, int Cin, int Cout, int ksize, int stride) {
+  if (B <= 0 || H <= 0 || W <= 0 || Cin <= 0 || Cout <= 0 || ksize < 1 || !(ksize & 1) || ksize * ksize > bg::kMaxTaps || stride != 1) return 0;
+  int taken = 0;
+  bg::conv_rows_impl(0, nullptr, nullptr, nullptr, B, H, W, Cin, Cout, ksize, stride, nullptr, nullptr, &taken, nullptr);
+  return taken && bg::conv_wgrad_thin_co_takes(B, H, W, Cin, Cout, ksize, stride);
+}
+
+int bg_conv2d_fwd_bn_in(const float* x, const float* wT_d, float* y, int B, int H, int W, int Cin, int Cout, int ksize,
+                        int stride, const bg_epilogue* epi, const bg_bn_input* bn, void* stream) {
+  if (epi && epi->stats_rows) *epi->stats_rows = 0;
+  BG_REQUIRE(x && wT_d && y && bn && bn->gamma && bn->beta && bn->mean && bn->inv, BG_ERR_NULL, "bg_conv2d_fwd_bn_in: null pointer");
+  BG_REQUIRE(B > 0 && H > 0 && W > 0 && Cin > 0 && Cout > 0, BG_ERR_BAD_SHAPE, "bg_conv2d_fwd_bn_in: B=%d H=%d W=%d Cin=%d Cout=%d", B, H, W, Cin, Cout);
+  BG_REQUIRE(bg::aligned16(x) && bg::aligned16(wT_d) && bg::aligned16(y), BG_ERR_BAD_ALIGNMENT, "bg_conv2d_fwd_bn_in: pointers must be 16-byte aligned");
+  bg::UsefulScope useful(bg::conv_useful_flops(B, H, W, Cin, Cout, ksize, stride));
+  const bg::BnInput tf{bn->gamma, bn->beta, bn->mean, bn->inv, bn->alpha};
+  int taken = 0;
+  if (int rc = bg::conv_rows_impl(0, x, wT_d, y, B, H, W, Cin, Cout, ksize, stride, epi, stream, &taken, &tf)) return rc;
+  BG_REQUIRE(taken, BG_ERR_UNSUPPORTED, "bg_conv2d_fwd_bn_in: the row kernel does not take this shape");
+  return BG_OK;
+}
+
+}
diff --git a/blurred-gan_amd/csrc/conv_wgrad.hip b/blurred-gan_amd/csrc/conv_wgrad.hip
--- a/blurred-gan_amd/csrc/conv_wgrad.hip
+++ b/blurred-gan_amd/csrc/conv_wgrad.hip
@@ -1,3 +1,4 @@
+#include "bn_act.h"
 #include "conv_common.h"
 #include <algorithm>
 #include <cmath>
@@ -26,6 +27,7 @@
   int lg_w, lg_h, lg_b, pow2;
   int order_n;
   unsigned char tap_order[32];
+  bg::BnInput tf;
 };
 
 __device__ inline int fastdiv(int m, unsigned mul, unsigned sh) { return (int)(((unsigned long long)(unsigned)m * mul) >> sh); }
@@ -764,8 +766,9 @@
 
 typedef float floatx4 __attribute__((ext_vector_type(4)));
 constexpr int kTcRows = 16, kTcHalo = 8;
-
-template <int MT, int K>
+constexpr int kTcTailPad = 160;
+
+template <int MT, int K, bool TF = false>
 __global__ __launch_bounds__(256) void conv_wgrad_thin_co_kernel(const WgradParams p, int nblocks, int blocks_per_img) {
   extern __shared__ __attribute__((aligned(16))) float tc_lds[];
   const int W = p.W, H = p.H, Ci = 16 * MT, Co = p.Co;
@@ -783,6 +786,17 @@
   const int b_base = li < ncol ? kTcHalo + (kq + p.pl - kw_n) * Co + co_n : 0;
   const int b_step = li < ncol ? 4 * Co : 0;
   const int ksteps = W / 4;
+  if (ksteps & 7)
+    for (int i = tid; i < kTcTailPad; i += 256) tc_lds[nrows * RS + i] = 0.f;
+  float t_g[MT], t_bt[MT], t_m[MT], t_iv[MT];
+  const float t_alpha = p.tf.alpha;
+  if (TF) {
+#pragma unroll
+    for (int mt = 0; mt < MT; ++mt) {
+      const int ci = mt * 16 + li;
+      t_g[mt] = p.tf.gamma[ci]; t_bt[mt] = p.tf.beta[ci]; t_m[mt] = p.tf.mean[ci]; t_iv[mt] = p.tf.inv[ci];
+    }
+  }
 
   for (int blk = blockIdx.x; blk < nblocks; blk += gridDim.x) {
     const int b = blk / blocks_per_img, y0 = (blk - b * blocks_per_img) * kTcRows;
@@ -815,9 +829,16 @@
 #pragma unroll
         for (int mt = 0; mt < MT; ++mt) a[q][mt] = (it < nitems && g * 8 + q < ksteps) ? xrow[(size_t)q * 4 * Ci + mt * 16] : 0.f;
     };
-    auto compute = [&](int it, const float (&a)[8][MT]) {
+    auto compute = [&](int it, const float (&ain)[8][MT]) {
       const int j = it / groups, g = it - j * groups;
       const int r = wave + 4 * j;
+      float a[8][MT];
+      const int px = g * 32 + kq;
+#pragma unroll
+      for (int q = 0; q < 8; ++q)
+#pragma unroll
+        for (int mt = 0; mt < MT; ++mt)
+          a[q][mt] = (TF && px + 4 * q < W) ? bg::bn_lrelu(ain[q][mt], t_g[mt], t_m[mt], t_iv[mt], t_bt[mt], t_alpha) : ain[q][mt];
 #pragma unroll
       for (int kh = 0; kh < K; ++kh) {
         const float* brow = tc_lds + (r + (K - 1) - kh) * RS + b_base + g * 8 * b_step;
@@ -1388,7 +1409,7 @@
   return std::max((size_t)((thin_ci_rows(s) - 1) * s + k) * ((size_t)W * Ci + 2 * kTiHalo), (size_t)k * (Co / 16) * 4 * 64) * sizeof(float);
 }
 inline size_t thin_co_lds(int W, int Ci, int Co, int k) {
-  return std::max((size_t)(kTcRows + k - 1) * ((size_t)W * Co + 2 * kTcHalo), (size_t)4 * k * (Ci / 16) * 4 * 64) * sizeof(float);
+  return std::max((size_t)(kTcRows + k - 1) * ((size_t)W * Co + 2 * kTcHalo) + kTcTailPad, (size_t)4 * k * (Ci / 16) * 4 * 64) * sizeof(float);
 }
 
 WgradPlan plan_wgrad(int B, int H, int W, int Ci, int Co, int k, int s) {
@@ -1534,6 +1555,10 @@
 
 }
 
+namespace bg {
+bool conv_wgrad_thin_co_takes(int B, int H, int W, int Cin, int Cout, int k, int s) { return plan_wgrad(B, H, W, Cin, Cout, k, s).mode == 30; }
+}
+
 extern "C" {
 
 size_t bg_conv2d_bwd_filter_workspace_bytes(int B, int H, int W, int Cin, int Cout, int ksize, int stride) {
@@ -1543,8 +1568,23 @@
   return (size_t)pl.ksplit * ksize * ksize * Cin * Cout * sizeof(float);
 }
 
+static int bwd_filter_impl(const float* x, const float* dy, float* dw, int B, int H, int W, int Cin, int Cout, int ksize, int stride,
+                           float beta, float scale, void* ws_d, size_t ws_bytes, void* stream, const bg::BnInput* tf);
+
 int bg_conv2d_bwd_filter(const float* x, const float* dy, float* dw, int B, int H, int W, int Cin, int Cout, int ksize,
                          int stride, float beta, float scale, void* ws_d, size_t ws_bytes, void* stream) {
+  return bwd_filter_impl(x, dy, dw, B, H, W, Cin, Cout, ksize, stride, beta, scale, ws_d, ws_bytes, stream, nullptr);
+}
+
+int bg_conv2d_bwd_filter_bn_in(const float* x, const float* dy, float* dw, int B, int H, int W, int Cin, int Cout, int ksize,
+                               int stride, float beta, float scale, void* ws_d, size_t ws_bytes, const bg_bn_input* bn, void* stream) {
+  BG_REQUIRE(bn && bn->gamma && bn->beta && bn->mean && bn->inv, BG_ERR_NULL, "bg_conv2d_bwd_filter_bn_in: null pointer");
+  const bg::BnInput tf{bn->gamma, bn->beta, bn->mean, bn->inv, bn->alpha};
+  return bwd_filter_impl(x, dy, dw, B, H, W, Cin, Cout, ksize, stride, beta, scale, ws_d, ws_bytes, stream, &tf);
+}
+
+static int bwd_filter_impl(const float* x, const float* dy, float* dw, int B, int H, int W, int Cin, int Cout, int ksize, int stride,
+                           float beta, float scale, void* ws_d, size_t ws_bytes, void* stream, const bg::BnInput* tf) {
   BG_REQUIRE(x && dy && dw, BG_ERR_NULL, "bg_conv2d_bwd_filter: null pointer");
   BG_REQUIRE(B > 0 && H > 0 && W > 0 && Cin > 0 && Cout > 0, BG_ERR_BAD_SHAPE, "bg_conv2d_bwd_filter: B=%d H=%d W=%d Cin=%d Cout=%d", B, H, W, Cin, Cout);
   BG_REQUIRE(ksize >= 1 && (ksize & 1) && ksize * ksize <= bg::kMaxTaps, BG_ERR_UNSUPPORTED, "bg_conv2d_bwd_filter: kernel size %d", ksize);
@@ -1552,6 +1592,7 @@
   BG_REQUIRE(bg::aligned16(x) && bg::aligned16(dy) && bg::aligned16(dw), BG_ERR_BAD_ALIGNMENT, "bg_conv2d_bwd_filter: pointers must be 16-byte aligned");
   bg::UsefulScope useful(bg::conv_useful_flops(B, H, W, Cin, Cout, ksize, stride));
   WgradPlan pl = plan_wgrad(B, H, W, Cin, Cout, ksize, stride);
+  BG_REQUIRE(!tf || pl.mode == 30, BG_ERR_UNSUPPORTED, "bg_conv2d_bwd_filter_bn_in: the thin-Co row kernel does not take this shape");
   const size_t nout = (size_t)ksize * ksize * Cin * Cout;
   const bool slabs = pl.ksplit > 1 || pl.always_slab;
   const size_t need = slabs ? (size_t)pl.ksplit * nout * sizeof(float) : 0;
@@ -1590,6 +1631,7 @@
     p.xcd_swizzle = (pl.mode == 6 || pl.mode == 7) ? swz_tg : swz;
   }
   p.beta = beta; p.scale = scale;
+  if (tf) p.tf = *tf;
   p.order_n = 0;
   {
     static const int no_sort = getenv("BG_NO_TILE_SORT") ? 1 : 0;
@@ -1655,7 +1697,12 @@
     const int mt = Cin / 16;
     const size_t lds = thin_co_lds(W, Cin, Cout, ksize);
     BG_REQUIRE(lds <= kRowLdsMax, BG_ERR_UNSUPPORTED, "bg_conv2d_bwd_filter: thin-Co row kernel needs %zu bytes of LDS", lds);
-    if (ksize == 5 && mt == 2) bg::launch((conv_wgrad_thin_co_kernel<2, 5>), dim3(pl.ksplit), dim3(256), lds, L.s, p, nblocks, bpi);
+    if (p.tf.gamma) {
+      if (ksize == 5 && mt == 2) bg::launch((conv_wgrad_thin_co_kernel<2, 5, true>), dim3(pl.ksplit), dim3(256), lds, L.s, p, nblocks, bpi);
+      else if (ksize == 5) bg::launch((conv_wgrad_thin_co_kernel<1, 5, true>), dim3(pl.ksplit), dim3(256), lds, L.s, p, nblocks, bpi);
+      else if (mt == 2) bg::launch((conv_wgrad_thin_co_kernel<2, 3, true>), dim3(pl.ksplit), dim3(256), lds, L.s, p, nblocks, bpi);
+      else bg::launch((conv_wgrad_thin_co_kernel<1, 3, true>), dim3(pl.ksplit), dim3(256), lds, L.s, p, nblocks, bpi);
+    } else if (ksize == 5 && mt == 2) bg::launch((conv_wgrad_thin_co_kernel<2, 5>), dim3(pl.ksplit), dim3(256), lds, L.s, p, nblocks, bpi);
     else if (ksize == 5) bg::launch((conv_wgrad_thin_co_kernel<1, 5>), dim3(pl.ksplit), dim3(256), lds, L.s, p, nblocks, bpi);
     else if (mt == 2) bg::launch((conv_wgrad_thin_co_kernel<2, 3>), dim3(pl.ksplit), dim3(256), lds, L.s, p, nblocks, bpi);
     else bg::launch((conv_wgrad_thin_co_kernel<1, 3>), dim3(pl.ksplit), dim3(256), lds, L.s, p, nblocks, bpi);
diff --git a/blurred-gan_amd/csrc/misc.hip b/blurred-gan_amd/csrc/misc.hip
--- a/blurred-gan_amd/csrc/misc.hip
+++ b/blurred-gan_amd/csrc/misc.hip
@@ -1,3 +1,4 @@
+#include "bn_act.h"
 #include "common.h"
 #include "reduce.h"
 #include <algorithm>
@@ -297,11 +298,16 @@
 
 __global__ __launch_bounds__(kT) void bn_stats_final_kernel(const float* __restrict__ partial, int nblk, int M, int C, float* save_mean,
                                                             float* save_inv, float* moving_mean, float* moving_var, float eps,
-                                                            float momentum, int unbiased) {
+                                                            float momentum, int unbiased, const float* __restrict__ gamma,
+                                                            const float* __restrict__ beta, float* affine) {
   const int c = blockIdx.x * (kT / 64) + (threadIdx.x >> 6);
   if (c >= C) return;
   const float s = wave_sum_partials(partial, nblk, 2, 0, C, c), s2 = wave_sum_partials(partial, nblk, 2, 1, C, c);
   if ((threadIdx.x & 63) != 0) return;
+  if (affine) {
+    affine[c] = gamma[c];
+    affine[C + c] = beta[c];
+  }
   const float mean = s / (float)M;
   const float var = fmaxf(s2 / (float)M - mean * mean, 0.f);
   save_mean[c] = mean;
@@ -402,12 +408,8 @@
     const unsigned total4 = (unsigned)(total >> 2);
     const unsigned stride = gridDim.x * kT;
     auto one = [&](const float4& xv, const float4& g, const float4& bt, const float4& m, const float4& iv) {
-      float4 v;
-      v.x = g.x * ((xv.x - m.x) * iv.x) + bt.x; v.y = g.y * ((xv.y - m.y) * iv.y) + bt.y;
-      v.z = g.z * ((xv.z - m.z) * iv.z) + bt.z; v.w = g.w * ((xv.w - m.w) * iv.w) + bt.w;
-      v.x = v.x > 0.f ? v.x : alpha * v.x; v.y = v.y > 0.f ? v.y : alpha * v.y;
-      v.z = v.z > 0.f ? v.z : alpha * v.z; v.w = v.w > 0.f ? v.w : alpha * v.w;
-      return v;
+      return make_float4(bg::bn_lrelu(xv.x, g.x, m.x, iv.x, bt.x, alpha), bg::bn_lrelu(xv.y, g.y, m.y, iv.y, bt.y, alpha),
+                         bg::bn_lrelu(xv.z, g.z, m.z, iv.z, bt.z, alpha), bg::bn_lrelu(xv.w, g.w, m.w, iv.w, bt.w, alpha));
     };
     auto params = [&](int c, float4& g, float4& bt, float4& m, float4& iv) {
       g = load4_param(gamma, c, pa); bt = load4_param(beta, c, pa); m = load4_param(mean, c, pa);
@@ -437,8 +439,7 @@
   for (size_t e = (size_t)blockIdx.x * kT + threadIdx.x; e < total; e += (size_t)gridDim.x * kT) {
     const int c = (int)(e % C);
     const float inv = is_var ? 1.0f / sqrtf(inv_or_var[c] + eps) : inv_or_var[c];
-    float v = gamma[c] * ((x[e] - mean[c]) * inv) + beta[c];
-    y[e] = v > 0.f ? v : alpha * v;
+    y[e] = bg::bn_lrelu(x[e], gamma[c], mean[c], inv, beta[c], alpha);
   }
 }
 
@@ -931,13 +932,14 @@
 
 size_t bg_bn_workspace_bytes(int M, int C) { return bg_colsum_workspace_bytes(M, C); }
 
-int bg_bn_train_fwd(const float* x, float* y, int M, int C, const float* gamma, const float* beta, float* moving_mean,
-                    float* moving_var, float* save_mean, float* save_inv, float eps, float momentum, int unbiased,
-                    float lrelu_alpha, void* ws_d, size_t ws_bytes, void* stream) {
-  BG_REQUIRE(x && y && gamma && beta && save_mean && save_inv, BG_ERR_NULL, "bg_bn_train_fwd: null pointer");
-  BG_REQUIRE((moving_mean == nullptr) == (moving_var == nullptr), BG_ERR_NULL, "bg_bn_train_fwd: moving_mean/var must both be given or both NULL");
-  BG_REQUIRE(M > 0 && C > 0, BG_ERR_BAD_SHAPE, "bg_bn_train_fwd: M=%d C=%d", M, C);
-  BG_REQUIRE(ws_d && ws_bytes >= bg_bn_workspace_bytes(M, C), BG_ERR_WORKSPACE, "bg_bn_train_fwd: workspace too small");
+int bg_bn_train_stats(const float* x, int M, int C, float* moving_mean, float* moving_var, float* save_mean, float* save_inv, float eps,
+                      float momentum, int unbiased, const float* gamma, const float* beta, float* affine_d, void* ws_d, size_t ws_bytes,
+                      void* stream) {
+  BG_REQUIRE(x && save_mean && save_inv, BG_ERR_NULL, "bg_bn_train_stats: null pointer");
+  BG_REQUIRE(!affine_d || (gamma && beta), BG_ERR_NULL, "bg_bn_train_stats: the affine copy needs gamma and beta");
+  BG_REQUIRE((moving_mean == nullptr) == (moving_var == nullptr), BG_ERR_NULL, "bg_bn_train_stats: moving_mean/var must both be given or both NULL");
+  BG_REQUIRE(M > 0 && C > 0, BG_ERR_BAD_SHAPE, "bg_bn_train_stats: M=%d C=%d", M, C);
+  BG_REQUIRE(ws_d && ws_bytes >= bg_bn_workspace_bytes(M, C), BG_ERR_WORKSPACE, "bg_bn_train_stats: workspace too small");
   const int nblk = red_blocks(M, C);
   float* partial = static_cast<float*>(ws_d);
   const size_t total = (size_t)M * C;
@@ -948,13 +950,36 @@
     int rc = L.done("bn_stats_partial_kernel");
     if (rc) return rc;
   }
-  {
-    bg::Launch L(stream, "bn_stats_final", 0, 0);
-    bg::launch(bn_stats_final_kernel, dim3(bg::cdiv(C, kT / 64)), dim3(kT), 0, L.s, partial, nblk, M, C, save_mean, save_inv,
-                       moving_mean, moving_var, eps, momentum, unbiased);
-    int rc = L.done("bn_stats_final_kernel");
-    if (rc) return rc;
-  }
+  bg::Launch L(stream, "bn_stats_final", 0, 0);
+  bg::launch(bn_stats_final_kernel, dim3(bg::cdiv(C, kT / 64)), dim3(kT), 0, L.s, partial, nblk, M, C, save_mean, save_inv,
+                     moving_mean, moving_var, eps, momentum, unbiased, gamma, beta, affine_d);
+  return L.done("bn_stats_final_kernel");
+}
+
+int bg_bn_train_stats_partials(const float* partial_d, int nrows, int M, int C, float* moving_mean, float* moving_var, float* save_mean,
+                               float* save_inv, float eps, float momentum, int unbiased, const float* gamma, const float* beta,
+                               float* affine_d, void* stream) {
+  BG_REQUIRE(partial_d && save_mean && save_inv, BG_ERR_NULL, "bg_bn_train_stats_partials: null pointer");
+  BG_REQUIRE(!affine_d || (gamma && beta), BG_ERR_NULL, "bg_bn_train_stats_partials: the affine copy needs gamma and beta");
+  BG_REQUIRE((moving_mean == nullptr) == (moving_var == nullptr), BG_ERR_NULL, "bg_bn_train_stats_partials: moving_mean/var must both be given or both NULL");
+  BG_REQUIRE(M > 0 && C > 0 && nrows > 0, BG_ERR_BAD_SHAPE, "bg_bn_train_stats_partials: M=%d C=%d nrows=%d", M, C, nrows);
+  bg::Launch L(stream, "bn_stats_final", 0, 0);
+  bg::launch(bn_stats_final_kernel, dim3(bg::cdiv(C, kT / 64)), dim3(kT), 0, L.s, partial_d, nrows, M, C, save_mean, save_inv,
+                     moving_mean, moving_var, eps, momentum, unbiased, gamma, beta, affine_d);
+  return L.done("bn_stats_final_kernel");
+}
+
+int bg_bn_train_fwd(const float* x, float* y, int M, int C, const float* gamma, const float* beta, float* moving_mean,
+                    float* moving_var, float* save_mean, float* save_inv, float eps, float momentum, int unbiased,
+                    float lrelu_alpha, void* ws_d, size_t ws_bytes, void* stream) {
+  BG_REQUIRE(x && y && gamma && beta && save_mean && save_inv, BG_ERR_NULL, "bg_bn_train_fwd: null pointer");
+  BG_REQUIRE((moving_mean == nullptr) == (moving_var == nullptr), BG_ERR_NULL, "bg_bn_train_fwd: moving_mean/var must both be given or both NULL");
+  BG_REQUIRE(M > 0 && C > 0, BG_ERR_BAD_SHAPE, "bg_bn_train_fwd: M=%d C=%d", M, C);
+  BG_REQUIRE(ws_d && ws_bytes >= bg_bn_workspace_bytes(M, C), BG_ERR_WORKSPACE, "bg_bn_train_fwd: workspace too small");
+  if (int rc = bg_bn_train_stats(x, M, C, moving_mean, moving_var, save_mean, save_inv, eps, momentum, unbiased, nullptr, nullptr, nullptr, ws_d,
+                                 ws_bytes, stream))
+    return rc;
+  const size_t total = (size_t)M * C;
   bg::Launch L(stream, "bn_apply_lrelu", 0, 8.0 * total);
   bg::launch(bn_apply_kernel, dim3(grid_for(total)), dim3(kT), 0, L.s, x, y, total, C, gamma, beta, save_mean, save_inv, 0, eps,
                      lrelu_alpha);
@@ -971,7 +996,7 @@
   {
     bg::Launch L(stream, "bn_stats_final", 0, 0);
     bg::launch(bn_stats_final_kernel, dim3(bg::cdiv(C, kT / 64)), dim3(kT), 0, L.s, partial_d, nrows, M, C, save_mean, save_inv,
-                       moving_mean, moving_var, eps, momentum, unbiased);
+                       moving_mean, moving_var, eps, momentum, unbiased, (const float*)nullptr, (const float*)nullptr, (float*)nullptr);
     int rc = L.done("bn_stats_final_kernel");
     if (rc) return rc;
   }
diff --git a/blurred-gan_amd/engine.py b/blurred-gan_amd/engine.py
--- a/blurred-gan_amd/engine.py
+++ b/blurred-gan_amd/engine.py
@@ -72,6 +72,22 @@
         return self.s[i], self.mbstd_stats(i)[4]
 
 
+class _Activations(list):
+
+    def __init__(self, ctx):
+        super().__init__()
+        self._ctx = ctx
+
+    def held(self, i):
+        return list.__getitem__(self, i)
+
+    def __getitem__(self, i):
+        t = list.__getitem__(self, i)
+        if isinstance(i, int) and self._ctx.bn_in[i % len(self) + 1] is not None:
+            return self._ctx.thin_bn_activation(i % len(self))
+        return t
+
+
 class Context(_StageBuffers):
 
     def __init__(self, net, B, device, drop_rows=None):
@@ -80,12 +96,13 @@
         f = lambda *s: torch.empty(*s, dtype=torch.float32, device=device)
         self.a0 = f(B, *net.in_shape)
         self.din = None
-        self.a, self.z, self.keep, self.mean, self.inv, self.dz, self.v = [], [], [], [], [], [], []
+        self.a, self.z, self.keep, self.mean, self.inv, self.dz, self.v = _Activations(self), [], [], [], [], [], []
         n = len(net.stages)
         self.u, self.u_rows, self.zdot, self.s, self.gin = [None] * n, None, [None] * n, [None] * n, [None] * n
         self.xin: List[Optional[torch.Tensor]] = [None] * len(net.stages)
-        for st in net.stages:
-            self.a.append(f(B, *st.out_shape))
+        self.bn_in: List[Optional[dict]] = [None] * (len(net.stages) + 1)
+        for i, st in enumerate(net.stages):
+            self.a.append(None if net.thin_bn_candidate(B, i) else f(B, *st.out_shape))
             self.dz.append(None)
             self.v.append(None)
             self.z.append(f(B, *st.out_shape) if st.bn is not None or st.ln is not None or st.pn is not None else None)
@@ -140,6 +157,19 @@
             self._extra[key] = torch.empty(n, dtype=torch.float32, device=self._device)
         return self._extra[key]
 
+    def bn_affine(self, i, C):
+        key = ("bn_affine", i)
+        if key not in self._extra:
+            self._extra[key] = torch.empty(2 * C, dtype=torch.float32, device=self._device)
+        return self._extra[key]
+
+    def thin_bn_activation(self, i):
+        st, C = self._net.stages[i], self._net.stages[i].out_shape[-1]
+        if self.a.held(i) is None:
+            list.__setitem__(self.a, i, torch.empty((self.B,) + st.out_shape, dtype=torch.float32, device=self._device))
+        aff = self.bn_affine(i, C)
+        return ops.bn_apply(self.z[i], self.a.held(i), self.z[i].numel() // C, C, aff[:C], aff[C:], self.mean[i], self.inv[i], lrelu_alpha=st.alpha)
+
     def bn_sums(self, i, C):
         key = ("bn_sums", i)
         if key not in self._extra:
@@ -187,7 +217,7 @@
 
     def __init__(self, ctx, lo, hi):
         self._ctx, self.lo, self.hi, self.B = ctx, lo, hi, hi - lo
-        self.a = [t[lo:hi] for t in ctx.a]
+        self.a = [None if t is None else t[lo:hi] for t in ctx.a]
         self.dz = [None if t is None else t[lo:hi] for t in ctx.dz]
         key = ("rowview_v", lo, hi)
         self.v = ctx._extra.setdefault(key, [None] * len(ctx.a))
@@ -315,6 +345,7 @@
         self._rows_checked = set()
         self._ws = None
         self._taps_cache = {}
+        self._thin_bn = {}
         self._taps_ring = {"i": 0, "bufs": [], "evs": []}
         self._splitk_bytes = {}
         self.rng_offset = 0
@@ -341,7 +372,8 @@
             nb = self._splitk_bytes[key] = ops.conv2d_splitk_workspace_bytes(bwd_data, B, H, W, Cin, Cout, k, stride)
         return ops.epilogue(mode, ws=self.workspace(nb) if nb else None, **kw)
 
-    def _conv(self, st, x, y, transpose, mode, **kw):
+    def _conv(self, st, x, y, transpose, mode, bn_in=None, **kw):
+        if bn_in is not None: return self.thin_bn_conv(st, x, y, mode, bn_in, **kw)
         bwd_data = (st.kind == "convT") != transpose
         lin = st.lin
         epi = self._epi(bwd_data, x.size(0), *st.geom, mode, **kw)
@@ -351,7 +383,8 @@
             ops.conv2d_fwd(x, self.store.kernel(lin, transposed=True), y, lin.k, lin.stride, epi, math=self.conv_math)
         return epi
 
-    def _filter_grad(self, st, a, dz, beta, scale):
+    def _filter_grad(self, st, a, dz, beta, scale, bn_in=None):
+        if bn_in is not None: return self.thin_bn_filter_grad(st, a, dz, beta, scale, bn_in)
         x, dy = (a, dz) if st.kind == "conv" else (dz, a)
         dW = self.store.grad_of(st.lin, "kernel")
         nb = ops.conv2d_bwd_filter_workspace_bytes(x.size(0), *st.geom)
@@ -442,7 +475,7 @@
         folded = () if training else self._fold_inference_bns(ctx)
         for i, st in enumerate(self.stages):
             xin = ctx.xin[i] = x.view(ctx.B, *st.in_shape)
-            x = ctx.a[i]
+            x = self.thin_bn_out(ctx, i, training)
             if st.kind == "mbstd": self.mbstd_forward(ctx, i, st, xin, x); continue
             if st.kind in RESAMPLE:
                 self._resample(st, xin, x)
@@ -516,13 +549,15 @@
             stat_rows = ops.conv2d_stats_rows(self._conv(st, xin, tgt, False, EPI_NONE, bias=bias, stats=stats))
         elif st.act == "lrelu":
             keep, _, keep_elems = ctx.dropout(i)
-            self._conv(st, xin, tgt, False, EPI_BIAS_LRELU, bias=bias, keep=keep, alpha=st.alpha, scale=st.drop_scale, keep_elems=keep_elems)
+            self._conv(st, xin, tgt, False, EPI_BIAS_LRELU, bn_in=ctx.bn_in[i], bias=bias, keep=keep, alpha=st.alpha, scale=st.drop_scale,
+                       keep_elems=keep_elems)
         else:
-            self._conv(st, xin, tgt, False, EPI_TANH if st.act == "tanh" else EPI_NONE, bias=bias)
+            self._conv(st, xin, tgt, False, EPI_TANH if st.act == "tanh" else EPI_NONE, bn_in=ctx.bn_in[i], bias=bias)
         if st.bn is not None:
             self._bn_forward(ctx, i, st, tgt, out, training, stat_rows)
 
     def _bn_forward(self, ctx, i, st, tgt, out, training, stat_rows):
+        if ctx.bn_in[i + 1] is not None: return self.thin_bn_stats(ctx, i, st, tgt, stat_rows)
         C = st.out_shape[-1]
         M = tgt.numel() // C
         if not training:
@@ -542,6 +577,46 @@
             ops.bn_train_fwd_partials(ctx.bn_partials(i, stat_rows, C), stat_rows, tgt, out, M, C, **train)
         else:
             ops.bn_train_fwd(tgt, out, M, C, ws=self.workspace(ops.bn_workspace_bytes(M, C)), **train)
+
+    def thin_bn_candidate(self, B, i):
+        key = (B, i)
+        if key not in self._thin_bn:
+            st, nxt = self.stages[i], self.stages[i + 1] if i + 1 < len(self.stages) else None
+            ok = (st.bn is not None and st.kind in ("conv", "convT") and nxt is not None and nxt.kind == "conv" and nxt.bn is None
+                  and nxt.ln is None and nxt.pn is None and ops.thin_bn.supported(B, *nxt.geom))
+            self._thin_bn[key] = bool(ok)
+        return self._thin_bn[key]
+
+    def thin_bn_out(self, ctx, i, training):
+        st = self.stages[i]
+        fused = (training and self.thin_bn_candidate(ctx.B, i) and not os.environ.get("BGAN_NO_THIN_BN_FUSE")
+                 and not (self.sync_bn and dist.collectives_active())
+                 and not ops.conv2d_math_taken(False, ctx.B, *self.stages[i + 1].geom, self.conv_math))
+        ctx.bn_in[i + 1] = dict(gamma=st.bn.vars["gamma"], beta=st.bn.vars["beta"], mean=ctx.mean[i], inv=ctx.inv[i], alpha=st.alpha) if fused else None
+        if not fused and ctx.a.held(i) is None:
+            ctx.buf(ctx.a, i)
+        return ctx.z[i] if fused else ctx.a.held(i)
+
+    def thin_bn_stats(self, ctx, i, st, z, stat_rows):
+        C = st.out_shape[-1]
+        M = z.numel() // C
+        a = st.bn_args()
+        kw = dict(moving_mean=a["moving_mean"], moving_var=a["moving_var"], save_mean=ctx.mean[i], save_inv=ctx.inv[i], eps=a["eps"],
+                  momentum=st.bn.momentum, unbiased=(len(st.out_shape) == 3), gamma=a["gamma"], beta=a["beta"], affine=ctx.bn_affine(i, C))
+        if stat_rows:
+            ops.thin_bn.stats_partials(ctx.bn_partials(i, stat_rows, C), stat_rows, M, C, **kw)
+        else:
+            ops.thin_bn.stats(z, M, C, ws=self.workspace(ops.bn_workspace_bytes(M, C)), **kw)
+
+    def thin_bn_conv(self, st, z, y, mode, bn_in, **kw):
+        epi = self._epi(False, z.size(0), *st.geom, mode, **kw)
+        ops.thin_bn.conv2d_fwd(z, self.store.kernel(st.lin, transposed=True), y, st.lin.k, st.lin.stride, epi, **bn_in)
+        return epi
+
+    def thin_bn_filter_grad(self, st, z, dz, beta, scale, bn_in):
+        nb = ops.conv2d_bwd_filter_workspace_bytes(z.size(0), *st.geom)
+        ops.thin_bn.conv2d_bwd_filter(z, dz, self.store.grad_of(st.lin, "kernel"), st.lin.k, st.lin.stride, **bn_in, acc_beta=beta, scale=scale,
+                                      ws=self.workspace(nb) if nb else None)
 
     def ln_args(self, ctx, i, st):
         C = st.out_shape[-1]
@@ -668,7 +743,7 @@
         if st.kind == "dense":
             ops.gemm(xw, dzw, self.store.grad_of(lin, "kernel"), st.in_shape[0], st.out_shape[0], WB, transA=True, beta=p.beta, scale=p.scale)
         elif not deferred:
-            self._filter_grad(st, xw, dzw, p.beta, p.scale)
+            self._filter_grad(st, xw, dzw, p.beta, p.scale, bn_in=p.ctx.bn_in[i])
         if "bias" in lin.vars:
             N = st.out_shape[-1]
             rows = dzw.numel() // N
diff --git a/blurred-gan_amd/ops.py b/blurred-gan_amd/ops.py
--- a/blurred-gan_amd/ops.py
+++ b/blurred-gan_amd/ops.py
@@ -325,6 +325,62 @@
     check(_lib.load().bg_bn_param_grads_f32(_ptr(sums), Cc, scale, _ptr(dgamma), _ptr(dbeta), _stream()), "bg_bn_param_grads_f32")
 
 
+class thin_bn:
+
+    @staticmethod
+    def supported(B, H, W, Cin, Cout, ksize, stride):
+        return bool(_lib.load().bg_conv2d_bn_in_supported(B, H, W, Cin, Cout, ksize, stride))
+
+    @staticmethod
+    def _bn(gamma, beta, mean, inv, alpha):
+        _f32(gamma, beta, mean, inv)
+        assert gamma.numel() == beta.numel() == mean.numel() == inv.numel()
+        return _lib.BnInput(_ptr(gamma), _ptr(beta), _ptr(mean), _ptr(inv), alpha)
+
+    @staticmethod
+    def stats(x, M, Cc, moving_mean, moving_var, save_mean, save_inv, ws, eps=1e-3, momentum=0.99, unbiased=True, gamma=None, beta=None,
+              affine=None):
+        _f32(x, save_mean, save_inv, gamma, beta, affine)
+        assert x.numel() == M * Cc and (affine is None or (affine.numel() == 2 * Cc and gamma.numel() == Cc == beta.numel()))
+        check(_lib.load().bg_bn_train_stats(_ptr(x), M, Cc, _ptr(moving_mean), _ptr(moving_var), _ptr(save_mean), _ptr(save_inv), eps,
+                                            momentum, int(unbiased), _ptr(gamma), _ptr(beta), _ptr(affine), _ptr(ws),
+                                            ws.numel() * ws.element_size(), _stream()), "bg_bn_train_stats")
+
+    @staticmethod
+    def stats_partials(partial, nrows, M, Cc, moving_mean, moving_var, save_mean, save_inv, eps=1e-3, momentum=0.99, unbiased=True,
+                       gamma=None, beta=None, affine=None):
+        _f32(partial, save_mean, save_inv, gamma, beta, affine)
+        assert partial.numel() >= nrows * 2 * Cc and (affine is None or (affine.numel() == 2 * Cc and gamma.numel() == Cc == beta.numel()))
+        check(_lib.load().bg_bn_train_stats_partials(_ptr(partial), nrows, M, Cc, _ptr(moving_mean), _ptr(moving_var), _ptr(save_mean),
+                                                     _ptr(save_inv), eps, momentum, int(unbiased), _ptr(gamma), _ptr(beta), _ptr(affine),
+                                                     _stream()), "bg_bn_train_stats_partials")
+
+    @staticmethod
+    def conv2d_fwd(z, wT, y, ksize, stride, epi, gamma, beta, mean, inv, alpha=LRELU_ALPHA):
+        _f32(z, wT, y)
+        B, H, W, Cin = z.shape
+        Cout = y.shape[3]
+        assert wT.numel() == ksize * ksize * Cin * Cout and gamma.numel() == Cin
+        assert tuple(y.shape) == (B, same_out(H, stride), same_out(W, stride), Cout), (z.shape, y.shape)
+        bn = thin_bn._bn(gamma, beta, mean, inv, alpha)
+        check(_lib.load().bg_conv2d_fwd_bn_in(_ptr(z), _ptr(wT), _ptr(y), B, H, W, Cin, Cout, ksize, stride,
+                                              C.byref(epi) if epi is not None else None, C.byref(bn), _stream()), "bg_conv2d_fwd_bn_in")
+        return y
+
+    @staticmethod
+    def conv2d_bwd_filter(z, dy, dw, ksize, stride, gamma, beta, mean, inv, alpha=LRELU_ALPHA, acc_beta=0.0, scale=1.0, ws=None):
+        _f32(z, dy, dw)
+        B, H, W, Cin = z.shape
+        Cout = dy.shape[3]
+        assert dw.numel() == ksize * ksize * Cin * Cout and gamma.numel() == Cin
+        assert tuple(dy.shape[:3]) == (B, same_out(H, stride), same_out(W, stride))
+        bn = thin_bn._bn(gamma, beta, mean, inv, alpha)
+        wsb = ws.numel() * ws.element_size() if ws is not None else 0
+        check(_lib.load().bg_conv2d_bwd_filter_bn_in(_ptr(z), _ptr(dy), _ptr(dw), B, H, W, Cin, Cout, ksize, stride, acc_beta, scale,
+                                                     _ptr(ws), wsb, C.byref(bn), _stream()), "bg_conv2d_bwd_filter_bn_in")
+        return dw
+
+
 class layernorm:
 
     @staticmethod
diff --git a/blurred-gan_amd/wgan.py b/blurred-gan_amd/wgan.py
--- a/blurred-gan_amd/wgan.py
+++ b/blurred-gan_amd/wgan.py
@@ -14,7 +14,7 @@
 from .layers import Sequential, get_seed
 from .utils import JsonSerializable, ParseableFromCommandLine
 
-_KEY_ENV = ("BGAN_NO_FUSED_BLUR3", "BGAN_NO_FUSED_BN_STATS", "BG_BLUR_BAND_LD", "BG_BLUR_NO_ROWS", "BG_BLUR_NO_PANEL", "BG_BLUR_PANEL16")
+_KEY_ENV = ("BGAN_NO_FUSED_BLUR3", "BGAN_NO_FUSED_BN_STATS", "BGAN_NO_THIN_BN_FUSE", "BG_BLUR_BAND_LD", "BG_BLUR_NO_ROWS", "BG_BLUR_NO_PANEL", "BG_BLUR_PANEL16")
 
 
 def _env_switches():
diff --git a/include/bgan.h b/include/bgan.h
--- a/include/bgan.h
+++ b/include/bgan.h
@@ -84,6 +84,19 @@
 size_t bg_conv2d_bwd_filter_workspace_bytes(int B, int H, int W, int Cin, int Cout, int ksize, int stride);
 int bg_conv2d_bwd_filter(const float* x, const float* dy, float* dw, int B, int H, int W, int Cin, int Cout,
                          int ksize, int stride, float beta, float scale, void* ws_d, size_t ws_bytes, void* stream);
+typedef struct {
+  const float* gamma;
+  const float* beta;
+  const float* mean;
+  const float* inv;
+  float alpha;
+} bg_bn_input;
+int bg_conv2d_bn_in_supported(int B, int H, int W, int Cin, int Cout, int ksize, int stride);
+int bg_conv2d_fwd_bn_in(const float* x, const float* wT_d, float* y, int B, int H, int W, int Cin, int Cout,
+                        int ksize, int stride, const bg_epilogue* epi, const bg_bn_input* bn, void* stream);
+int bg_conv2d_bwd_filter_bn_in(const float* x, const float* dy, float* dw, int B, int H, int W, int Cin, int Cout,
+                               int ksize, int stride, float beta, float scale, void* ws_d, size_t ws_bytes, const bg_bn_input* bn,
+                               void* stream);
 int bg_transpose_last2(const float* src, float* dst, int T, int R, int C, void* stream);
 int bg_transpose_last2_batched(const float* src_base, float* dst_base, const int* desc_d, int n, int total_tiles, void* stream);
 
@@ -121,6 +134,12 @@
 int bg_bn_train_fwd_partials(const float* partial_d, int nrows, const float* x, float* y, int M, int C, const float* gamma,
                              const float* beta, float* moving_mean, float* moving_var, float* save_mean, float* save_inv, float eps,
                              float momentum, int unbiased, float lrelu_alpha, void* stream);
+int bg_bn_train_stats(const float* x, int M, int C, float* moving_mean, float* moving_var, float* save_mean, float* save_inv,
+                      float eps, float momentum, int unbiased, const float* gamma, const float* beta, float* affine_d, void* ws_d,
+                      size_t ws_bytes, void* stream);
+int bg_bn_train_stats_partials(const float* partial_d, int nrows, int M, int C, float* moving_mean, float* moving_var,
+                               float* save_mean, float* save_inv, float eps, float momentum, int unbiased, const float* gamma,
+                               const float* beta, float* affine_d, void* stream);
 int bg_bn_sums_from_partials(const float* partial_d, int nrows, int C, float* sums_d, void* stream);
 int bg_bn_bwd_stats_f32(const float* dy, const float* y, const float* x, int M, int C, const float* gamma, const float* beta,
                         const float* save_mean, const float* save_inv, float lrelu_alpha, float* sums_d, void* ws_d, size_t ws_bytes,
```
